# Daniel-Lin-S/decode_tonal_langauge

Measured on AMD Instinct MI355X. Metric: mel-frames/sec (train step) SynthesisModelCNN, 128ch x 400t batch256, higher is better.
Workload: dtype f32; 1 GPU; SynthesisModelCNN 128ch x 400t -> 80 mel, 4 tones x 2 syllables, L=5, global batch 256 (strong scaling: 256 windows on rank 0), dropout 0.5, NAdam, 1,376,768,720 params; per_gpu_batch=256, global_batch=256, parallelism=dp1, init=drawn on every rank

## Files before the change

### decode_tonal_langauge_amd/_classifier_engine.py

```python
from __future__ import annotations

import os
from typing import Dict, List, Tuple

import torch

from . import _kernels
from ._cnn_engine import CnnEngine, _r4
from ._lib import EPI_LRELU, EPI_STORE, LOAD_DIRECT, check, ptr


class CnnClassifierEngine(CnnEngine):
    F63_CAPABLE = False

    def __init__(self, n_electrodes: int, n_timepoints: int, stage_defs, hidden: int, n_classes: int,
                 negative_slope: float):
        super().__init__(n_classes, n_electrodes, n_timepoints, 0, stage_defs[-1][0], 0.0, negative_slope,
                         stage_defs, [4])
        self.hidden = hidden
        self.n_classes = n_classes
        last = self.stages[-1]
        self.c_last = last.cout
        self.tp_last = last.tp_out
        self.ld_last = last.cout if last.pool else self.ld5
        self.kflat_cls = n_electrodes * self.tp_last * self.ld_last
        self._packed: Dict[str, Tuple[int, torch.Tensor]] = {}
        self.n63, self.tp63 = self._plan63(stage_defs, n_timepoints)

    def _plan63(self, stage_defs, T):
        from . import _kernels
        if _kernels.get("wino") != "6":
            return 0, []
        c1, k1, p1 = stage_defs[0]
        if not (p1 and 1 <= k1 <= 3 and c1 in (128, 256, 512, 1024) and T >= 2 * self.tout1 + 2 and T * 4 <= 64 * 1024):
            return 0, []
        n, cin = 0, c1
        for st in self.stages:
            if not (st.k == 3 and st.pool and cin % 128 == 0 and st.cout % 64 == 0 and cin >= 40 and st.tout >= 1):
                break
            n, cin = n + 1, st.cout
        n = min(n, 3)
        if n == 0:
            return 0, []
        unit = 6 << (n - 1)
        tp = (self.tout1 + unit - 1) // unit * unit
        tps = []
        for _ in range(n):
            tps.append(tp)
            tp //= 2
        return n, tps

    def _forward63(self, convs, x, S, T):
        from ._lib import EPI_POOL, EPI_POOLV, LOAD_V
        lib, st_ = self.lib, self._stream()
        dev = x.device
        z = lambda *sh: torch.zeros(*sh, dtype=torch.float32, device=dev)
        zi = lambda *sh: torch.zeros(*sh, dtype=torch.int32, device=dev)
        buf = self._buf63
        w1, b1 = convs[0]
        tp1 = self.tp63[0]
        if "V1" not in buf:
            nh = S * tp1 // 6
            buf["V1"] = z((nh + 24 + 127) // 128 * 128, 8, self.c1)
            buf["b1"] = zi(S * tp1, self.c1 // 32)
        check(lib.tl_conv1_fwd_v6(ptr(x), ptr(w1.reshape(self.c1, self.k1).contiguous()), ptr(b1), None, ptr(buf["V1"]),
                                  ptr(buf["b1"]), None, S, T, self.k1, self.c1, tp1, self.tout1, self.slope, st_), "tl_conv1_fwd_v6")
        V = buf["V1"]
        tile_rows = self._nt63_rows()
        for i in range(self.n63):
            st, (w, b) = self.stages[i], convs[1 + i]
            tp_in = self.tp63[i]
            last = i == self.n63 - 1
            wp = self._cached(f"conv{st.idx}w63", w, lambda w=w: self._pack_wino63(w, True))
            rows_in = S * tp_in
            kb = f"bits{st.idx}"
            if kb not in buf:
                buf[kb] = zi(S * (st.tp_out if last else tp_in // 2), st.cout // 32)
            kw = dict(A=ptr(V), A_rows=V.shape[0], lda=V.shape[2], loader=LOAD_V, Bw=ptr(wp), bias=ptr(b), M=rows_in, N=st.cout,
                      K=st.cin, ldb=st.cin, J=3, row_shift=0, Tp=tp_in, slope=self.slope, obits=ptr(buf[kb]),
                      ld_obits=st.cout // 32, Tvalid=2 * st.tout)
            if last:
                dst = self.P[st.idx]
                self._nt(fn="tl_conv3_wino63v_nt", out=ptr(dst), ldo=dst.shape[1], epilogue=EPI_POOL, out_tp=st.tp_out, **kw)
            else:
                rows_out = S * (tp_in // 2)
                kv, kh = f"V{st.idx}", f"halo{st.idx}"
                ntm = -(-rows_in // tile_rows)
                if kv not in buf:
                    nh = rows_out // 6
                    buf[kv] = z((nh + 24 + 127) // 128 * 128, 8, st.cout)
                    buf[kh] = z(ntm, 2, st.cout)
                Vn, halo = buf[kv], buf[kh]
                self._nt(fn="tl_conv3_wino63v_nt", out=None, ldo=st.cout, epilogue=EPI_POOLV, vout=ptr(Vn), vhalo=ptr(halo),
                         vout_quads=Vn.shape[0], ld_vout=Vn.shape[2], **kw)
                check(lib.tl_wino63_v_fixup(ptr(Vn), ptr(halo), rows_out // 6, ntm, tp_in // 2, st.cout, Vn.shape[2], st_),
                      "tl_wino63_v_fixup")
                V = Vn
        return 1 + self.n63

    def _alloc(self, B: int, dev):
        if self._B == B and getattr(self, "_dev", None) == dev:
            return
        self._B, self._dev = B, dev
        S = B * self.C
        self.S = S
        self._buf63 = {}
        self.V = {}
        self._gy_A = None
        self._vhalo = {}
        z = lambda *s: torch.zeros(*s, dtype=torch.float32, device=dev)
        zi = lambda *s: torch.zeros(*s, dtype=torch.int32, device=dev)
        self.P = {1: z(S * self.tp1, self.c1)}
        self.bits = {1: zi(S * self.tp1, self.c1 // 32)}
        for st in self.stages:
            rows = S * st.tp_out
            self.P[st.idx] = z(rows, st.cout if st.pool else _r4(st.cout))
            if st.pool:
                self.bits[st.idx] = zi(rows, st.cout // 32)

    def _cached(self, key: str, param: torch.Tensor, build):
        ver = (param._version, param.data_ptr())
        hit = self._packed.get(key)
        if hit is None or hit[0] != ver:
            hit = self._packed[key] = (ver, build())
        return hit[1]

    def forward_scores(self, convs: List[Tuple[torch.Tensor, torch.Tensor]], fc1, fc2, x: torch.Tensor,
                       p_drop: float = 0.0, seed: int = 0) -> torch.Tensor:
        B, Cn, T = x.shape
        if Cn != self.C or T != self.T:
            raise ValueError(f"expected input (B, {self.C}, {self.T}), got {tuple(x.shape)}")
        x = x.contiguous().float()
        dev = x.device
        self._alloc(B, dev)
        lib, st_ = self.lib, self._stream()
        S = self.S
        w1, b1 = convs[0]
        done = 1
        if self.n63:
            done = self._forward63(convs, x, S, T)
        else:
            check(lib.tl_conv1_fwd(ptr(x), ptr(w1.reshape(self.c1, self.k1).contiguous()), ptr(b1), ptr(self.P[1]),
                                   ptr(self.bits[1]), None, S, T, self.k1, self.c1, self.tp1, self.tout1, self.slope, st_),
                  "tl_conv1_fwd")
        for st, (w, b) in list(zip(self.stages, convs[1:]))[done - 1:]:
            v43 = self._v43(st)
            if v43:
                wp = self._cached(f"conv{st.idx}w43", w, lambda w=w: self._pack_wino43(w, True))
            else:
                wp = self._cached(f"conv{st.idx}", w, lambda w=w, st=st: self._pack_conv(w, st.cin, False))
            src, dst = self.P[st.idx - 1], self.P[st.idx]
            kw = dict(A=ptr(src), Bw=ptr(wp), bias=ptr(b), out=ptr(dst), M=S * st.tp_in, A_rows=src.shape[0],
                      N=st.cout, K=st.cin, lda=src.shape[1], ldb=st.cin, ldo=dst.shape[1], J=st.k, row_shift=0,
                      Tp=st.tp_in, slope=self.slope, loader=LOAD_DIRECT)
            if st.pool:
                from ._lib import EPI_POOL
                kw.update(epilogue=EPI_POOL, obits=ptr(self.bits[st.idx]), ld_obits=st.cout // 32, Tvalid=2 * st.tout)
            else:
                kw.update(epilogue=EPI_LRELU, Tvalid=st.tout)
            if v43:
                from ._lib import LOAD_V
                V = self._input_transform(st)
                kw.update(A=ptr(V), A_rows=V.shape[0], lda=V.shape[2], loader=LOAD_V)
            self._nt(fn="tl_conv3_wino43v_nt" if v43 else "tl_gemm_nt_window", **kw)
        feat = self.P[self.stages[-1].idx]
        if p_drop > 0.0:
            check(lib.tl_dropout_scale(ptr(feat), feat.numel(), float(p_drop), int(seed), st_), "tl_dropout_scale")
        w_fc1, b_fc1 = fc1
        lat, latC = self.lat, self.lat * self.C

        def pack_fc1():
            dst = torch.empty(self.hidden, self.kflat_cls, dtype=torch.float32, device=dev)
            self._permute(w_fc1, dst, (self.hidden, self.C, self.tp_last, self.ld_last),
                          (self.c_last * latC, 1, self.C, latC), (self.hidden, self.C, lat, self.c_last))
            return dst
        wp1 = self._cached("fc1", w_fc1, pack_fc1)
        f32 = dict(dtype=torch.float32, device=dev)
        nkc = (self.kflat_cls + 31) // 32
        tiles = ((B + 127) // 128) * ((self.hidden + 127) // 128)
        sk = self._splitk(tiles, nkc, 1024)
        if sk > 1:
            slab = torch.empty(sk, B, self.hidden, **f32)
            self._nt(A=ptr(feat), Bw=ptr(wp1), out=ptr(slab), M=B, A_rows=B, N=self.hidden, K=self.kflat_cls,
                     lda=self.kflat_cls, ldb=self.kflat_cls, ldo=self.hidden, loader=LOAD_DIRECT, epilogue=EPI_STORE,
                     splitk=sk, slab_stride=B * self.hidden)
            a1 = torch.empty(B, self.hidden, **f32)
            check(lib.tl_splitk_bias_lrelu(ptr(slab), ptr(b_fc1), ptr(a1), sk, B * self.hidden, self.hidden, float(self.slope), st_),
                  "tl_splitk_bias_lrelu")
        else:
            a1 = torch.empty(B, self.hidden, **f32)
            self._nt(A=ptr(feat), Bw=ptr(wp1), bias=ptr(b_fc1), out=ptr(a1), M=B, A_rows=B, N=self.hidden,
                     K=self.kflat_cls, lda=self.kflat_cls, ldb=self.kflat_cls, ldo=self.hidden, loader=LOAD_DIRECT,
                     epilogue=EPI_LRELU, slope=self.slope)
        w_fc2, b_fc2 = fc2
        out = torch.empty(B, self.n_classes, **f32)
        if self.n_classes <= 64 and self.hidden % 4 == 0:
            check(lib.tl_linear_rows(ptr(a1), ptr(w_fc2.contiguous()), ptr(b_fc2), ptr(out), B, self.hidden, self.n_classes,
                                     self.hidden, 1, st_), "tl_linear_rows")
            return out
        self._nt(A=ptr(a1), Bw=ptr(w_fc2.contiguous()), bias=ptr(b_fc2), out=ptr(out), M=B, A_rows=B,
                 N=self.n_classes, K=self.hidden, lda=self.hidden, ldb=self.hidden, ldo=self.n_classes,
                 loader=LOAD_DIRECT, epilogue=EPI_STORE)
        return torch.sigmoid(out)


def _launch_nt(lib, fn: str = "tl_gemm_nt_window", **kw) -> None:
    import ctypes as C
    from ._lib import NtParams
    p = NtParams()
    p.splitk, p.bm, p.J, p.Tp, p.Tvalid, p.slope = 1, 128, 1, 1, 1, 0.0
    for k, v in kw.items():
        setattr(p, k, v)
    check(getattr(lib, fn)(C.byref(p), torch.cuda.current_stream().cuda_stream), fn)


class LstmInferEngine:

    def __init__(self, in_dim: int, hidden: int):
        from . import _lib
        self.lib = _lib.load()
        self.in_dim, self.H = in_dim, hidden
        self.Kp, self.Hp = _r4(in_dim), (hidden + 7) // 8 * 8
        self._packed = None

    def _weights(self, w_ih, w_hh, b_ih, b_hh):
        ver = tuple((t._version, t.data_ptr()) for t in (w_ih, w_hh, b_ih, b_hh))
        if self._packed is None or self._packed[0] != ver:
            H, Hp, Kp, dev = self.H, self.Hp, self.Kp, w_hh.device
            wi = torch.zeros(4, Hp, Kp, dtype=torch.float32, device=dev)
            wi[:, :H, :self.in_dim] = w_ih.detach().float().view(4, H, self.in_dim)
            wh = torch.zeros(4, Hp, Hp, dtype=torch.float32, device=dev)
            wh[:, :H, :H] = w_hh.detach().float().view(4, H, H)
            bs = torch.zeros(4, Hp, dtype=torch.float32, device=dev)
            bs[:, :H] = (b_ih.detach().float() + b_hh.detach().float()).view(4, H)
            whp = wh.permute(1, 0, 2).contiguous().view(4 * Hp, Hp)
            self._packed = (ver, wi.view(4 * Hp, Kp), wh.view(4 * Hp, Hp), bs.view(4 * Hp), whp)
        return self._packed[1:]

    @torch.no_grad()
    def last_hidden(self, x_seq: torch.Tensor, w_ih, w_hh, b_ih, b_hh) -> torch.Tensor:
        B, T, D = x_seq.shape
        if D != self.in_dim:
            raise ValueError(f"expected input width {self.in_dim}, got {D}")
        dev = x_seq.device
        wi, wh, bs, whp = self._weights(w_ih, w_hh, b_ih, b_hh)
        H, Hp, Kp = self.H, self.Hp, self.Kp
        f32 = dict(dtype=torch.float32, device=dev)
        x = x_seq.float()
        if Kp != D:
            xp_in = torch.zeros(B, T, Kp, **f32)
            xp_in[:, :, :D] = x
            x = xp_in
        x = x.contiguous()
        rows = B * T
        xp = torch.empty(rows, 4 * Hp, **f32)
        _launch_nt(self.lib, A=ptr(x), Bw=ptr(wi), bias=ptr(bs), out=ptr(xp), M=rows, A_rows=rows, N=4 * Hp, K=Kp,
                   lda=Kp, ldb=Kp, ldo=4 * Hp, loader=LOAD_DIRECT, epilogue=EPI_STORE)
        h = torch.empty(B, Hp, **f32)
        c = torch.empty(B, Hp, **f32)
        import ctypes as C
        h2 = torch.empty(B, Hp, **f32)
        in_b = C.c_int(0)
        check(self.lib.tl_lstm_infer_seq_fused(ptr(xp), T * 4 * Hp, ptr(whp), ptr(h), ptr(h2), ptr(c), B, Hp, T,
                                               C.byref(in_b), torch.cuda.current_stream().cuda_stream),
              "tl_lstm_infer_seq_fused")
        h = h2 if in_b.value else h
        return h[:, :H] if Hp != H else h


class CnnRnnConvEngine:

    K = 7

    def __init__(self, input_channels: int, input_length: int, lstm_dim: int, negative_slope: float):
        from . import _lib
        self.lib = _lib.load()
        self.C, self.T = input_channels, input_length
        self.w1 = lstm_dim // input_length
        self.W = self.w1 + input_channels
        self.slope = float(negative_slope)
        self.t1 = (input_length - self.K + 1) // 2
        self.ta = self.t1 - self.K + 1
        self.tb = self.ta - self.K + 1
        self.tq = self.tb // 3
        if self.tq < 1:
            raise ValueError("input_length too small for the CNN-RNN convolution stack")
        _kernels.validate()
        self.conv7_form = _kernels.get("conv7")
        self.Tp = (self.t1 + 5) // 6 * 6 if self.conv7_form == "wino63" else (self.t1 + 3) // 4 * 4
        self._packed: Dict[str, Tuple[tuple, torch.Tensor]] = {}
        self._B = None

    def _cached(self, key: str, param: torch.Tensor, build):
        ver = (param._version, param.data_ptr())
        hit = self._packed.get(key)
        if hit is None or hit[0] != ver:
            hit = self._packed[key] = (ver, build())
        return hit[1]

    def _alloc(self, B: int, dev):
        if self._B == B and self._dev == dev:
            return
        self._B, self._dev = B, dev
        z = lambda *s: torch.zeros(*s, dtype=torch.float32, device=dev)
        zi = lambda *s: torch.zeros(*s, dtype=torch.int32, device=dev)
        rows = B * self.W * self.Tp
        self.P, self.Y1, self.Y2 = z(rows + 8, 1024), z(rows + 8, 512), z(rows, 256)
        nb = B * self.w1 * self.Tp
        self.Pb, self.Pa = self.P[:nb], self.P[nb:rows]
        self.bits_a, self.bits_b = zi(B * self.C * self.Tp, 32), zi(B * self.w1 * self.Tp, 32)
        self.V7 = None
        if self.conv7_form == "wino63":
            nh_pad = (rows // 6 + 2 + 127) // 128 * 128
            self.V7 = (z(nh_pad, 8, 1024), z(nh_pad, 8, 1024))

    def _conv7(self, src, w, b, dst, cin, cout, key, rows):
        from ._lib import NtParams
        import ctypes as C
        st_ = torch.cuda.current_stream().cuda_stream
        if self.conv7_form == "wino63" and cin % 8 == 0 and cout % 32 == 0:
            nhex = rows // 6
            V0 = self.V7[0].view(-1)[: self.V7[0].shape[0] * 8 * cin].view(-1, 8, cin)
            V1 = self.V7[1].view(-1)[: self.V7[1].shape[0] * 8 * cin].view(-1, 8, cin)
            tvalid = self.t1 if cin == 1024 else self.ta
            if V0.shape[2] != self.V7[0].shape[2]:
                h0 = (nhex + 1) // 2 * 2
                V0[h0:].zero_()
                V1[h0:].zero_()
            check(self.lib.tl_wino63_xform2(ptr(src), ptr(V0), ptr(V1), rows, self.Tp, tvalid, cin, src.shape[1], cin, st_),
                  "tl_wino63_xform2")

            def pack63():
                wp = torch.empty(3 * cin // 8, 8, cout, 8, dtype=torch.float32, device=w.device)
                check(self.lib.tl_wino63_weights7(ptr(w.detach().reshape(cout, cin, self.K).contiguous()), ptr(wp), cout, cin,
                                                  self.K, st_), "tl_wino63_weights7")
                return wp
            wp = self._cached(key + "wino63", w, pack63)
            from ._lib import LOAD_V
            _launch_nt(self.lib, fn="tl_conv7_wino63v_nt", A=ptr(V0), aux=ptr(V1), A_rows=V0.shape[0], lda=cin, Bw=ptr(wp),
                       bias=ptr(b.detach()), out=ptr(dst), M=rows, N=cout, K=cin, ldb=3 * cin, ldo=dst.shape[1], J=self.K,
                       row_shift=0, Tp=self.Tp, Tvalid=self.Tp, slope=self.slope, loader=LOAD_V, epilogue=EPI_LRELU)
            return
        if src.shape[0] < rows + 8:
            raise RuntimeError("conv7: the input buffer is shorter than the rows the 7-tap window reads")
        wp = self._cached(key + "direct", w, lambda: w.detach().reshape(cout, cin, self.K).permute(2, 0, 1).contiguous())
        p = NtParams()
        p.A, p.Bw, p.bias, p.out = ptr(src), ptr(wp), ptr(b.detach()), ptr(dst)
        p.M, p.A_rows = rows, rows + 8
        p.N, p.K, p.lda, p.ldb, p.ldo = cout, cin, cin, cin, cout
        p.J, p.row_shift, p.Tp, p.Tvalid, p.slope = self.K, 0, self.Tp, self.Tp, self.slope
        p.loader, p.epilogue, p.splitk, p.bm = LOAD_DIRECT, EPI_LRELU, 1, 128
        check(self.lib.tl_gemm_nt_window(C.byref(p), st_), "tl_gemm_nt_window")

    @torch.no_grad()
    def linear(self, a: torch.Tensor, w: torch.Tensor, b: torch.Tensor, sigmoid: bool = False) -> torch.Tensor:
        a = a.contiguous().float()
        B, K = a.shape
        if K % 4 != 0:
            raise ValueError("linear: the feature width must be a multiple of 4")
        N = w.shape[0]
        out = torch.empty(B, N, dtype=torch.float32, device=a.device)
        if N <= 64:
            check(self.lib.tl_linear_rows(ptr(a), ptr(w.contiguous()), ptr(b), ptr(out), B, K, N, K, int(sigmoid),
                                          torch.cuda.current_stream().cuda_stream), "tl_linear_rows")
            return out
        _launch_nt(self.lib, A=ptr(a), Bw=ptr(w.contiguous()), bias=ptr(b), out=ptr(out), M=B, A_rows=B, N=N, K=K, lda=K,
                   ldb=K, ldo=N, loader=LOAD_DIRECT, epilogue=EPI_STORE)
        return torch.sigmoid(out) if sigmoid else out

    @torch.no_grad()
    def features(self, x: torch.Tensor, h1: torch.Tensor, block1, block2, conv3a, conv3b, p_drop: float = 0.0,
                 seed: int = 0) -> torch.Tensor:
        B = x.shape[0]
        dev = x.device
        self._alloc(B, dev)
        lib, st_ = self.lib, torch.cuda.current_stream().cuda_stream
        xa = x.contiguous().float()
        xb = h1.float().reshape(B, self.T, self.w1).permute(0, 2, 1).contiguous()
        for seqs, n, (w, b), P, bits in ((xa, B * self.C, block1, self.Pa, self.bits_a),
                                         (xb, B * self.w1, block2, self.Pb, self.bits_b)):
            check(lib.tl_conv1_fwd(ptr(seqs), ptr(w.detach().reshape(1024, self.K).contiguous()), ptr(b.detach()), ptr(P),
                                   ptr(bits), None, n, self.T, self.K, 1024, self.Tp, self.t1, self.slope, st_),
                  "tl_conv1_fwd")
        rows = B * self.W * self.Tp
        self._conv7(self.P, conv3a[0], conv3a[1], self.Y1, 1024, 512, "conv3a", rows)
# ... 10 lines not shown
```

### decode_tonal_langauge_amd/_cnn_engine.py

```python
from __future__ import annotations

import ctypes as C
import os
import math
from typing import Dict, List, Optional

import torch

from . import _kernels, _lib
from ._lib import (EPI_C1WGRAD, EPI_GY, EPI_LRELU, EPI_MASK, EPI_MASKY, EPI_POOL, EPI_POOLV, EPI_STORE, LOAD_DIRECT, LOAD_UNPOOL, LOAD_V,
                   LOAD_Y, NtParams, TnParams, check, ptr)


def _r4(n: int) -> int:
    return (n + 3) // 4 * 4


class _Stage:

    def __init__(self, idx, cin, cout, k, pool, tin, tp_in):
        self.idx, self.cin, self.cout, self.k, self.pool = idx, cin, cout, k, pool
        self.tin, self.tp_in = tin, tp_in
        self.tc = tin - k + 1
        self.tout = self.tc // 2 if pool else self.tc
        self.tp_out = tp_in // 2 if pool else tp_in


class CnnEngine:
    F63_CAPABLE = True

    def __init__(self, output_dim: int, n_channels: int, n_timepoints: int, lstm_channels: int,
                 conv_channels: int, dropout: float, negative_slope: float, stage_defs, concat_widths):
        if negative_slope < 0:
            raise ValueError("the MI355X path needs negative_slope >= 0 (max-pool / LeakyReLU are fused)")
        self.lib = _lib.load()
        self.out_dim = output_dim
        self.C = n_channels
        self.T = n_timepoints
        self.Lc = lstm_channels
        self.Cc = conv_channels
        self.p_drop = float(dropout)
        self.slope = float(negative_slope)
        self.cslope = 0.1
        k1 = stage_defs[0][1]
        npool_after = sum(1 for s in stage_defs[1:] if s[2])
        tc1 = n_timepoints - k1 + 1
        self.k1 = k1
        self.c1 = stage_defs[0][0]
        self.tout1 = tc1 // 2
        if not stage_defs[0][2]:
            raise ValueError("first stage must pool")
        align = 1 << npool_after
        self.tp1 = max(align, (self.tout1 + align - 1) // align * align)
        _kernels.validate()
        self.wino63 = (self.F63_CAPABLE and _kernels.get("wino") == "6"
                       and self._f63_covers(stage_defs, n_timepoints))
        tp1_default = self.tp1
        if self.wino63:
            self.tp1 = (self.tout1 + 11) // 12 * 12
        self.f63_yprod = (self.wino63 and _kernels.get("f63_yprod") != "0" and stage_defs[0][0] % 256 == 0
                          and self.tp1 >= 12)
        self.f63_yprod3 = (self.wino63 and _kernels.get("f63_yprod") != "0" and stage_defs[1][0] % 256 == 0)
        self.stages: List[_Stage] = []
        cin, tin, tp = self.c1, self.tout1, self.tp1
        for i, (cout, k, pool) in enumerate(stage_defs[1:], start=2):
            st = _Stage(i, cin, cout, k, pool, tin, tp)
            if st.tout < 1:
                raise ValueError("n_timepoints too small for the conv stack")
            if self.wino63 and i == 3:
                st.tp_out = tp1_default // 4
            self.stages.append(st)
            cin, tin, tp = cout, st.tout, st.tp_out
        self.gy4 = self._gy_applies()
        self.lat = tin
        self.tp5 = tp
        self.H = self.lat * n_channels * lstm_channels
        self.ld5 = _r4(conv_channels)
        self.ldx = _r4(conv_channels + lstm_channels)
        self.concat_dims = []
        cin_t, cin_ld = conv_channels + lstm_channels, self.ldx
        for w in concat_widths:
            self.concat_dims.append((cin_t, cin_ld, w, _r4(w)))
            cin_t, cin_ld = w, _r4(w)
        self.ldy5 = self.concat_dims[-1][3]
        self.kflat = n_channels * self.tp5 * self.ldy5
        self.ldd = _r4(output_dim)
        self.lowrank_param = "label_lstm.weight_hh_l0"
        self.lstm_shard = None
        self._sh = None
        self.timers = None
        mode = _kernels.get("wino")
        self.wino43 = mode != "0"
        self.store_p1 = _kernels.get("store_p1") == "1"
        self.fuse_c1 = True
        self.wino_vout = True
        self.tn_bm = 0
        self._gy_A = None
        self._vhalo = {}
        self._B = None
        self.generation = 0
        self._saved_generation = -1

    def _alloc(self, B: int, dev):
        if self._B == B and self._dev == dev:
            return
        self._B, self._dev = B, dev
        S = B * self.C
        self.S = S
        f32 = dict(dtype=torch.float32, device=dev)
        z = lambda *s: torch.zeros(*s, **f32)
        zi = lambda *s: torch.zeros(*s, dtype=torch.int32, device=dev)
        self._v_ready = {}
        self._gy_A = None
        self._vhalo = {}
        self.P = {}
        if not (self.wino63 or self._conv1_writes_v()) or self.store_p1:
            self.P[1] = z(S * self.tp1, self.c1)
        self.bits = {1: zi(S * self.tp1, self.c1 // 32)}
        self.sbits = {1: zi(S * self.tp1, self.c1 // 32)}
        for st in self.stages:
            rows = S * st.tp_out
            ld = st.cout if st.pool else self.ld5
            no_rows = (self.wino63 and st.idx == 2) or (self._writes_v(st) and not self._f63(st))
            if not no_rows or self.store_p1:
                self.P[st.idx] = z(rows, ld)
            if st.pool:
                self.bits[st.idx] = zi(rows, st.cout // 32)
                self.sbits[st.idx] = zi(rows, st.cout // 32)
        rows5 = S * self.tp5
        self.rows5 = rows5
        self.Xc = z(rows5, self.ldx)
        self.Y = [z(rows5, d[3]) for d in self.concat_dims]
        self.out_slab = None
        self.Yt = {}
        self._y_ready = {}
        self.V = {}
        self.Vd = {}
        self._vd_ready = {}
        self.G = None

    def _alloc_bwd(self):
        if self.G is not None:
            return
        dev = self._dev
        f32 = dict(dtype=torch.float32, device=dev)
        z = lambda *s: torch.zeros(*s, **f32)
        S = self.S
        self.G = {}
        if not self.wino63 and not (self.fuse_c1 and self._c1_fusable() and self._v43(self.stages[0])):
            self.G[1] = z(S * self.tp1, self.c1)
        for st in self.stages:
            if not (self.f63_yprod and st.idx == 2) and not (self.gy4 and st.idx == 3):
                self.G[st.idx] = z(S * st.tp_out, st.cout if st.pool else self.ld5)
        self.GY = [z(self.rows5, d[3]) for d in self.concat_dims]
        self.dXc = z(self.rows5, self.ldx)

    def _stream(self):
        return torch.cuda.current_stream().cuda_stream

    def enable_timers(self, on: bool = True):
        self.timers = {} if on else None

    def _tick(self, name):
        if self.timers is None or name is None:
            return None
        ev = (torch.cuda.Event(enable_timing=True), torch.cuda.Event(enable_timing=True))
        self.timers.setdefault(name, []).append(ev)
        ev[0].record()
        return ev

    def timer_summary(self):
        torch.cuda.synchronize()
        out = {}
        for k, evs in (self.timers or {}).items():
            ms = [a.elapsed_time(b) for a, b in evs]
            out[k] = (len(ms), sum(ms) / max(len(ms), 1))
        return out

    def _permute(self, src, dst, dims, strides, lims=None, nz=1, zs=0, src_off=0, bias=None):
        d = (C.c_int64 * 4)(*dims)
        s = (C.c_int64 * 4)(*strides)
        l = (C.c_int64 * 4)(*(lims if lims is not None else dims))
        check(self.lib.tl_permute_reduce(src.data_ptr() + 4 * src_off, dst.data_ptr(), d, s, l, nz, zs, ptr(bias),
                                         self._stream()), "tl_permute_reduce")

    def _nt(self, tag=None, fn="tl_gemm_nt_window", **kw):
        p = NtParams()
        p.splitk, p.bm, p.J, p.Tp, p.slope = 1, 128, 1, 1, 0.0
        for k, v in kw.items():
            setattr(p, k, v)
        ev = self._tick(tag)
        check(getattr(self.lib, fn)(C.byref(p), self._stream()), fn)
        if ev:
            ev[1].record()

    def _tn(self, tag=None, fn="tl_gemm_tn_window", **kw):
        p = TnParams()
        p.splitk, p.J, p.Tp, p.Tvalid = 1, 1, 1, 1
        for k, v in kw.items():
            setattr(p, k, v)
        ev = self._tick(tag)
        check(getattr(self.lib, fn)(C.byref(p), self._stream()), fn)
        if ev:
            ev[1].record()

    @staticmethod
    def _splitk(tiles: int, ksteps: int, target: int = 2048) -> int:
        return int(max(1, min(ksteps, (target + tiles - 1) // tiles, 1024)))

    @staticmethod
    def _splitk_rounds(tiles: int, ksteps: int, slots: int = 512, max_sk: int = 32, min_rounds: float = 1.9) -> int:
        cands = []
        for sk in range(1, max(1, min(max_sk, ksteps)) + 1):
            n = tiles * sk
            cands.append((sk, n, n / (-(-n // slots) * slots)))
        full = [c for c in cands if c[2] >= 0.95]
        for sk, n, _ in full:
            if n >= min_rounds * slots:
                return sk
        if full:
            return full[-1][0]
        return max(cands, key=lambda c: c[2])[0]

    def _pack_conv(self, w, cin_ld, flip_for_dgrad):
        O, I, J, _ = w.shape
        if not flip_for_dgrad:
            dst = torch.empty(J, O, cin_ld, dtype=torch.float32, device=w.device)
            self._permute(w, dst, (1, J, O, cin_ld), (0, 1, I * J, J), (1, J, O, I))
            return dst
        old = _r4(O)
        dst = torch.empty(J, cin_ld, old, dtype=torch.float32, device=w.device)
        self._permute(w, dst, (1, J, cin_ld, old), (0, -1, J, I * J), (1, J, I, O), src_off=J - 1)
        return dst


    @staticmethod
    def _f63_covers(stage_defs, T) -> bool:
        if len(stage_defs) < 4:
            return False
        (c1, k1, p1), (c2, k2, p2), (c3, k3, p3) = stage_defs[0], stage_defs[1], stage_defs[2]
        tout1 = (T - k1 + 1) // 2
        tout2 = (tout1 - 2) // 2
        tout3 = (tout2 - 2) // 2
        return (p1 and p2 and p3 and k2 == 3 and k3 == 3 and 1 <= k1 <= 3 and c1 in (128, 256, 512, 1024)
                and c2 % 128 == 0 and c3 % 64 == 0 and tout3 >= 1 and T >= 2 * tout1 + 2)

    def _f63(self, st) -> bool:
        return self.wino63 and st.idx in (2, 3)

    def _nt63_rows(self) -> int:
        return int(self.lib.tl_wino63_nt_tile_rows())

    def _v_hex_buffer(self, store, idx, rows, cin):
        nh = rows // 6
        nh_pad = (nh + 24 + 127) // 128 * 128
        V = store.get(idx)
        if V is None or V.shape[0] != nh_pad or V.shape[1] != 8 or V.shape[2] != cin:
            V = store[idx] = torch.zeros(nh_pad, 8, cin, dtype=torch.float32, device=self._dev)
        return V

    def _halo_buffer(self, key, ntm, cout):
        halo = self._vhalo.get(key)
        if halo is None or halo.shape[0] != ntm or halo.shape[2] != cout:
            halo = self._vhalo[key] = torch.zeros(ntm, 2, cout, dtype=torch.float32, device=self._dev)
        return halo

    def _pack_wino63(self, w, forward: bool):
        O, I = w.shape[0], w.shape[1]
        dst = torch.empty(8, O, I, dtype=torch.float32, device=w.device) if forward else \
            torch.empty(8, I, O, dtype=torch.float32, device=w.device)
        check(self.lib.tl_wino63_weights(ptr(w), ptr(dst) if forward else None, None if forward else ptr(dst), O, I, I, O,
                                         self._stream()), "tl_wino63_weights")
        return dst

    def f63_issue_factor(self, st) -> float:
        return (st.tp_in // 6) * 8.0 / (st.tc * 3.0)

    def _stage_forward63(self, st, w, bia) -> None:
        S = self.S
        wp = self._pack_wino63(w, True)
        V = self._v_ready[st.idx - 1]
        if st.idx == 2 and self.store_p1 and 2 not in self.P:
            self.P[2] = torch.zeros(S * st.tp_out, st.cout, dtype=torch.float32, device=self._dev)
        Pout = self.P.get(st.idx) if (st.idx != 2 or self.store_p1) else None
        kw = dict(A=ptr(V), A_rows=V.shape[0], lda=V.shape[2], loader=LOAD_V, Bw=ptr(wp), bias=ptr(bia), out=ptr(Pout),
                  M=S * st.tp_in, N=st.cout, K=st.cin, ldb=st.cin, ldo=Pout.shape[1] if Pout is not None else st.cout, J=3,
                  row_shift=0, Tp=st.tp_in, slope=self.slope, obits=ptr(self.bits[st.idx]), osign=ptr(self.sbits[st.idx]),
                  ld_obits=st.cout // 32, Tvalid=2 * st.tout)
        if st.idx == 2:
            rows_out = S * st.tp_out
            Vn = self._v_hex_buffer(self.V, 2, rows_out, st.cout)
            ntm = -(-(S * st.tp_in) // self._nt63_rows())
            halo = self._halo_buffer(2, ntm, st.cout)
            kw.update(epilogue=EPI_POOLV, vout=ptr(Vn), vhalo=ptr(halo), vout_quads=Vn.shape[0], ld_vout=Vn.shape[2])
            self._nt(tag="conv2_fwd", fn="tl_conv3_wino63v_nt", **kw)
            check(self.lib.tl_wino63_v_fixup(ptr(Vn), ptr(halo), rows_out // 6, ntm, st.tp_out, st.cout, Vn.shape[2],
                                             self._stream()), "tl_wino63_v_fixup")
            self._v_ready[2] = Vn
        else:
            if Pout is None:
                raise RuntimeError("F(6,3) stage 3 writes pooled rows: its output buffer was not allocated")
            kw.update(epilogue=EPI_POOL, out_tp=st.tp_out)
            self._nt(tag="conv3_fwd", fn="tl_conv3_wino63v_nt", **kw)

    def _stage_wgrad63(self, st, gw, gb) -> None:
        S = self.S
        f32 = dict(dtype=torch.float32, device=self._dev)
        rows_in = S * st.tp_in
        nd = st.cout
        ldg = nd
        V = self._v_ready[st.idx - 1]
        tiles = (st.cin // 64) * (nd // 64)
        sk = self._splitk(tiles, (rows_in + 35) // 36, 4096)
        slab = torch.empty(sk, 8 * st.cin, ldg, **f32)
        bias_part = torch.empty(sk, nd, **f32)
        if (st.idx == 3 and self.f63_yprod3 and self._y_ready.get(3) != self.generation):
            Gs = self.G[3]
            Y3 = self._v_hex_buffer(self.Yt, 3, rows_in, nd)
            Vd3 = self._v_hex_buffer(self.Vd, 3, rows_in, nd)
            ev = self._tick("conv3_yvd")
            check(self.lib.tl_wino63_unpool_yvd(ptr(Gs), ptr(self.bits[3]), ptr(Y3), ptr(Vd3), rows_in, Gs.shape[0], st.tp_in,
                                                st.tp_out, 2 * st.tout, nd, Gs.shape[1], st.cout // 32, nd, self._stream()),
                  "tl_wino63_unpool_yvd")
            if ev:
                ev[1].record()
            self._y_ready[3] = self.generation
            self._vd_ready[3] = self.generation
        if self._y_ready.get(st.idx) == self.generation:
            Y = self.Yt[st.idx]
            self._y_ready[st.idx] = -1
            self._tn(tag=f"conv{st.idx}_wgrad", fn="tl_conv3_wino63v_tn", A=ptr(V), B=ptr(Y), slab=ptr(slab), Krows=rows_in,
                     A_rows=V.shape[0], B_rows=Y.shape[0], Mdim=st.cin, Ndim=nd, lda=V.shape[2], ldb=Y.shape[2], ldc=ldg, J=3,
                     Tp=st.tp_in, splitk=sk, slab_stride=8 * st.cin * ldg, loader=LOAD_Y, Tvalid=2 * st.tout,
                     colsum=ptr(bias_part))
        else:
            Gs = self.G[st.idx]
            Vd = self._v_hex_buffer(self.Vd, st.idx, rows_in, nd)
            self._tn(tag=f"conv{st.idx}_wgrad", fn="tl_conv3_wino63v_tn", A=ptr(V), B=ptr(Gs), slab=ptr(slab), Krows=rows_in,
                     A_rows=V.shape[0], B_rows=Gs.shape[0], Mdim=st.cin, Ndim=nd, lda=V.shape[2], ldb=Gs.shape[1], ldc=ldg, J=3,
                     Tp=st.tp_in, splitk=sk, slab_stride=8 * st.cin * ldg, loader=LOAD_UNPOOL, bbits=ptr(self.bits[st.idx]),
                     ld_bbits=st.cout // 32, Tvalid=2 * st.tout, colsum=ptr(bias_part), vd=ptr(Vd), ld_vd=nd, g_tp=st.tp_out)
            self._vd_ready[st.idx] = self.generation
        if sk > 1:
            red = torch.empty(8 * st.cin, ldg, **f32)
            n = 8 * st.cin * ldg
            self._permute(slab, red, (1, 1, 1, n), (0, 0, 0, 1), nz=sk, zs=n)
        else:
            red = slab
        check(self.lib.tl_wino63_wgrad_finalize(ptr(red), ptr(gw), st.cout, st.cin, ldg, self._stream()),
              "tl_wino63_wgrad_finalize")
        self._permute(bias_part, gb, (1, 1, 1, st.cout), (0, 0, 0, 1), nz=sk, zs=nd)

    def _gy_stage(self, st) -> bool:
        return self.gy4 and st.idx == 4

    def _gy_applies(self) -> bool:
        if not (self.wino63 and self.f63_yprod3 and len(self.stages) >= 3):
            return False
        below, st = self.stages[1], self.stages[2]
        return (_kernels.get("conv4_dgrad") == "nt63" and st.k == 1 and st.pool and self._f63(below)
                and st.cout % 32 == 0 and st.cout >= 40 and st.cin % 32 == 0 and (below.tp_in // 2) % 3 == 0)

    def _stage_dgrad_gy(self, st, w):
        S = self.S
        below = self.stages[1]
        tpg = below.tp_in // 2
        rows = S * tpg
        f32 = dict(dtype=torch.float32, device=self._dev)
        nh = -(-rows // 6)
        nh_pad = (nh + 127) // 128 * 128
        A = self._gy_A
        if A is None or A.shape[0] != nh_pad or A.shape[2] != st.cout:
            A = self._gy_A = torch.zeros(nh_pad, 8, st.cout, **f32)
        Gs = self.G[st.idx]
        ev = self._tick(f"conv{st.idx}_dgrad")
        check(self.lib.tl_wino63_unpool_rows6(ptr(Gs), ptr(self.bits[st.idx]), ptr(A), rows, Gs.shape[0], tpg, st.tp_out,
                                              2 * st.tout, st.cout, Gs.shape[1], st.cout // 32, st.cout, 0, self._stream()),
              "tl_wino63_unpool_rows6")
        taps = torch.empty(st.cout // 8, 8, st.cin, 8, **f32)
        check(self.lib.tl_wino63_weights1(ptr(w), ptr(taps), st.cout, st.cin, st.cout, self._stream()), "tl_wino63_weights1")
        rows3 = S * below.tp_in
        Y3 = self._v_hex_buffer(self.Yt, below.idx, rows3, below.cout)
        Vd3 = self._v_hex_buffer(self.Vd, below.idx, rows3, below.cout)
        ntm = -(-rows // self._nt63_rows())
        halo = self._halo_buffer("d3", ntm, below.cout)
        self._nt(tag=None, fn="tl_conv1_wino63v_dgrad_nt", A=ptr(A), A_rows=A.shape[0], lda=A.shape[2], loader=LOAD_V,
                 Bw=ptr(taps), M=rows, N=st.cin, K=st.cout, ldb=st.cout, ldo=st.cin, J=1, row_shift=0, Tp=tpg, slope=self.slope,
                 auxbits=ptr(self.sbits[below.idx]), ld_auxbits=self.sbits[below.idx].shape[1], abits=ptr(self.bits[below.idx]),
                 ld_abits=below.cout // 32, out_tp=below.tp_out, Tvalid_in=2 * below.tout, epilogue=EPI_GY, out=None,
                 vout=ptr(Y3), vout2=ptr(Vd3), vhalo=ptr(halo), vout_quads=Y3.shape[0], ld_vout=Y3.shape[2])
        check(self.lib.tl_wino63_vd_fixup(ptr(Vd3), ptr(halo), rows // 3, ntm, below.tp_in // 6, below.cout, Vd3.shape[2],
                                          self._stream()), "tl_wino63_vd_fixup")
        if ev:
            ev[1].record()
        self._y_ready[below.idx] = self.generation
        self._vd_ready[below.idx] = self.generation
        return None

    def _stage_dgrad63(self, st, w):
        S = self.S
        rows_in = S * st.tp_in
        if self._vd_ready.get(st.idx) != self.generation:
            raise RuntimeError("F(6,3) input gradient: the stage's weight-gradient pass (which writes Vd) must run first")
        self._vd_ready[st.idx] = -1
        Vd = self.Vd[st.idx]
        wd = self._pack_wino63(w, False)
        kw = dict(A=ptr(Vd), A_rows=Vd.shape[0], lda=Vd.shape[2], loader=LOAD_V, Bw=ptr(wd), M=rows_in, N=st.cin,
                  K=st.cout, ldb=st.cout, ldo=st.cin, J=3, row_shift=-2, Tp=st.tp_in, slope=self.slope,
                  auxbits=ptr(self.sbits[st.idx - 1]), ld_auxbits=self.sbits[st.idx - 1].shape[1])
        if st.idx == 3 and self.f63_yprod:
            below = self.stages[0]
            rows2 = S * below.tp_in
            Y2 = self._v_hex_buffer(self.Yt, 2, rows2, below.cout)
            Vd2 = self._v_hex_buffer(self.Vd, 2, rows2, below.cout)
            ntm = -(-rows_in // self._nt63_rows())
            halo = self._halo_buffer("d2", ntm, below.cout)
            self._nt(tag="conv3_dgrad", fn="tl_conv3_wino63v_nt", epilogue=EPI_MASKY, out=None, vout=ptr(Y2), vout2=ptr(Vd2),
                     vhalo=ptr(halo), vout_quads=Y2.shape[0], ld_vout=Y2.shape[2], abits=ptr(self.bits[2]),
                     ld_abits=below.cout // 32, Tvalid_in=2 * below.tout, **kw)
            check(self.lib.tl_wino63_vd_fixup(ptr(Vd2), ptr(halo), rows_in // 3, ntm, below.tp_in // 6, below.cout, Vd2.shape[2],
                                              self._stream()), "tl_wino63_vd_fixup")
            self._y_ready[2] = self.generation
            self._vd_ready[2] = self.generation
            return None
        if st.idx == 3:
            self._nt(tag="conv3_dgrad", fn="tl_conv3_wino63v_nt", epilogue=EPI_MASK, out=ptr(self.G[2]), **kw)
            return None
        ntm = -(-rows_in // self._nt63_rows())
        part = torch.empty(ntm, (self.k1 + 1) * self.c1, dtype=torch.float32, device=self._dev)
        self._nt(tag="conv2_dgrad", fn="tl_conv3_wino63v_nt", epilogue=EPI_C1WGRAD, out=None, c1x=ptr(self._x),
                 c1bits=ptr(self.bits[1]), c1partial=ptr(part), c1T=self.T, c1kt=self.k1, Tvalid=self.tout1, **kw)
        return part

    def _c1_fusable(self) -> bool:
        return self.k1 <= 3 and self.T >= 2 * self.tout1 + 2

    def _v43(self, st) -> bool:
        return (self.wino43 and st.k == 3 and st.pool and st.cin % 64 == 0 and st.cout % 32 == 0 and st.tp_in % 4 == 0
                and _r4(st.cout) % 16 == 0)

    def _tn_bm(self, st) -> int:
        wide = st.cin % 128 == 0
        dma8 = wide and _r4(st.cout) % 64 == 0 and (st.cout // 32) % 2 == 0
        if self.tn_bm == 127:
            return 127 if wide else 64
        if self.tn_bm in (0, 128):
            return 128 if dma8 else 64
        return 64

    def _conv1_writes_v(self) -> bool:
        return (self._v43(self.stages[0]) and self.tp1 % 4 == 0 and self.c1 in (128, 256, 512, 1024)
                and (self.fuse_c1 and self._c1_fusable()))

    def _writes_v(self, st) -> bool:
        if not (self.wino_vout and st.pool and st.idx - 1 < len(self.stages)):
            return False
        nxt = self.stages[st.idx - 1]
        return self._v43(st) and self._v43(nxt) and st.tp_in % 8 == 0 and nxt.cin == st.cout

    def _pin(self, st):
        return self.P.get(st.idx - 1)

    def _v_buffer(self, idx, rows, cin):
        nq = rows // 4
        nq_pad = (nq + 127) // 128 * 128
        V = self.V.get(idx)
        if V is None or V.shape[0] != nq_pad or V.shape[2] != cin:
            V = self.V[idx] = torch.zeros(nq_pad, 6, cin, dtype=torch.float32, device=self._dev)
        return V

    def _input_transform(self, st):
        src = self.P[st.idx - 1]
        V = self._v_buffer(st.idx - 1, src.shape[0], st.cin)
        ev = self._tick(f"conv{st.idx}_xform")
        check(self.lib.tl_wino43_input_transform(ptr(src), ptr(V), src.shape[0], st.tp_in, st.cin, src.shape[1], st.cin,
                                                 self._stream()), "tl_wino43_input_transform")
        if ev:
            ev[1].record()
        return V

    def wgrad_issue_factor(self, st) -> float:
        if self._f63(st):
            return self.f63_issue_factor(st)
        return 0.5 if self._v43(st) else 1.0

    def kernel_families(self):
        if self.wino63:
            self._fam_share = {}
            st2, st3 = self.stages[0], self.stages[1]
            f6 = "Winograd F(6,3) on pre-transformed operands, LDS-DMA"
            tn = "wino63v_tn4_kernel<true>" if st3.cin % 256 == 0 and st3.tp_in >= 12 else "wino63v_tn_kernel<true>"
            tn2 = "wino63v_tn4_kernel<true>" if st2.cin % 256 == 0 else "wino63v_tn_kernel<true>"
            fams = {f"wino63v_nt_kernel<POOLV> (conv2 forward, {f6}; writes V of its pooled output for conv3)": ["conv2_fwd"],
                    f"wino63v_nt_kernel<POOL> (conv3 forward, {f6})": ["conv3_fwd"],
                    f"wino63v_nt_kernel<C1WGRAD> (conv2 input gradient + conv1 weight gradient, {f6})": ["conv2_dgrad"],
                    }
            if self.f63_yprod3:
                gy = self.gy4
                src = "the epilogue of conv4's input gradient" if gy else "wino63_unpool_yvd_kernel"
                fams[f"wino63v_tn4y_kernel (conv3 weight gradient, {f6}: both operands by LDS-DMA, no transform in the kernel; Y3 / Vd3 "
                     f"from {src})"] = ["conv3_wgrad"]
            else:
                fams[f"{tn} (conv3 weight gradient, {f6}; also writes Vd)"] = ["conv3_wgrad"]
            if self.f63_yprod:
                fams[f"wino63v_nt_kernel<MASKY> (conv3 input gradient, {f6}; writes Y and Vd of conv2 instead of the gradient rows)"] = ["conv3_dgrad"]
                fams[f"wino63v_tn4y_kernel (conv2 weight gradient, {f6}: both operands by LDS-DMA, no transform in the kernel)"] = ["conv2_wgrad"]
            else:
                fams[f"wino63v_nt_kernel<MASK> (conv3 input gradient, {f6})"] = ["conv3_dgrad"]
                fams[f"{tn2} (conv2 weight gradient, {f6}; also writes Vd)"] = ["conv2_wgrad"]
            issued = {k: self.f63_issue_factor(st2 if "conv2" in k else st3) for k in fams}
            return fams, issued
        self._fam_share = {}
        if not all(self._v43(st) for st in self.stages[:2]):
            fams = {"nt_window_kernel<128,UNPOOL,MASK> (conv input-gradient)": ["conv2_dgrad", "conv3_dgrad", "conv4_dgrad"],
                    "nt_window_kernel<128,DIRECT,POOL> (conv forward)": ["conv2_fwd", "conv3_fwd", "conv4_fwd"],
                    "tn3_kernel<UNPOOL> (conv weight-gradient)": ["conv2_wgrad", "conv3_wgrad"]}
            return fams, {k: 1.0 for k in fams}
        form = "Winograd F(4,3) on pre-transformed operands, LDS-DMA"
        fused = self.fuse_c1 and self._c1_fusable()
        bm = self._tn_bm(self.stages[0])
        extra = {}
        if bm == 128:
            tn = f"wino43v_tn8_kernel<true> (conv2/conv3 weight gradient, {form}; also writes Vd for the input gradient)"
        else:
            ntm = (self.stages[0].cin + 63) // 64
            tn = f"wino43v_tn_kernel<false, 2> (conv2/conv3 weight gradient, C_in tiles 1..{ntm - 1} of {ntm}, {form})"
            vdn = f"wino43v_tn_kernel<true, 2> (conv2/conv3 weight gradient, C_in tile 0 of {ntm}, {form}, + writes Vd for the input gradient)"
            extra[vdn] = ["conv2_wgrad_vd", "conv3_wgrad_vd"]
            self._fam_share = {tn: (ntm - 1) / ntm, vdn: 1.0 / ntm}
        fams = {tn: ["conv2_wgrad", "conv3_wgrad"]}
        if self._writes_v(self.stages[0]):
            fams[f"wino43v_nt_kernel<POOLV> (conv2 forward, {form}; writes V of its pooled output for conv3 instead of the raw rows)"] = ["conv2_fwd"]
            fams[f"wino43v_nt_kernel<POOL> (conv3 forward, {form})"] = ["conv3_fwd"]
        else:
            fams[f"wino43v_nt_kernel<POOL> (conv2/conv3 forward, {form})"] = ["conv2_fwd", "conv3_fwd"]
        fams.update(extra)
        if fused:
            fams[f"wino43v_nt_kernel<UNPOOL,C1WGRAD> (conv2 input gradient + conv1 weight gradient, {form})"] = ["conv2_dgrad"]
            fams[f"wino43v_nt_kernel<UNPOOL,MASK> (conv3 input gradient, {form})"] = ["conv3_dgrad"]
        else:
            fams[f"wino43v_nt_kernel<UNPOOL,MASK> (conv2/conv3 input gradient, {form})"] = ["conv2_dgrad", "conv3_dgrad"]
        return fams, {k: 0.5 for k in fams}

    def _pack_wino43(self, w, forward: bool):
        O, I = w.shape[0], w.shape[1]
        dst = torch.empty(6, O, I, dtype=torch.float32, device=w.device) if forward else \
            torch.empty(6, I, O, dtype=torch.float32, device=w.device)
        check(self.lib.tl_wino43_weights(ptr(w), ptr(dst) if forward else None, None if forward else ptr(dst), O, I, I, O,
                                         self._stream()), "tl_wino43_weights")
        return dst

    STAGE_NAMES = {2: "ecog_conv_block.3", 3: "ecog_conv_block.6", 4: "ecog_conv_block.9", 5: "ecog_conv_block.12"}

    def stage_forward(self, st: _Stage, w: torch.Tensor, bia: torch.Tensor) -> None:
        if self._f63(st):
            return self._stage_forward63(st, w, bia)
        S = self.S
        v43 = self._v43(st)
        wp = self._pack_wino43(w, True) if v43 else self._pack_conv(w, st.cin, False)
        src = self._pin(st)
        vout = self._writes_v(st)
        if vout and self.store_p1 and st.idx not in self.P:
            self.P[st.idx] = torch.zeros(S * st.tp_out, st.cout, dtype=torch.float32, device=self._dev)
        Pout = self.P.get(st.idx) if (not vout or self.store_p1) else None
        kw = dict(A=ptr(src), Bw=ptr(wp), bias=ptr(bia), out=ptr(Pout), M=S * st.tp_in,
                  A_rows=S * st.tp_in, N=st.cout, K=st.cin, lda=st.cin, ldb=st.cin,
                  ldo=Pout.shape[1] if Pout is not None else st.cout, J=st.k, row_shift=0, Tp=st.tp_in, slope=self.slope,
                  loader=LOAD_DIRECT)
        if st.pool:
            kw.update(epilogue=EPI_POOL, obits=ptr(self.bits[st.idx]), osign=ptr(self.sbits[st.idx]),
                      ld_obits=st.cout // 32, Tvalid=2 * st.tout)
        else:
            kw.update(epilogue=EPI_LRELU, Tvalid=st.tout)
        if not v43:
            self._nt(tag=f"conv{st.idx}_fwd", fn="tl_gemm_nt_window", **kw)
            return
        V = self._v_ready.get(st.idx - 1)
        if V is None:
            V = self._v_ready[st.idx - 1] = self._input_transform(st)
        kw.update(A=ptr(V), A_rows=V.shape[0], lda=V.shape[2], loader=LOAD_V)
        if vout:
            rows_out = S * st.tp_out
            Vn = self._v_buffer(st.idx, rows_out, st.cout)
            ntm = (S * st.tp_in + 511) // 512
            halo = self._halo_buffer(st.idx, ntm, st.cout)
            kw.update(epilogue=EPI_POOLV, vout=ptr(Vn), vhalo=ptr(halo), vout_quads=Vn.shape[0], ld_vout=Vn.shape[2])
            self._nt(tag=f"conv{st.idx}_fwd", fn="tl_conv3_wino43v_nt", **kw)
            check(self.lib.tl_wino43_v_fixup(ptr(Vn), ptr(halo), rows_out // 4, ntm, st.tp_out, st.cout, Vn.shape[2],
                                             self._stream()), "tl_wino43_v_fixup")
            self._v_ready[st.idx] = Vn
            return
        self._nt(tag=f"conv{st.idx}_fwd", fn="tl_conv3_wino43v_nt", **kw)

    def _colsum(self, Gm, rows, ncols, ld, Tp, Tvalid, dst):
        nc4 = _r4(ncols)
        rpb = max(1, 256 // (nc4 // 4))
        nblk = int(min(2048, max(1, rows // (rpb * 16))))
        part = torch.empty(nblk, nc4, dtype=torch.float32, device=Gm.device)
        check(self.lib.tl_colsum(ptr(Gm), ptr(part), nblk, rows, nc4, ld, Tp, Tvalid, self._stream()), "tl_colsum")
        self._permute(part, dst, (1, 1, 1, ncols), (0, 0, 0, 1), nz=nblk, zs=nc4)

    def _reduce_c1_partials(self, part: torch.Tensor, gw: torch.Tensor, gb: torch.Tensor) -> None:
        f32 = dict(dtype=torch.float32, device=part.device)
        nblk = part.shape[0]
        zs = (self.k1 + 1) * self.c1
        if nblk >= 256 and zs % 4 == 0:
            red = torch.empty(zs, **f32)
            flat = part.view(-1)
            for c0 in range(0, zs, 1024):
                nc = min(1024, zs - c0)
                self._colsum(flat[c0:], nblk, nc, zs, 1, 1, red[c0:c0 + nc])
            self._permute(red, gw, (1, 1, self.c1, self.k1), (0, 0, 1, self.c1))
            self._permute(red, gb, (1, 1, 1, self.c1), (0, 0, 0, 1), src_off=self.k1 * self.c1)
        else:
            self._permute(part, gw, (1, 1, self.c1, self.k1), (0, 0, 1, self.c1), nz=nblk, zs=zs)
            self._permute(part, gb, (1, 1, 1, self.c1), (0, 0, 0, 1), nz=nblk, zs=zs, src_off=self.k1 * self.c1)

    def stage_wgrad(self, st: _Stage, gw: torch.Tensor, gb: torch.Tensor) -> None:
        if self._f63(st):
            return self._stage_wgrad63(st, gw, gb)
        S = self.S
        f32 = dict(dtype=torch.float32, device=self._dev)
        Xin = self._pin(st)
        Gs = self.G[st.idx]
        rows_in = S * st.tp_in
        ldg = Gs.shape[1]
        nd = _r4(st.cout)
        if self._v43(st):
            tiles = ((st.cin + 63) // 64) * ((nd + 63) // 64)
            bm = self._tn_bm(st)
            sk = self._splitk(tiles, (rows_in + 31) // 32, 4096 if bm in (127, 128) else 8192)
            slab = torch.empty(sk, 6 * st.cin, ldg, **f32)
            bias_part = torch.empty(sk, nd, **f32)
            V = self._v_ready.get(st.idx - 1)
            if V is None:
                V = self._v_ready[st.idx - 1] = self._input_transform(st)
            nq_pad = (rows_in // 4 + 127) // 128 * 128
            Vd = self.Vd.get(st.idx)
            if Vd is None or Vd.shape[0] != nq_pad or Vd.shape[2] != nd:
                Vd = self.Vd[st.idx] = torch.zeros(nq_pad, 6, nd, **f32)
            kw = dict(A=ptr(V), B=ptr(Gs), slab=ptr(slab), Krows=rows_in, A_rows=V.shape[0], B_rows=Gs.shape[0],
                      Mdim=st.cin, Ndim=nd, lda=V.shape[2], ldb=ldg, ldc=ldg, J=3, Tp=st.tp_in, splitk=sk,
                      slab_stride=6 * st.cin * ldg, loader=LOAD_UNPOOL, bbits=ptr(self.bits[st.idx]),
                      ld_bbits=st.cout // 32, Tvalid=2 * st.tout, colsum=ptr(bias_part), bm=bm, vd=ptr(Vd), ld_vd=nd)
            self._vd_ready[st.idx] = self.generation
            if self.timers is not None and bm != 128:
                self._tn(tag=f"conv{st.idx}_wgrad_vd", fn="tl_conv3_wino43v_tn", part=1, **kw)
                self._tn(tag=f"conv{st.idx}_wgrad", fn="tl_conv3_wino43v_tn", part=2, **kw)
            else:
                self._tn(tag=f"conv{st.idx}_wgrad", fn="tl_conv3_wino43v_tn", **kw)
            if sk > 1:
                red = torch.empty(6 * st.cin, ldg, **f32)
                n = 6 * st.cin * ldg
                self._permute(slab, red, (1, 1, 1, n), (0, 0, 0, 1), nz=sk, zs=n)
            else:
                red = slab
            check(self.lib.tl_wino43_wgrad_finalize(ptr(red), ptr(gw), st.cout, st.cin, ldg, self._stream()),
                  "tl_wino43_wgrad_finalize")
            self._permute(bias_part, gb, (1, 1, 1, st.cout), (0, 0, 0, 1), nz=sk, zs=nd)
            return
        if st.k == 3:
            tiles = ((st.cin + 127) // 128) * ((nd + 63) // 64)
        else:
            tiles = st.k * ((st.cin + 127) // 128) * ((nd + 127) // 128)
        sk = self._splitk(tiles, (rows_in + 31) // 32, 1024)
        slab = torch.empty(sk, st.k * st.cin, ldg, **f32)
        kw = dict(A=ptr(Xin), B=ptr(Gs), slab=ptr(slab), Krows=rows_in, A_rows=Xin.shape[0], B_rows=Gs.shape[0],
                  Mdim=st.cin, Ndim=nd, lda=st.cin, ldb=ldg, ldc=ldg, J=st.k, Tp=st.tp_in, splitk=sk,
                  slab_stride=st.k * st.cin * ldg)
        if st.pool:
            kw.update(loader=LOAD_UNPOOL, bbits=ptr(self.bits[st.idx]), ld_bbits=st.cout // 32, Tvalid=2 * st.tout)
        else:
            kw.update(loader=LOAD_DIRECT, Tvalid=st.tout)
        fold = (not st.pool) and st.k == 1 and rows_in > 512 and st.cin > 32
        bpart = torch.empty(sk, nd, **f32) if fold else None
        if fold:
            kw.update(colsum=ptr(bpart))
        self._tn(tag=f"conv{st.idx}_wgrad", **kw)
        if sk > 1:
            red = torch.empty(st.k * st.cin, ldg, **f32)
            n = st.k * st.cin * ldg
            self._permute(slab, red, (1, 1, 1, n), (0, 0, 0, 1), nz=sk, zs=n)
        else:
            red = slab
        self._permute(red, gw, (1, st.cout, st.cin, st.k), (0, 1, ldg, st.cin * ldg))
        if fold:
            self._permute(bpart, gb, (1, 1, 1, st.cout), (0, 0, 0, 1), nz=sk, zs=nd)
        else:
            self._colsum(Gs, Gs.shape[0], st.cout, ldg, st.tp_out, st.tout, gb)

    def stage_dgrad(self, st: _Stage, w: torch.Tensor):
        if self._f63(st):
            return self._stage_dgrad63(st, w)
        if self._gy_stage(st):
            return self._stage_dgrad_gy(st, w)
        S = self.S
        Xin = self._pin(st)
        Gs = self.G[st.idx]
        rows_in = S * st.tp_in
        ldg = Gs.shape[1]
        v43 = self._v43(st)
        wd = self._pack_wino43(w, False) if v43 else self._pack_conv(w, st.cin, True)
        kd = wd.shape[2]
        fuse = st.idx == 2 and v43 and self.fuse_c1 and self._c1_fusable()
        kw = dict(A=ptr(Gs), Bw=ptr(wd), aux=ptr(Xin), out=None if fuse else ptr(self.G[st.idx - 1]), M=rows_in,
                  A_rows=Gs.shape[0], N=st.cin, K=kd, lda=ldg, ldb=kd, ldo=st.cin, ldaux=st.cin, J=st.k,
                  row_shift=-(st.k - 1), Tp=st.tp_in, epilogue=EPI_MASK, slope=self.slope)
        if (st.idx - 1) in self.sbits:
            kw.update(auxbits=ptr(self.sbits[st.idx - 1]), ld_auxbits=self.sbits[st.idx - 1].shape[1])
        if st.pool:
            kw.update(loader=LOAD_UNPOOL, abits=ptr(self.bits[st.idx]), ld_abits=st.cout // 32,
                      Tvalid_in=2 * st.tout)
        else:
            kw.update(loader=LOAD_DIRECT)
        if not v43:
            self._nt(tag=f"conv{st.idx}_dgrad", fn="tl_gemm_nt_window", **kw)
            return None
        part = None
        if fuse:
            ntm = (rows_in + 511) // 512
            part = torch.empty(ntm, (self.k1 + 1) * self.c1, dtype=torch.float32, device=self._dev)
            kw.update(epilogue=EPI_C1WGRAD, out=None, c1x=ptr(self._x), c1bits=ptr(self.bits[1]), c1partial=ptr(part),
                      c1T=self.T, c1kt=self.k1, Tvalid=self.tout1)
        if self._vd_ready.get(st.idx) != self.generation or st.idx not in self.Vd:
            raise RuntimeError("F(4,3) input gradient: the stage's weight-gradient pass (which writes Vd) must run first")
        Vd = self.Vd[st.idx]
        kw.update(A=ptr(Vd), A_rows=Vd.shape[0], lda=Vd.shape[2], loader=LOAD_V)
        self._vd_ready[st.idx] = -1
        self._nt(tag=f"conv{st.idx}_dgrad", fn="tl_conv3_wino43v_nt", **kw)
        return part

    def _lstm_forward(self, prm, xu, U, L, dev, training, label_table) -> None:
        lib, st_ = self.lib, self._stream()
        H = self.H
        f32 = dict(dtype=torch.float32, device=dev)
        self._act = torch.empty(L, U, 4 * H, **f32)
        self._c = torch.empty(L, U, H, **f32)
        self._h = torch.empty(L, U, H, **f32)
        hh = torch.empty(U, 4 * H, **f32) if L > 1 else None
        w_ih, w_hh = prm["label_lstm.weight_ih_l0"], prm["label_lstm.weight_hh_l0"]
        b_ih, b_hh = prm["label_lstm.bias_ih_l0"], prm["label_lstm.bias_hh_l0"]
        bm = 32 if U <= 64 else 128
        self._sh = None
        if (self.lstm_shard is not None and label_table is not None and training and L > 1 and (L - 1) * U <= 64
                and (4 * H) % (4 * self.lstm_shard[1]) == 0):
            rk, wd = self.lstm_shard
            self._sh = (rk * (4 * H // wd), 4 * H // wd, wd)
        nloc = self._sh[1] if self._sh else 4 * H
        sk_f = self._splitk_rounds(((U + bm - 1) // bm) * ((nloc + 127) // 128), (H + 31) // 32, min_rounds=8.9) if L > 1 else 1
        slab_f = torch.empty(sk_f, U, nloc, **f32) if sk_f > 1 else None
        if self._sh:
            from . import parallel
            hh_loc = torch.empty(U, nloc, **f32)
            hh_all = torch.empty(self._sh[2], U, nloc, **f32)
        for t in range(L):
            if t > 0 and self._sh:
                r0, R, wd = self._sh
                self._nt(A=ptr(self._h[t - 1]), Bw=w_hh.data_ptr() + 4 * r0 * H, out=ptr(slab_f if sk_f > 1 else hh_loc),
                         M=U, A_rows=U, N=R, K=H, lda=H, ldb=H, ldo=R, loader=LOAD_DIRECT, epilogue=EPI_STORE, bm=bm,
                         splitk=sk_f, slab_stride=U * R)
                if sk_f > 1:
                    self._permute(slab_f, hh_loc, (1, 1, 1, U * R), (0, 0, 0, 1), nz=sk_f, zs=U * R)
                parallel.all_gather_blocks(hh_all, hh_loc)
                self._permute(hh_all, hh, (1, U, wd, R), (0, R, U * R, 1))
            elif t > 0:
                self._nt(A=ptr(self._h[t - 1]), Bw=ptr(w_hh), out=ptr(slab_f if sk_f > 1 else hh), M=U, A_rows=U,
                         N=4 * H, K=H, lda=H, ldb=H, ldo=4 * H, loader=LOAD_DIRECT, epilogue=EPI_STORE, bm=bm,
                         splitk=sk_f, slab_stride=U * 4 * H)
                if sk_f > 1:
                    n = U * 4 * H
                    self._permute(slab_f, hh, (1, 1, 1, n), (0, 0, 0, 1), nz=sk_f, zs=n)
            check(lib.tl_lstm_cell_fwd(ptr(hh) if t > 0 else None, ptr(xu[t]), ptr(w_ih), ptr(b_ih), ptr(b_hh),
                                       ptr(self._c[t - 1]) if t > 0 else None, ptr(self._act[t]), ptr(self._c[t]),
                                       ptr(self._h[t]), U, H, 2, 4 * H, st_), "tl_lstm_cell_fwd")

    def forward(self, prm: Dict[str, torch.Tensor], x: torch.Tensor, labels: torch.Tensor, training: bool,
                save: bool, seed: int = 0, row0: int = 0, label_ids: Optional[torch.Tensor] = None,
                label_table: Optional[torch.Tensor] = None) -> torch.Tensor:
        B, Cn, T = x.shape
        if Cn != self.C or T != self.T:
            raise ValueError(f"expected ECoG input (B, {self.C}, {self.T}), got {tuple(x.shape)}")
        if labels.dim() != 3 or labels.shape[0] != B or labels.shape[1] != 2:
            raise ValueError(f"expected labels (B, 2, L), got {tuple(labels.shape)}")
        x = x.contiguous().float()
        labels = labels.contiguous().float()
        dev = x.device
        self._alloc(B, dev)
        lib, st_ = self.lib, self._stream()
        S = self.S
        self.generation += 1
        p_drop = self.p_drop if training else 0.0
        self._p_drop_used, self._seed_used = p_drop, seed
        self._drop_row0 = int(row0) * self.C * self.tp5
        self._x = x
        self._v_ready = {}
        w1 = prm["ecog_conv_block.0.weight"].reshape(self.c1, self.k1).contiguous()
        if self.wino63:
            V1 = self._v_hex_buffer(self.V, 1, S * self.tp1, self.c1)
            if self.store_p1 and 1 not in self.P:
                self.P[1] = torch.zeros(S * self.tp1, self.c1, dtype=torch.float32, device=dev)
            ev = self._tick("conv1_fwd")
            check(lib.tl_conv1_fwd_v6(ptr(x), ptr(w1), ptr(prm["ecog_conv_block.0.bias"]),
                                      ptr(self.P[1]) if self.store_p1 else None, ptr(V1), ptr(self.bits[1]), ptr(self.sbits[1]),
                                      S, T, self.k1, self.c1, self.tp1, self.tout1, self.slope, st_), "tl_conv1_fwd_v6")
            if ev:
                ev[1].record()
            self._v_ready[1] = V1
        elif self._conv1_writes_v():
            if self.store_p1 and 1 not in self.P:
                self.P[1] = torch.zeros(S * self.tp1, self.c1, dtype=torch.float32, device=dev)
            V1 = self._v_buffer(1, S * self.tp1, self.c1)
            check(lib.tl_conv1_fwd_v(ptr(x), ptr(w1), ptr(prm["ecog_conv_block.0.bias"]),
                                     ptr(self.P[1]) if self.store_p1 else None, ptr(V1), ptr(self.bits[1]), ptr(self.sbits[1]),
# ... 251 lines not shown
```

### decode_tonal_langauge_amd/_kernels.py

```python
from __future__ import annotations

import os
from typing import Callable, Dict, Tuple, Union

_Allowed = Union[frozenset, Callable[[str], bool]]


def _int(lo: int, hi: int) -> Callable[[str], bool]:
    def ok(v: str) -> bool:
        try:
            return lo <= int(v) <= hi
        except ValueError:
            return False
    return ok


_B = frozenset({"0", "1"})
KEYS: Dict[str, Tuple[str, _Allowed, str, str]] = {
    "wino": ("TONAL_WINO", frozenset({"6", "4", "0"}), "6",
             "conv2 / conv3: 6 Winograd F(6,3) on pre-transformed operands (F(4,3) V form where the stack does not allow it), "
             "4 the F(4,3) V form, 0 direct MFMA kernels (also the fallback for every shape neither form covers)"),
    "f63_yprod": ("TONAL_F63_YPROD", _B, "1", "F(6,3): the backward operands Y / Vd of stages 2 and 3 come pre-transformed out of the "
                                              "input-gradient epilogue of the stage above (0: the weight-gradient kernels un-pool and "
                                              "transform the gradient rows themselves)"),
    "conv4_dgrad": ("TONAL_CONV4_DGRAD", frozenset({"nt63", "gemm"}), "nt63",
                    "F(6,3): the one-tap stage behind conv3 - nt63: its input gradient on the NT63 kernel, writing Y3 / Vd3 "
                    "(no gradient rows, no tl_wino63_unpool_yvd); gemm: one-tap GEMM + tl_wino63_unpool_yvd"),
    "store_p1": ("TONAL_STORE_P1", _B, "0", "keep the raw pooled rows of stages 1 / 2 beside V (tests)"),
    "conv7": ("TONAL_CONV7", frozenset({"wino63", "direct"}), "wino63", "the CNN-RNN classifier's 7-tap convolutions"),
    "whh_dh": ("TONAL_WHH_DH", _B, "1", "single process: the W_hh NAdam pass also produces the last BPTT product dh_1 = dgates_2 . W_hh "
                                        "(0: a W_hh stream of its own for it)"),
    "whh_stream": ("TONAL_WHH_STREAM", _B, "1", "label LSTM backward: dgates . W_hh as a pure stream of the weight (tl_lstm_gw; 0: the skinny "
                                                "MFMA GEMM with split-K slabs, also the form for more than 8 distinct label rows)"),
    "graph": ("TONAL_GRAPH", _B, "1", "SynthesisLite step replayed as a HIP graph"),
    "lstm_shard": ("TONAL_LSTM_SHARD", _B, "1", "data parallel: label LSTM sharded by gate rows"),
    "hilbert": ("TONAL_HILBERT", frozenset({"auto", "ols", "ols_full", "sym", "taps", "fft"}), "auto",
                "Hilbert bank: force a path (ols band-limited overlap-save, ols_full all 1024 bins per band, sym / taps the "
                "time-domain kernels with / without Hermitian symmetry, fft the DFT-domain form)"),
    "hilbert_f32": ("TONAL_HILBERT_F32", _B, "0", "float32 recordings: fp32 transforms end to end (default: fp64 math)"),
    "butter": ("TONAL_BUTTER", frozenset({"seq", "scan"}), "seq",
               "zero-phase Butterworth: seq the sequential recurrence (bit-identical to scipy's loop), scan the time-parallel "
               "block scan (2e-8 - 5e-8 from it: the size of the reference's own rounding; ~20 x faster)"),
}
_LEGACY = {v[0]: k for k, v in KEYS.items()}
_cache: Tuple[str, Dict[str, str]] = ("", {})


def _check(key: str, value: str) -> str:
    allowed = KEYS[key][1]
    ok = allowed(value) if callable(allowed) else value in allowed
    if not ok:
        what = "an integer in range" if callable(allowed) else "one of " + ", ".join(sorted(allowed))
        raise ValueError(f"TONAL_KERNELS: {key}={value!r} is not a value this switch takes ({what})")
    return value


def _parsed() -> Dict[str, str]:
    global _cache
    raw = os.environ.get("TONAL_KERNELS", "")
    if raw == _cache[0]:
        return _cache[1]
    out: Dict[str, str] = {}
    for item in raw.split(","):
        item = item.strip()
        if not item:
            continue
        key, sep, value = item.partition("=")
        key, value = key.strip(), value.strip()
        if not sep or key not in KEYS:
            raise ValueError(f"TONAL_KERNELS: unknown setting {item!r}; keys: " + ", ".join(sorted(KEYS)))
        out[key] = _check(key, value)
    _cache = (raw, out)
    return out


def get(key: str, default: str = None) -> str:
    legacy, _allowed, table_default, _doc = KEYS[key]
    spec = _parsed()
    if key in spec:
        return spec[key]
    if legacy in os.environ:
        if os.environ.get("TONAL_AB") != "1":
            raise RuntimeError(f"{legacy} is an A/B switch of the test suite and is ignored by the product: use "
                               f"TONAL_KERNELS={key}={os.environ[legacy]} (or set TONAL_AB=1 to run an A/B comparison)")
        return _check(key, os.environ[legacy])
    return table_default if default is None else default


def validate() -> None:
    _parsed()
    if os.environ.get("TONAL_AB") != "1":
        for legacy, key in _LEGACY.items():
            if legacy in os.environ:
                get(key)
```

### decode_tonal_langauge_amd/csrc/tonal_wino63.hip

```cpp
#include "tonal_common.h"
#include "tonal_wino43_epi.h"
#include "tonal_wino43v_epi.h"
#include "tonal_wino63_epi.h"
#include "tonal_wino63_kloop.h"
#include <type_traits>

namespace tl {

typedef __attribute__((address_space(3))) void lds_void6_t;
__device__ __forceinline__ void dma16h(__amdgpu_buffer_rsrc_t rs, char* lds_dst, unsigned voff, unsigned soff) {
  __builtin_amdgcn_raw_ptr_buffer_load_lds(rs, (lds_void6_t*)lds_dst, 16, voff, soff, 0, 0);
}

typedef int v6_i32x4 __attribute__((ext_vector_type(4)));
__device__ __forceinline__ v6_i32x4 v6_rsrc_words(const void* base, long long bytes) {
  const unsigned long long a = (unsigned long long)base;
  const long long n = bytes < 0 ? 0 : (bytes < 0x7fffffffLL ? bytes : 0x7fffffffLL);
  return v6_i32x4{(int)(unsigned)a, (int)(unsigned)((a >> 32) & 0xffffu), (int)n, 0x00020000};
}

__device__ __forceinline__ long long v6_at(long long hex, int i, int c, int kc8) {
  return ((((hex >> 1) * kc8 + (c >> 3)) * 8 + i) * 2 + (hex & 1)) * 8 + (c & 7);
}

__global__ void wino63_weights_kernel(const float* __restrict__ w, float* __restrict__ fwd, float* __restrict__ dgr, int O,
                                      int I, int ld_f, int ld_d) {
  const long long n_f = (long long)O * ld_f, n_d = (long long)I * ld_d;
  const long long idx = (long long)blockIdx.x * blockDim.x + threadIdx.x;
  auto emit = [](float* dst, int R, int r, int k, float g0, float g1, float g2) {
    float* d0 = dst + (((long long)(k >> 3) * 8) * R + r) * 8 + (k & 7);
    const long long n = (long long)R * 8;
    const float s = g0 + g2;
    d0[0] = -g0;
    d0[n] = (-2.f / 9.f) * (s + g1);
    d0[2 * n] = (-2.f / 9.f) * (s - g1);
    const float a = fmaf(4.f, g2, g0), b = 2.f * g1;
    d0[3 * n] = (1.f / 90.f) * (a + b);
    d0[4 * n] = (1.f / 90.f) * (a - b);
    const float c = fmaf(4.f, g0, g2), d = 2.f * g1;
    d0[5 * n] = (8.f / 45.f) * (c + d);
    d0[6 * n] = (8.f / 45.f) * (c - d);
    d0[7 * n] = g2;
  };
  if (fwd != nullptr && idx < n_f) {
    const int o = (int)(idx / ld_f), i = (int)(idx % ld_f);
    float g0 = 0.f, g1 = 0.f, g2 = 0.f;
    if (i < I) {
      const float* s = w + ((long long)o * I + i) * 3;
      g0 = s[0], g1 = s[1], g2 = s[2];
    }
    emit(fwd, O, o, i, g0, g1, g2);
  }
  if (dgr != nullptr && idx < n_d) {
    const int i = (int)(idx / ld_d), o = (int)(idx % ld_d);
    float g0 = 0.f, g1 = 0.f, g2 = 0.f;
    if (o < O) {
      const float* s = w + ((long long)o * I + i) * 3;
      g0 = s[2], g1 = s[1], g2 = s[0];
    }
    emit(dgr, I, i, o, g0, g1, g2);
  }
}

__global__ void wino63_wgrad_finalize_kernel(const float* __restrict__ red, float* __restrict__ gw, int O, int I, int ld) {
  const long long idx = (long long)blockIdx.x * blockDim.x + threadIdx.x;
  if (idx >= (long long)O * I) return;
  const int i = (int)(idx / O), o = (int)(idx % O);
  const long long plane = (long long)I * ld;
  const float* s = red + (long long)i * ld + o;
  float m[8];
#pragma unroll
  for (int t = 0; t < 8; ++t) m[t] = s[t * plane];
  const float a12 = m[1] + m[2], s12 = m[1] - m[2], a34 = m[3] + m[4], s34 = m[3] - m[4], a56 = m[5] + m[6], s56 = m[5] - m[6];
  float* d = gw + ((long long)o * I + i) * 3;
  d[0] = -m[0] - (2.f / 9.f) * a12 + (1.f / 90.f) * a34 + (32.f / 45.f) * a56;
  d[1] = -(2.f / 9.f) * s12 + (1.f / 45.f) * s34 + (16.f / 45.f) * s56;
  d[2] = -(2.f / 9.f) * a12 + (2.f / 45.f) * a34 + (8.f / 45.f) * a56 + m[7];
}

__global__ void wino63_weights7_kernel(const float* __restrict__ w, float* __restrict__ fwd, int O, int I, int taps) {
  const long long idx = (long long)blockIdx.x * blockDim.x + threadIdx.x;
  if (idx >= 3LL * O * I) return;
  const int k = (int)(idx % (3LL * I)), o = (int)(idx / (3LL * I));
  const int seg = k / I, i = k - seg * I;
  const float* s = w + ((long long)o * I + i) * taps + 3 * seg;
  const float g0 = 3 * seg < taps ? s[0] : 0.f, g1 = 3 * seg + 1 < taps ? s[1] : 0.f, g2 = 3 * seg + 2 < taps ? s[2] : 0.f;
  float* d0 = fwd + (((long long)(k >> 3) * 8) * O + o) * 8 + (k & 7);
  const long long n = (long long)O * 8;
  const float sm = g0 + g2;
  d0[0] = -g0;
  d0[n] = (-2.f / 9.f) * (sm + g1);
  d0[2 * n] = (-2.f / 9.f) * (sm - g1);
  const float a = fmaf(4.f, g2, g0), b = 2.f * g1;
  d0[3 * n] = (1.f / 90.f) * (a + b);
  d0[4 * n] = (1.f / 90.f) * (a - b);
  const float c = fmaf(4.f, g0, g2), d = 2.f * g1;
  d0[5 * n] = (8.f / 45.f) * (c + d);
  d0[6 * n] = (8.f / 45.f) * (c - d);
  d0[7 * n] = g2;
}

__global__ __launch_bounds__(256, 4) void wino63_xform2_kernel(const float* __restrict__ P, float* __restrict__ V0, float* __restrict__ V1,
                                                             long long nhex, int hps, int Tp, int Tvalid, int C, int ldp, int ldv) {
  const int tpp = C >> 1;
  const long long idx = (long long)blockIdx.x * blockDim.x + threadIdx.x;
  const long long pair = idx / tpp;
  const int tl_ = (int)(idx - pair * tpp);
  const int half = tl_ & 1, hpar = (tl_ >> 1) & 1, kc = tl_ >> 2;
  const int c = 8 * kc + 4 * half;
  const long long hg = 2 * pair + hpar;
  if (hg >= nhex) return;
  const long long seq = hg / hps;
  const int hs = (int)(hg - seq * hps);
  const float* src = P + (seq * Tp + 6LL * hs) * (long long)ldp + c;
  f32x4 d[11];
#pragma unroll
  for (int j = 0; j < 11; ++j) {
    d[j] = f32x4{0.f, 0.f, 0.f, 0.f};
    if (6 * hs + j < Tvalid) d[j] = *reinterpret_cast<const f32x4*>(src + (long long)j * ldp);
  }
  f32x4 o0[8], o1[8];
#pragma unroll
  for (int k = 0; k < 4; ++k) {
    float a[8], b[8], va[8], vb[8];
#pragma unroll
    for (int j = 0; j < 8; ++j) {
      a[j] = d[j][k];
      b[j] = d[j + 3][k];
    }
    wino63_bt(a, va);
    wino63_bt(b, vb);
#pragma unroll
    for (int j = 0; j < 8; ++j) {
      o0[j][k] = va[j];
      o1[j][k] = vb[j];
    }
  }
  const long long at = v6_at(hg, 0, c, ldv >> 3);
#pragma unroll
  for (int j = 0; j < 8; ++j) *reinterpret_cast<f32x4*>(V0 + at + 16 * j) = o0[j];
#pragma unroll
  for (int j = 0; j < 8; ++j) *reinterpret_cast<f32x4*>(V1 + at + 16 * j) = o1[j];
}

__global__ __launch_bounds__(256, 4) void wino63_v_fixup_kernel(float* __restrict__ V, const float* __restrict__ halo, long long hexes,
                                                              long long tiles, int Tq, int C, int ldv) {
  const int c4n = C >> 2;
  const long long idx = (long long)blockIdx.x * blockDim.x + threadIdx.x;
  if (idx >= tiles * c4n) return;
  const long long t = idx / c4n;
  const int c = (int)(idx - t * c4n) * 4;
  const long long q = t * 64 + 63;
  if (q >= hexes) return;
  float* v = V + v6_at(q, 0, c, ldv >> 3);
  f32x4 d[8];
#pragma unroll
  for (int j = 0; j < 6; ++j) d[j] = *reinterpret_cast<const f32x4*>(v + 16 * j);
  const int tq = (int)((6 * q) % Tq);
  if (tq + 6 < Tq && t + 1 < tiles) {
    d[6] = *reinterpret_cast<const f32x4*>(halo + ((t + 1) * 2) * (long long)C + c);
    d[7] = *reinterpret_cast<const f32x4*>(halo + ((t + 1) * 2 + 1) * (long long)C + c);
  } else {
    d[6] = d[7] = f32x4{0.f, 0.f, 0.f, 0.f};
  }
  f32x4 o[8];
#pragma unroll
  for (int k = 0; k < 4; ++k) {
    float dd[8], vv[8];
#pragma unroll
    for (int j = 0; j < 8; ++j) dd[j] = d[j][k];
    wino63_bt(dd, vv);
#pragma unroll
    for (int j = 0; j < 8; ++j) o[j][k] = vv[j];
  }
#pragma unroll
  for (int j = 0; j < 8; ++j) *reinterpret_cast<f32x4*>(v + 16 * j) = o[j];
}

constexpr int V6_BH = 128, V6_BN = 64, V6_BK = 8;
constexpr int V6_ROWB = V6_BK * 4;
constexpr int V6_A_BYTES = 8 * V6_BH * V6_ROWB;
constexpr int V6_B_BYTES = 8 * V6_BN * V6_ROWB;
constexpr int V6_STAGE = V6_A_BYTES + V6_B_BYTES;
constexpr int V6_ROWS = 6 * V6_BH;

template <int EPI>
__global__ __launch_bounds__(512, 2) void wino63v_nt_kernel(const tl_nt_params p) {
  __shared__ __attribute__((aligned(1024))) char lds[3 * V6_STAGE + ((EPI == W_EPI_POOLV || EPI == W_EPI_MASKY || EPI == W_EPI_GY) ? 4096 : EPI == W_EPI_C1W ? 16384 : 0)];
  const int tid = threadIdx.x;
  const int lane = tid & 63;
  const int wave = __builtin_amdgcn_readfirstlane(tid >> 6);
  const int wm = wave >> 1, wn = wave & 1;
  const int lr = lane & 31, lh = lane >> 5;

  const int ntn = (p.N + V6_BN - 1) / V6_BN;
  const long long ntm = (p.M + V6_ROWS - 1) / V6_ROWS;
  const long long nwg = ntm * ntn;
  constexpr bool SEG3 = EPI == W_EPI_LRELU;
  constexpr bool SIX = EPI == W_EPI_GY;
  const int kseg = p.K / V6_BK;
  const int nsteps = SEG3 ? 3 * kseg : kseg;
  f32x16 acc[8];
  f32x4 faL[4], fbL[4], faH[4], fbH[4];

  const int prow = lane >> 1;
  const int src_chunk = (lane & 1) ^ ((lane >> 4) & 1);
  const v6_i32x4 rsB = v6_rsrc_words(p.Bw, (SIX && wave >= 6) ? 0 : 8LL * p.N * p.ldb * 4);
  const unsigned lds0 = (unsigned)(unsigned long long)(lds_void6_t*)lds;
  const unsigned dst_a0 = lds0 + (unsigned)(wave * V6_BH * V6_ROWB);
  const unsigned dst_b0 = lds0 + (unsigned)(V6_A_BYTES + wave * V6_BN * V6_ROWB);
  const int hex_of_row = (prow & 3) | ((prow >> 3) << 2) | (((prow >> 2) & 1) << 4);
  const int kc8 = p.lda >> 3;
  unsigned avoff[4], bv_lane[2];
#pragma unroll
  for (int t = 0; t < 4; ++t) avoff[t] = (unsigned)(v6_at(t * 32 + hex_of_row, wave, src_chunk * 4, kc8) * 4);
  unsigned avoff1[4];
#pragma unroll
  for (int t = 0; t < 4; ++t) avoff1[t] = SEG3 ? (unsigned)(v6_at(t * 32 + hex_of_row + 1, wave, src_chunk * 4, kc8) * 4) : avoff[t];
#pragma unroll
  for (int t = 0; t < 2; ++t) bv_lane[t] = (unsigned)((((long long)wave * p.N + t * 32 + prow) * 8 + src_chunk * 4) * 4);
  const unsigned b_step = (unsigned)p.N * 256u;

  struct tile_t {
    long long tm, R0;
    int n0;
    v6_i32x4 rsA, rsA1;
    unsigned bvoff[2];
  };
  const long long a_tile_bytes = (long long)V6_BH * 8 * p.lda * 4, a_total_bytes = p.A_rows * 8LL * p.lda * 4;
  auto place = [&](tile_t& t, long long tm, int tn) {
    t.tm = tm;
    t.R0 = tm * V6_ROWS;
    t.n0 = tn * V6_BN;
    const long long ab = tm * a_tile_bytes;
    t.rsA = v6_rsrc_words(reinterpret_cast<const char*>(p.A) + ab, (SIX && wave >= 6) ? 0 : a_total_bytes - ab);
    t.rsA1 = SEG3 ? v6_rsrc_words(reinterpret_cast<const char*>(p.aux) + ab, a_total_bytes - ab) : t.rsA;
    if (t.n0 + V6_BN <= p.N) {
      const unsigned nb4 = (unsigned)t.n0 * 32u;
#pragma unroll
      for (int k = 0; k < 2; ++k) t.bvoff[k] = bv_lane[k] + nb4;
    } else {
#pragma unroll
      for (int k = 0; k < 2; ++k) {
        int n = t.n0 + k * 32 + prow;
        if (n > p.N - 1) n = p.N - 1;
        t.bvoff[k] = (unsigned)((((long long)wave * p.N + n) * 8 + src_chunk * 4) * 4);
      }
    }
  };
  tile_t cur;
  {
    long long bid = blockIdx.x;
    const long long q = nwg / 8, r = nwg % 8, x = bid % 8, i = bid / 8;
    bid = (x < r ? x * (q + 1) : r * (q + 1) + (x - r) * q) + i;
    place(cur, bid / ntn, (int)(bid % ntn));
  }
  const int walk = (int)(gridDim.x >> 3), walk_q = walk / ntn, walk_r = walk - walk_q * ntn;
  auto advance = [&](const tile_t& c) -> tile_t {
    tile_t t = c;
    int tn = c.n0 / V6_BN + walk_r;
    long long tm = c.tm + walk_q;
    if (tn >= ntn) {
      tn -= ntn;
      ++tm;
    }
    place(t, tm, tn);
    return t;
  };
  auto next3 = [](int s) { return s == 2 ? 0 : s + 1; };

  const int cphys = (lh ^ ((lr >> 3) & 1)) << 4;
  const unsigned a_row = lds0 + (unsigned)((wm * 32 + lr) * V6_ROWB + cphys);
  const unsigned b_row = lds0 + (unsigned)((wn * 32 + lr) * V6_ROWB + cphys);
  int stg = 0;

  struct dma_src {
    v6_i32x4 ra;
    unsigned va[4], vb[2], sa, sb;
  };
  auto src_of = [&](const tile_t& t, int step) {
    dma_src d;
    int ks = step;
    if constexpr (SEG3) {
      const int seg = (step >= kseg ? 1 : 0) + (step >= 2 * kseg ? 1 : 0);
      ks = step - seg * kseg;
#pragma unroll
      for (int k = 0; k < 4; ++k) {
        d.ra[k] = seg == 1 ? t.rsA1[k] : t.rsA[k];
        d.va[k] = seg == 2 ? avoff1[k] : avoff[k];
      }
    } else {
      d.ra = t.rsA;
#pragma unroll
      for (int k = 0; k < 4; ++k) d.va[k] = avoff[k];
    }
    d.vb[0] = t.bvoff[0];
    d.vb[1] = t.bvoff[1];
#pragma unroll
    for (int k = 0; k < 4; ++k) d.ra[k] = __builtin_amdgcn_readfirstlane(d.ra[k]);
    d.sa = (unsigned)__builtin_amdgcn_readfirstlane(ks * 512);
    d.sb = (unsigned)__builtin_amdgcn_readfirstlane((int)((unsigned)step * b_step));
    return d;
  };
#define V6K_INPUTS(src, dst, wimm)                                                                                             \
  [a] "v"(a_row + (unsigned)stg * (unsigned)V6_STAGE), [b] "v"(b_row + (unsigned)stg * (unsigned)V6_STAGE),                    \
      [va0] "v"((src).va[0]), [va1] "v"((src).va[1]), [va2] "v"((src).va[2]), [va3] "v"((src).va[3]), [vb0] "v"((src).vb[0]), \
      [vb1] "v"((src).vb[1]), [ra] "s"((src).ra), [rb] "s"(rsB), [m0a] "s"(dst_a0 + (unsigned)(dst) * (unsigned)V6_STAGE),     \
      [m0b] "s"(dst_b0 + (unsigned)(dst) * (unsigned)V6_STAGE), [sa] "s"((src).sa), [sb] "s"((src).sb), [w] "n"(wimm)
#pragma clang diagnostic ignored "-Winline-asm"
#define V6K_STMT_R(REGS, TEXT, tl_, step, dst, wimm)                                                                     \
  do {                                                                                                                   \
    const dma_src src_ = src_of(tl_, step);                                                                              \
    asm volatile(TEXT : REGS(acc, faL, fbL, faH, fbH) : V6K_INPUTS(src_, dst, wimm) : "memory", "scc", "m0");                  \
  } while (0)
#define V6K_STMT(TEXT, tl_, step, dst, wimm) V6K_STMT_R(V6K_REGS, TEXT, tl_, step, dst, wimm)
  auto issue = [&](const tile_t& tl_, int step, int dst) {
    const dma_src src_ = src_of(tl_, step);
    asm volatile(V6K_ISSUE : : V6K_INPUTS(src_, dst, 0) : "memory", "scc", "m0");
  };
  constexpr bool early = EPI == W_EPI_POOLV || EPI == W_EPI_C1W;
  constexpr int NST = v6_stores<EPI>();
  constexpr int first_n = NST + 6 > 63 ? 63 : NST + 6;
  constexpr int first_wait = (first_n & 15) | (7 << 4) | (0 << 8) | ((first_n >> 4) << 14);

  issue(cur, 0, 0);
  issue(cur, 1, 1);
  __builtin_amdgcn_s_waitcnt(0x0f70);
  for (long long vb = blockIdx.x; vb < nwg; vb += gridDim.x) {
    __builtin_amdgcn_s_barrier();
    asm volatile("" ::: "memory");
    auto prefetch = [&] {
      if constexpr (EPI == W_EPI_POOL || EPI == W_EPI_POOLV || EPI == W_EPI_LRELU) return v5_prefetch_pool(p, cur.n0, wn, lr);
      else if constexpr (EPI == W_EPI_MASK) return v6_prefetch_mask(p, cur.R0, cur.n0, wm, wn, lr, lh);
      else if constexpr (EPI == W_EPI_MASKY) return v6_prefetch_masky(p, cur.R0, cur.n0, wm, wn, lr, lh);
      else if constexpr (EPI == W_EPI_GY) return v6_prefetch_masky<true>(p, cur.R0, cur.n0, wm, wn, lr, lh);
      else return v6_prefetch_c1w(p, cur.R0, cur.n0, wm, wn, lr, lh);
    };
    decltype(prefetch()) pre;
#define V6K_RUN(KIND, RSFX, tl_, step, dst, wimm)                                                                              \
  do {                                                                                                                         \
    if constexpr (SIX) V6K_STMT_R(V6K6_REGS##RSFX, V6K6_##KIND##_L, tl_, step, dst, wimm);                                     \
    else if constexpr (early) V6K_STMT_R(V6K_REGS##RSFX, V6K_##KIND##_E, tl_, step, dst, wimm);                                \
    else V6K_STMT_R(V6K_REGS##RSFX, V6K_##KIND##_L, tl_, step, dst, wimm);                                                     \
  } while (0)
    if constexpr (SIX) V6K_STMT_R(V6K6_REGS_FIRST, V6K6_FIRST, cur, 2, stg == 0 ? 2 : stg - 1, first_wait);
    else V6K_STMT_R(V6K_REGS_FIRST, V6K_FIRST, cur, 2, stg == 0 ? 2 : stg - 1, first_wait);
    stg = next3(stg);
    V6K_RUN(STEP1, _STEP1, cur, 3, stg == 0 ? 2 : stg - 1, 0);
    stg = next3(stg);
    {
      int s = 2;
      do {
        V6K_RUN(NORM, , cur, s + 2, stg == 0 ? 2 : stg - 1, 0);
        stg = next3(stg);
      } while (++s + 2 < nsteps);
    }
    V6K_RUN(PRELAST, , cur, 0, 0, 0);
    stg = next3(stg);
    pre = prefetch();
    V6K_RUN(LAST, , cur, 0, 0, 0);
    stg = next3(stg);
#undef V6K_RUN

    const tile_t done = cur;
    const long long nb = vb + gridDim.x;
    const int last_stage = stg == 0 ? 2 : stg - 1;
    __builtin_amdgcn_s_waitcnt(0x0f70);
    if (nb < nwg) {
      cur = advance(cur);
      issue(cur, 0, stg);
      issue(cur, 1, next3(stg));
    }
    __builtin_amdgcn_sched_barrier(0);
    float* scratch = reinterpret_cast<float*>(lds + last_stage * V6_STAGE);
    (void)scratch;
    const bool full = done.R0 + V6_ROWS <= p.M && done.n0 + V6_BN <= p.N;
    if constexpr (EPI == W_EPI_POOL) {
      if (full) v6_epilogue_pool<false, true>(p, acc, pre, nullptr, done.R0, done.n0, wm, wn, lr, lh, done.tm);
      else v6_epilogue_pool<false, false>(p, acc, pre, nullptr, done.R0, done.n0, wm, wn, lr, lh, done.tm);
    } else if constexpr (EPI == W_EPI_POOLV) {
      float* xch = reinterpret_cast<float*>(lds + 3 * V6_STAGE);
      if (full) v6_epilogue_pool<true, true>(p, acc, pre, xch, done.R0, done.n0, wm, wn, lr, lh, done.tm);
      else v6_epilogue_pool<true, false>(p, acc, pre, xch, done.R0, done.n0, wm, wn, lr, lh, done.tm);
    } else if constexpr (EPI == W_EPI_LRELU) {
      if (full) v6_epilogue_lrelu<true>(p, acc, pre, done.R0, done.n0, wm, wn, lr, lh);
      else v6_epilogue_lrelu<false>(p, acc, pre, done.R0, done.n0, wm, wn, lr, lh);
    } else if constexpr (EPI == W_EPI_MASK) {
      if (full) v6_epilogue_mask<true>(p, acc, pre, done.R0, done.n0, wm, wn, lr, lh);
      else v6_epilogue_mask<false>(p, acc, pre, done.R0, done.n0, wm, wn, lr, lh);
    } else if constexpr (EPI == W_EPI_MASKY) {
      float* xch = reinterpret_cast<float*>(lds + 3 * V6_STAGE);
      if (full) v6_epilogue_masky<true>(p, acc, pre, xch, done.R0, done.n0, wm, wn, lr, lh, done.tm);
      else v6_epilogue_masky<false>(p, acc, pre, xch, done.R0, done.n0, wm, wn, lr, lh, done.tm);
    } else if constexpr (EPI == W_EPI_GY) {
      float* xch = reinterpret_cast<float*>(lds + 3 * V6_STAGE);
      if (full) v6_epilogue_masky<true, true>(p, acc, pre, xch, done.R0, done.n0, wm, wn, lr, lh, done.tm);
      else v6_epilogue_masky<false, true>(p, acc, pre, xch, done.R0, done.n0, wm, wn, lr, lh, done.tm);
    } else {
      v6_epilogue_c1w(p, acc, pre, reinterpret_cast<float*>(lds + 3 * V6_STAGE) + wave * 512, scratch, done.R0, done.n0, wm, wn,
                      lr, lh, done.tm);
    }
    {
      constexpr int n = NST + 6 > 63 ? 63 : NST + 6;
      __builtin_amdgcn_s_waitcnt((n & 15) | (7 << 4) | (15 << 8) | ((n >> 4) << 14));
    }
  }
}



constexpr int T6_BN = 64, T6_H = 6;
constexpr int T6_PLANE = T6_H * 64;
constexpr int T6_TILE = 8 * T6_PLANE;
constexpr int T6_NA = 4, T6_NG = 6;
constexpr int T6_GW = T6_H * 4 * 64;
constexpr int T6_GT = T6_GW + 64;

template <bool WVD>
__global__ __launch_bounds__(512, 1) void wino63v_tn_kernel(const tl_tn_params p, int mtn) {
  constexpr int NA = T6_NA, NG = T6_NG, GW = T6_GW, GT = T6_GT;
  __shared__ __attribute__((aligned(1024))) float lds[(NA * 2 + 2) * T6_TILE + NG * GT];
  float* As = lds;
  float* Bs = lds + NA * 2 * T6_TILE;
  float* Gs = Bs + 2 * T6_TILE;
  const int tid = threadIdx.x, lane = tid & 63;
  const int wave = __builtin_amdgcn_readfirstlane(tid >> 6);
  const int wm = wave >> 1, wn = wave & 1, lr = lane & 31, lh = lane >> 5;
  const int ntn = p.Ndim / T6_BN;
  const long long tiles = (long long)mtn * ntn;
  const long long nwg = tiles * p.splitk;
  long long bid = (long long)blockIdx.y * gridDim.x + blockIdx.x;
  {
    const long long q = nwg / 8, r = nwg % 8, x = bid % 8, i = bid / 8;
    bid = (x < r ? x * (q + 1) : r * (q + 1) + (x - r) * q) + i;
  }
  const int z = __builtin_amdgcn_readfirstlane((int)(bid / tiles));
  const int tt = __builtin_amdgcn_readfirstlane((int)(bid % tiles));
  const int mi = __builtin_amdgcn_readfirstlane(tt / ntn);
  const int m0 = mi * 128, n0 = __builtin_amdgcn_readfirstlane((tt % ntn) * T6_BN);

  const long long hexes_all = p.Krows / 6;
  const long long ksteps_all = (hexes_all + T6_H - 1) / T6_H;
  const long long per = __builtin_amdgcn_readfirstlane((int)((ksteps_all + p.splitk - 1) / p.splitk));
  const long long ks_begin = z * per;
  long long ks_end = ks_begin + per;
  if (ks_end > ksteps_all) ks_end = ksteps_all;
  const int nsteps = ks_end > ks_begin ? (int)(ks_end - ks_begin) : 0;

  f32x16 acc[8];
#pragma unroll
  for (int i = 0; i < 8; ++i)
#pragma unroll
    for (int e = 0; e < 16; ++e) acc[i][e] = 0.f;

  const long long v_h0 = ks_begin * T6_H;
  const int kc8 = p.lda >> 3;
  const __amdgpu_buffer_rsrc_t rsV = __builtin_amdgcn_make_buffer_rsrc(
      (void*)(p.A + v_h0 * 8 * (long long)p.lda), 0, clip31((p.A_rows - v_h0) * 8 * (long long)p.lda * 4), 0x00020000);
  unsigned vvoff[3], vdst[3];
#pragma unroll
  for (int t = 0; t < 3; ++t) {
    const int half = (wave * 3 + t) / 12, pc = (wave * 3 + t) % 12;
    const int rho = 4 * pc + (lane >> 4), i = rho / 6, hx = rho % 6;
    const int chunk = (lane & 15) ^ ((hx & 1) << 3);
    vvoff[t] = (unsigned)(v6_at(hx, i, m0 + half * 64 + chunk * 4, kc8) * 4);
    vdst[t] = (unsigned)((half * T6_TILE + pc * 256) * 4);
  }
  const unsigned v_step = (unsigned)(T6_H * 8 * p.lda * 4);
  auto issue_v = [&](int step) {
    char* base = reinterpret_cast<char*>(As) + (step & (NA - 1)) * (2 * T6_TILE * 4);
    const unsigned soff = (unsigned)step * v_step;
#pragma unroll
    for (int t = 0; t < 3; ++t) dma16h(rsV, base + vdst[t], vvoff[t] + soff, 0u);
  };
  const int Tq = p.Tp >> 1, hps = p.Tp / 6;
  const int g_tp = p.g_tp > 0 ? p.g_tp : Tq;
  const bool wpiece = wave >= 6;
  const int myhex = wpiece ? (lane >> 3) : wave;
  const long long seq0 = v_h0 / hps;
  const int hs0 = (int)(v_h0 - seq0 * hps);
  const long long g_r0 = seq0 * g_tp + 3LL * hs0;
  int g_hs = hs0 + myhex, g_off = 3 * myhex;
  while (g_hs >= hps) {
    g_hs -= hps;
    g_off += g_tp - Tq;
  }
  const int ldw4 = p.ld_bbits * 4;
  const __amdgpu_buffer_rsrc_t rsG = __builtin_amdgcn_make_buffer_rsrc(
      wpiece ? (void*)(p.bbits + g_r0 * (long long)p.ld_bbits + (n0 >> 5)) : (void*)(p.B + g_r0 * (long long)p.ldb + n0), 0,
      wpiece ? clip31((p.B_rows - g_r0) * (long long)ldw4 - (long long)(n0 >> 5) * 4)
             : clip31((p.B_rows - g_r0) * (long long)p.ldb * 4 - (long long)n0 * 4),
      0x00020000);
  const unsigned g_lane = wpiece ? (unsigned)(((lane >> 1) & 3) * ldw4 + (lane & 1) * 4)
                                 : (unsigned)(((lane >> 4) * (long long)p.ldb + (lane & 15) * 4) * 4);
  const unsigned g_row4 = wpiece ? (unsigned)ldw4 : (unsigned)(p.ldb * 4);
  const unsigned gdst = wpiece ? (unsigned)(GW * 4) : (unsigned)(wave * 256 * 4);
  const bool g_live = !wpiece || lane < 48;
  auto issue_g = [&](int slot) {
    const unsigned voff = g_live ? (unsigned)g_off * g_row4 + g_lane : 0xfffffff0u;
    if (wpiece) __builtin_amdgcn_raw_ptr_buffer_load_lds(rsG, (lds_void6_t*)(reinterpret_cast<char*>(Gs) + slot * (GT * 4) + gdst), 4, voff, 0u, 0, 0);
    else dma16h(rsG, reinterpret_cast<char*>(Gs) + slot * (GT * 4) + gdst, voff, 0u);
    g_hs += T6_H;
    g_off += 3 * T6_H;
    while (g_hs >= hps) {
      g_hs -= hps;
      g_off += g_tp - Tq;
    }
  };
  auto next6 = [](int v) { return v == NG - 1 ? 0 : v + 1; };

  constexpr bool write_vd = WVD;
  const bool ywave = wave < T6_H;
  const int sw = lane ^ ((wave & 1) << 5);
  int tq = __builtin_amdgcn_readfirstlane((int)((6 * (v_h0 + (ywave ? wave : 0))) % p.Tp));
  const int dstep = __builtin_amdgcn_readfirstlane((6 * T6_H) % p.Tp);
  float bsum = 0.f;
  const int kcd = write_vd ? (p.ld_vd >> 3) : 1;
  const unsigned vd_pstride = (unsigned)(16 * p.ld_vd * 4);
  const long long vd_hexes = ((hexes_all + 1) >> 1) << 1;
  const __amdgpu_buffer_rsrc_t rsVd = __builtin_amdgcn_make_buffer_rsrc(
      write_vd ? (void*)(p.vd + v_h0 * 8 * (long long)p.ld_vd) : (void*)p.slab, 0,
      write_vd ? clip31((vd_hexes - v_h0) * 8 * (long long)p.ld_vd * 4) : 0, 0x00020000);
  const unsigned vdA_lane = (unsigned)(v6_at(0, lane & 3, n0 + (lane & ~3), kcd) * 4);
  const unsigned vdB_lane = vdA_lane + 4u * 64u;
  const int nhex = (int)hexes_all, h_first = (int)v_h0;
  const int h_end = h_first + nsteps * T6_H;
  const int hs_lim = nhex < h_end ? nhex : h_end;
  struct y_in {
    float g[3];
    unsigned long long mo[3], me[3];
    int tq;
  };
  struct y_out {
    float d[6];
  };
  auto uni = [](unsigned long long v) -> unsigned long long {
    return (unsigned long long)(unsigned)__builtin_amdgcn_readfirstlane((int)(unsigned)v) |
           ((unsigned long long)(unsigned)__builtin_amdgcn_readfirstlane((int)(unsigned)(v >> 32)) << 32);
  };
  const int wy = ywave ? wave : 0;
  auto fetch_y = [&](int sd, int slot, y_in& y) {
    const int h = h_first + sd * T6_H + wy;
    const int live = ywave & (h < hs_lim);
    const float* gs = Gs + slot * GT;
    const unsigned long long* ws = reinterpret_cast<const unsigned long long*>(gs + GW) + wy * 4;
#pragma unroll
    for (int r = 0; r < 3; ++r) {
      y.g[r] = gs[wy * 256 + r * 64 + lane];
      const unsigned long long w = uni(ws[r]);
      const int v = live & (tq + 2 * r < p.Tvalid);
      y.mo[r] = v ? w : 0ull;
      y.me[r] = v ? ~w : 0ull;
    }
    y.tq = tq;
    tq += dstep;
    if (tq >= p.Tp) tq -= p.Tp;
  };
  auto compute_y = [&](int sd, const y_in& y) -> y_out {
    y_out u;
#pragma unroll
    for (int r = 0; r < 3; ++r) {
      u.d[2 * r] = selm0(y.me[r], y.g[r]);
      u.d[2 * r + 1] = selm0(y.mo[r], y.g[r]);
    }
    const float ev1 = (u.d[0] + u.d[2]) + u.d[4], od1 = (u.d[1] + u.d[3]) + u.d[5];
    const float ev2 = fmaf(16.f, u.d[4], fmaf(4.f, u.d[2], u.d[0])), od2 = fmaf(32.f, u.d[5], fmaf(8.f, u.d[3], 2.f * u.d[1]));
    const float ev3 = fmaf(0.0625f, u.d[4], fmaf(0.25f, u.d[2], u.d[0])), od3 = fmaf(0.03125f, u.d[5], fmaf(0.125f, u.d[3], 0.5f * u.d[1]));
    float o[8];
    o[0] = u.d[0];
    o[1] = ev1 + od1;
    o[2] = ev1 - od1;
    o[3] = ev2 + od2;
    o[4] = ev2 - od2;
    o[5] = ev3 + od3;
    o[6] = ev3 - od3;
    o[7] = u.d[5];
    bsum += o[1];
    if (ywave) {
      float* dst = Bs + (sd & 1) * T6_TILE + wave * 64 + sw;
#pragma unroll
      for (int i = 0; i < 8; ++i) dst[i * T6_PLANE] = o[i];
    }
    return u;
  };
  typedef unsigned v4u32 __attribute__((ext_vector_type(4)));
  auto vd_part = [&](int sd, int tqc, const y_out& u, float gp, unsigned long long wp) {
    const int h = h_first + sd * T6_H + wy;
    const int vp = ywave & (tqc >= 2) & (tqc - 2 < p.Tvalid) & (h < hs_lim);
    float d[8], v[8];
    d[1] = selm0(vp ? wp : 0ull, gp);
    d[0] = selm0(vp ? ~wp : 0ull, gp);
#pragma unroll
    for (int k = 0; k < 6; ++k) d[2 + k] = u.d[k];
    wino63_bt(d, v);
    const bool odd = lane & 1, hi = lane & 2;
    auto xch = [](float x, auto CTRL) -> float {
      return __builtin_bit_cast(float, __builtin_amdgcn_mov_dpp(__builtin_bit_cast(int, x), decltype(CTRL)::value, 0xf, 0xf, true));
// ... 249 lines not shown
  const int sw = lane ^ ((wave & 1) << 5);
  int tq = __builtin_amdgcn_readfirstlane((int)((6 * (v_h0 + (ywave ? wave : 0))) % p.Tp));
  const int dstep = __builtin_amdgcn_readfirstlane((6 * T6_H) % p.Tp);
  float bsum = 0.f;
  const int kcd = write_vd ? (p.ld_vd >> 3) : 1;
  const unsigned vd_pstride = (unsigned)(16 * p.ld_vd * 4);
  const long long vd_hexes = ((hexes_all + 1) >> 1) << 1;
  const __amdgpu_buffer_rsrc_t rsVd = __builtin_amdgcn_make_buffer_rsrc(
      write_vd ? (void*)(p.vd + v_h0 * 8 * (long long)p.ld_vd) : (void*)p.slab, 0,
      write_vd ? clip31((vd_hexes - v_h0) * 8 * (long long)p.ld_vd * 4) : 0, 0x00020000);
  const unsigned vdA_lane = (unsigned)(v6_at(0, lane & 3, n0 + (lane & ~3), kcd) * 4);
  const unsigned vdB_lane = vdA_lane + 4u * 64u;
  const int nhex = (int)hexes_all, h_first = (int)v_h0;
  const int h_end = h_first + nsteps * T6_H;
  const int hs_lim = nhex < h_end ? nhex : h_end;
  struct y_in {
    float g[3];
    unsigned long long mo[3], me[3];
    int tq;
  };
  struct y_out {
    float d[6];
  };
  auto uni = [](unsigned long long v) -> unsigned long long {
    return (unsigned long long)(unsigned)__builtin_amdgcn_readfirstlane((int)(unsigned)v) |
           ((unsigned long long)(unsigned)__builtin_amdgcn_readfirstlane((int)(unsigned)(v >> 32)) << 32);
  };
  const int wy = ywave ? wave : 0;
  struct y_raw {
    float g[3];
    unsigned long long w[3];
  };
  auto fetch_raw = [&](int slot, y_raw& r) {
    const float* gs = Gs + slot * GT;
    const unsigned long long* ws = reinterpret_cast<const unsigned long long*>(gs + GW) + wy * 4;
#pragma unroll
    for (int q = 0; q < 3; ++q) {
      r.g[q] = gs[wy * 256 + q * 64 + lane];
      r.w[q] = ws[q];
    }
  };
  auto masks_y = [&](int sd, const y_raw& r, y_in& y) {
    const int h = h_first + sd * T6_H + wy;
    const int live = ywave & (h < hs_lim);
#pragma unroll
    for (int q = 0; q < 3; ++q) {
      y.g[q] = r.g[q];
      const unsigned long long w = uni(r.w[q]);
      const int v = live & (tq + 2 * q < p.Tvalid);
      y.mo[q] = v ? w : 0ull;
      y.me[q] = v ? ~w : 0ull;
    }
    y.tq = tq;
    tq += dstep;
    tq -= tq >= p.Tp ? p.Tp : 0;
  };
  auto fetch_y = [&](int sd, int slot, y_in& y) {
    y_raw r;
    fetch_raw(slot, r);
    masks_y(sd, r, y);
  };
  auto compute_y = [&](int sd, const y_in& y) -> y_out {
    y_out u;
#pragma unroll
    for (int r = 0; r < 3; ++r) {
      u.d[2 * r] = selm0(y.me[r], y.g[r]);
      u.d[2 * r + 1] = selm0(y.mo[r], y.g[r]);
    }
    const float ev2 = fmaf(16.f, u.d[4], fmaf(4.f, u.d[2], u.d[0])), od2 = fmaf(32.f, u.d[5], fmaf(8.f, u.d[3], 2.f * u.d[1]));
    float o[4];
    if (th == 0) {
      const float ev1 = (u.d[0] + u.d[2]) + u.d[4], od1 = (u.d[1] + u.d[3]) + u.d[5];
      o[0] = u.d[0];
      o[1] = ev1 + od1;
      o[2] = ev1 - od1;
      o[3] = ev2 + od2;
      bsum += o[1];
    } else {
      const float ev3 = fmaf(0.0625f, u.d[4], fmaf(0.25f, u.d[2], u.d[0])), od3 = fmaf(0.03125f, u.d[5], fmaf(0.125f, u.d[3], 0.5f * u.d[1]));
      o[0] = ev2 - od2;
      o[1] = ev3 + od3;
      o[2] = ev3 - od3;
      o[3] = u.d[5];
    }
    {
      float* dst = (ywave ? Bs + (sd & 1) * QT + wave * 64 : Ydummy + (wave - T6_H) * 64) + sw;
#pragma unroll
      for (int i = 0; i < 4; ++i) dst[i * T6_PLANE] = o[i];
    }
    return u;
  };
  typedef unsigned v4u32 __attribute__((ext_vector_type(4)));
  auto vd_part = [&](int sd, int tqc, const y_out& u, float gp, unsigned long long wp) {
    const int h = h_first + sd * T6_H + wy;
    const int vp = ywave & (tqc >= 2) & (tqc - 2 < p.Tvalid) & (h < hs_lim);
    float d[8], v[8];
    d[1] = selm0(vp ? wp : 0ull, gp);
    d[0] = selm0(vp ? ~wp : 0ull, gp);
#pragma unroll
    for (int k = 0; k < 6; ++k) d[2 + k] = u.d[k];
    wino63_bt(d, v);
    const bool odd = lane & 1, hi = lane & 2;
    auto xch = [](float x, auto CTRL) -> float {
      return __builtin_bit_cast(float, __builtin_amdgcn_mov_dpp(__builtin_bit_cast(int, x), decltype(CTRL)::value, 0xf, 0xf, true));
    };
    using X1 = std::integral_constant<int, 0xB1>;
    using X2 = std::integral_constant<int, 0x4E>;
    auto stage = [&](float& a, float& b, bool up, auto CTRL) {
      const float r = xch(up ? a : b, CTRL);
      a = up ? r : a;
      b = up ? b : r;
    };
#pragma unroll
    for (int g4 = 0; g4 < 8; g4 += 4) {
      stage(v[g4 + 0], v[g4 + 1], odd, X1{});
      stage(v[g4 + 2], v[g4 + 3], odd, X1{});
      stage(v[g4 + 0], v[g4 + 2], hi, X2{});
      stage(v[g4 + 1], v[g4 + 3], hi, X2{});
    }
    const f32x4 va4 = {v[0], v[1], v[2], v[3]};
    const f32x4 vb4 = {v[4], v[5], v[6], v[7]};
    const bool ok = ywave && h < hs_lim;
    const unsigned hoff = (unsigned)((h - h_first) >> 1) * vd_pstride + (unsigned)((h - h_first) & 1) * 32u;
    __builtin_amdgcn_raw_buffer_store_b128(__builtin_bit_cast(v4u32, va4), rsVd, ok ? hoff + vdA_lane : 0xfffffff0u, 0u, 2);
    __builtin_amdgcn_raw_buffer_store_b128(__builtin_bit_cast(v4u32, vb4), rsVd, ok ? hoff + vdB_lane : 0xfffffff0u, 0u, 2);
  };
  auto front_row = [&](int slot, int pslot, float& gp, unsigned long long& wp) {
    const int s_ = wy > 0 ? slot : pslot, hx = wy > 0 ? wy - 1 : T6_H - 1;
    gp = Gs[s_ * GT + hx * 256 + 128 + lane];
    wp = uni(reinterpret_cast<const unsigned long long*>(Gs + s_ * GT + GW)[hx * 4 + 2]);
  };

  const int a_off0 = wm * QT + lh * 64 + (lr ^ (lh << 5)), a_off1 = wm * QT + lh * 64 + ((32 + lr) ^ (lh << 5));
  const int b_off = lh * 64 + ((wn * 32 + lr) ^ (lh << 5));
  float fa0[8], fb0[4], fa1[8], fb1[4], fac[8], fbc[4];
  auto load_frag = [&](float (&fa)[8], float (&fb)[4], int abuf, int bbuf, int sl) {
    const float* a_s = As + abuf * (4 * QT) + sl * 128;
    const float* b_s = Bs + bbuf * QT + sl * 128 + b_off;
#pragma unroll
    for (int t = 0; t < 4; ++t) {
      fa[t] = a_s[a_off0 + t * T6_PLANE];
      fa[4 + t] = a_s[a_off1 + t * T6_PLANE];
      fb[t] = b_s[t * T6_PLANE];
    }
  };
  auto mfma8 = [&](const float (&fa)[8], const float (&fb)[4]) {
#pragma unroll
    for (int i = 0; i < 8; ++i) acc[i] = __builtin_amdgcn_mfma_f32_32x32x2f32(fa[i], fb[i & 3], acc[i], 0, 0, 0);
  };
#pragma unroll
  for (int i = 0; i < 8; ++i) fac[i] = 0.f;
#pragma unroll
  for (int i = 0; i < 4; ++i) fbc[i] = 0.f;

  {
    issue_v(0);
    issue_v(1);
    issue_v(2);
    issue_g(0);
    issue_g(1);
    issue_g(2);
    issue_g(3);
    float gp0 = 0.f;
    unsigned long long wp0 = 0ull;
    if (write_vd && hs0 > 0) {
      const long long pr = g_r0 - 1;
      if (pr < p.B_rows) {
        gp0 = p.B[pr * (long long)p.ldb + n0 + lane];
        const uint32_t* wsrc = p.bbits + pr * (long long)p.ld_bbits + (n0 >> 5);
        wp0 = (unsigned long long)wsrc[0] | ((unsigned long long)wsrc[1] << 32);
      }
    }
    __builtin_amdgcn_s_waitcnt(0x0070);
    __builtin_amdgcn_s_barrier();
    asm volatile("" ::: "memory");
    {
      y_in y0;
      fetch_y(0, 0, y0);
      const y_out u0 = compute_y(0, y0);
      if (write_vd && mi == 0) {
        float gp;
        unsigned long long wp;
        front_row(0, NG - 1, gp, wp);
        if (wave == 0) {
          gp = gp0;
          wp = uni(wp0);
        }
        vd_part(0, y0.tq, u0, gp, wp);
      }
    }
    __builtin_amdgcn_s_waitcnt(0x0070);
    __builtin_amdgcn_s_barrier();
    asm volatile("" ::: "memory");
  }
  int slot1 = 1, slot4 = 4;
  int turn = 1;
  for (int s = 0; s < nsteps; ++s) {
    const int abuf = s & (NA - 1), bbuf = s & 1;
    const int slot0 = slot1 == 0 ? NG - 1 : slot1 - 1;
    __builtin_amdgcn_sched_barrier(0);
    issue_v(s + 3);
    issue_g(slot4);
    y_raw yr;
    fetch_raw(slot1, yr);
    load_frag(fa0, fb0, abuf, bbuf, 0);
    mfma8(fac, fbc);
    load_frag(fa1, fb1, abuf, bbuf, 1);
    mfma8(fa0, fb0);
    __builtin_amdgcn_sched_group_barrier(0x100, 6 + 6, 0);
#pragma unroll
    for (int t = 0; t < 16; ++t) {
      __builtin_amdgcn_sched_group_barrier(0x008, 1, 0);
      if (t < 4) __builtin_amdgcn_sched_group_barrier(0x010, 1, 0);
      if (t >= 4 && t < 10) __builtin_amdgcn_sched_group_barrier(0x100, 1, 0);
    }
    __builtin_amdgcn_sched_barrier(0);
    load_frag(fac, fbc, abuf, bbuf, 2);
    y_in yn;
    y_out un = {};
    masks_y(s + 1, yr, yn);
    un = compute_y(s + 1, yn);
    mfma8(fa1, fb1);
    __builtin_amdgcn_sched_group_barrier(0x100, 6, 0);
#pragma unroll
    for (int t = 0; t < 8; ++t) {
      __builtin_amdgcn_sched_group_barrier(0x008, 1, 0);
      __builtin_amdgcn_sched_group_barrier(0x002, 5, 0);
      if (t >= 6) __builtin_amdgcn_sched_group_barrier(0x200, 2, 0);
    }
    __builtin_amdgcn_sched_barrier(0);
    if constexpr (write_vd) {
      if (ywave && turn == mi && s + 1 < nsteps) {
        float gp;
        unsigned long long wp;
        front_row(slot1, slot0, gp, wp);
        vd_part(s + 1, yn.tq, un, gp, wp);
      }
      turn = turn + 1 == nslots ? 0 : turn + 1;
    }
    __builtin_amdgcn_s_waitcnt(0x0078);
    __builtin_amdgcn_s_barrier();
    asm volatile("" ::: "memory");
    slot1 = next6(slot1);
    slot4 = next6(slot4);
  }
  mfma8(fac, fbc);

  if (p.colsum != nullptr && mi == 0) {
    __syncthreads();
    float* red = lds;
    red[wave * 64 + lane] = ywave ? bsum : 0.f;
    __syncthreads();
    if (tid < 64) {
      float t = 0.f;
#pragma unroll
      for (int q = 0; q < T6_H; ++q) t += red[q * 64 + tid];
      p.colsum[(long long)z * p.Ndim + n0 + tid] = t;
    }
  }
  float* out = p.slab + (long long)z * p.slab_stride;
  const int col = n0 + wn * 32 + lr;
#pragma unroll
  for (int i = 0; i < 8; ++i)
#pragma unroll
    for (int e = 0; e < 16; ++e) {
      const int m = m0 + wm * 64 + (i >> 2) * 32 + (e & 3) + 8 * (e >> 2) + 4 * lh;
      out[((long long)(i0 + (i & 3)) * p.Mdim + m) * (long long)p.ldc + col] = acc[i][e];
    }
}

__global__ __launch_bounds__(256, 4) void wino63_vd_fixup_kernel(float* __restrict__ Vd, const float* __restrict__ halo, long long hexes,
                                                               long long tiles, int hps, int C, int ldv) {
  const int c4n = C >> 2;
  const long long idx = (long long)blockIdx.x * blockDim.x + threadIdx.x;
  if (idx >= tiles * c4n) return;
  const long long t = idx / c4n;
  const int c = (int)(idx - t * c4n) * 4;
  const long long q = t * 256;
  if (q >= hexes) return;
  float* v = Vd + v6_at(q, 0, c, ldv >> 3);
  f32x4 d[8];
#pragma unroll
  for (int j = 2; j < 8; ++j) d[j] = *reinterpret_cast<const f32x4*>(v + 16 * j);
  if (t > 0 && (q % hps) != 0) {
    d[0] = *reinterpret_cast<const f32x4*>(halo + ((t - 1) * 2) * (long long)C + c);
    d[1] = *reinterpret_cast<const f32x4*>(halo + ((t - 1) * 2 + 1) * (long long)C + c);
  } else {
    d[0] = d[1] = f32x4{0.f, 0.f, 0.f, 0.f};
  }
  f32x4 o[8];
#pragma unroll
  for (int k = 0; k < 4; ++k) {
    float dd[8], vv[8];
#pragma unroll
    for (int j = 0; j < 8; ++j) dd[j] = d[j][k];
    wino63_bt(dd, vv);
#pragma unroll
    for (int j = 0; j < 8; ++j) o[j][k] = vv[j];
  }
#pragma unroll
  for (int j = 0; j < 8; ++j) *reinterpret_cast<f32x4*>(v + 16 * j) = o[j];
}

__global__ __launch_bounds__(512, 1) void wino63v_tn4y_kernel(const tl_tn_params p, int mtn) {
  constexpr int NA = 4;
  constexpr int QT = 4 * T6_PLANE;
  __shared__ __attribute__((aligned(1024))) float lds[NA * 4 * QT + NA * QT + 256];
  float* As = lds;
  float* Ys = lds + NA * 4 * QT;
  const int tid = threadIdx.x, lane = tid & 63;
  const int wave = __builtin_amdgcn_readfirstlane(tid >> 6);
  const int wm = wave >> 1, wn = wave & 1, lr = lane & 31, lh = lane >> 5;
  const int ntn = p.Ndim / T6_BN;
  const long long tiles = 2LL * mtn * ntn;
  const long long nwg = tiles * p.splitk;
  long long bid = (long long)blockIdx.y * gridDim.x + blockIdx.x;
  {
    const long long q = nwg / 8, r = nwg % 8, x = bid % 8, i = bid / 8;
    bid = (x < r ? x * (q + 1) : r * (q + 1) + (x - r) * q) + i;
  }
  const int z = __builtin_amdgcn_readfirstlane((int)(bid / tiles));
  const int tt = __builtin_amdgcn_readfirstlane((int)(bid % tiles));
  const int mi = __builtin_amdgcn_readfirstlane(tt % (2 * mtn));
  const int th = mi & 1, i0 = 4 * th;
  const int m0 = (mi >> 1) * 256, n0 = __builtin_amdgcn_readfirstlane((tt / (2 * mtn)) * T6_BN);
  const long long hexes_all = p.Krows / 6;
  const long long ksteps_all = (hexes_all + T6_H - 1) / T6_H;
  const long long per = __builtin_amdgcn_readfirstlane((int)((ksteps_all + p.splitk - 1) / p.splitk));
  const long long ks_begin = z * per;
  long long ks_end = ks_begin + per;
  if (ks_end > ksteps_all) ks_end = ksteps_all;
  const int nsteps = ks_end > ks_begin ? (int)(ks_end - ks_begin) : 0;

  f32x16 acc[8];
#pragma unroll
  for (int i = 0; i < 8; ++i)
#pragma unroll
    for (int e = 0; e < 16; ++e) acc[i][e] = 0.f;

  const long long v_h0 = ks_begin * T6_H;
  const int kc8 = p.lda >> 3, kcy = p.ldb >> 3;
  const __amdgpu_buffer_rsrc_t rsV = __builtin_amdgcn_make_buffer_rsrc(
      (void*)(p.A + v_h0 * 8 * (long long)p.lda), 0, clip31((p.A_rows - v_h0) * 8 * (long long)p.lda * 4), 0x00020000);
  const __amdgpu_buffer_rsrc_t rsY = __builtin_amdgcn_make_buffer_rsrc(
      (void*)(p.B + v_h0 * 8 * (long long)p.ldb), 0, clip31((p.B_rows - v_h0) * 8 * (long long)p.ldb * 4), 0x00020000);
  unsigned vvoff[3], vdst[3];
#pragma unroll
  for (int t = 0; t < 3; ++t) {
    const int quarter = (wave * 3 + t) / 6, pc = (wave * 3 + t) % 6;
    const int rho = 4 * pc + (lane >> 4), i = rho / 6, hx = rho % 6;
    const int chunk = (lane & 15) ^ ((hx & 1) << 3);
    vvoff[t] = (unsigned)(v6_at(hx, i0 + i, m0 + quarter * 64 + chunk * 4, kc8) * 4);
    vdst[t] = (unsigned)((quarter * QT + pc * 256) * 4);
  }
  const bool ypiece = wave < T6_H;
  unsigned yvoff;
  {
    const int rho = 4 * (ypiece ? wave : 0) + (lane >> 4), i = rho / 6, hx = rho % 6;
    const int chunk = (lane & 15) ^ ((hx & 1) << 3);
    yvoff = (unsigned)(v6_at(hx, i0 + i, n0 + chunk * 4, kcy) * 4);
  }
  const unsigned v_step = (unsigned)(T6_H * 8 * p.lda * 4), y_step = (unsigned)(T6_H * 8 * p.ldb * 4);
  auto issue = [&](int step) {
    char* vb = reinterpret_cast<char*>(As) + (step & (NA - 1)) * (4 * QT * 4);
    const unsigned soff = (unsigned)step * v_step;
#pragma unroll
    for (int t = 0; t < 3; ++t) dma16h(rsV, vb + vdst[t], vvoff[t] + soff, 0u);
    char* yb = reinterpret_cast<char*>(Ys) + (ypiece ? ((step & (NA - 1)) * QT + wave * 256) * 4 : NA * QT * 4);
    dma16h(rsY, yb, ypiece ? yvoff + (unsigned)step * y_step : 0xfffffff0u, 0u);
  };
  const int a_off0 = wm * QT + lh * 64 + (lr ^ (lh << 5)), a_off1 = wm * QT + lh * 64 + ((32 + lr) ^ (lh << 5));
  const int b_off = lh * 64 + ((wn * 32 + lr) ^ (lh << 5));
  float fa0[8], fb0[4], fa1[8], fb1[4], fac[8], fbc[4];
  auto load_frag = [&](float (&fa)[8], float (&fb)[4], int buf, int sl) {
    const float* a_s = As + buf * (4 * QT) + sl * 128;
    const float* b_s = Ys + buf * QT + sl * 128 + b_off;
#pragma unroll
    for (int t = 0; t < 4; ++t) {
      fa[t] = a_s[a_off0 + t * T6_PLANE];
      fa[4 + t] = a_s[a_off1 + t * T6_PLANE];
      fb[t] = b_s[t * T6_PLANE];
    }
  };
  auto mfma8 = [&](const float (&fa)[8], const float (&fb)[4]) {
#pragma unroll
    for (int i = 0; i < 8; ++i) acc[i] = __builtin_amdgcn_mfma_f32_32x32x2f32(fa[i], fb[i & 3], acc[i], 0, 0, 0);
  };
#pragma unroll
  for (int i = 0; i < 8; ++i) fac[i] = 0.f;
#pragma unroll
  for (int i = 0; i < 4; ++i) fbc[i] = 0.f;
  const bool summer = p.colsum != nullptr && mi == 0 && wave == 0;
  float bsum = 0.f;
  issue(0);
  issue(1);
  issue(2);
  __builtin_amdgcn_s_waitcnt(0x0078);
  __builtin_amdgcn_s_barrier();
  asm volatile("" ::: "memory");
  for (int s = 0; s < nsteps; ++s) {
    const int buf = s & (NA - 1);
    __builtin_amdgcn_sched_barrier(0);
    issue(s + 3);
    load_frag(fa0, fb0, buf, 0);
    mfma8(fac, fbc);
    load_frag(fa1, fb1, buf, 1);
    mfma8(fa0, fb0);
    load_frag(fac, fbc, buf, 2);
    mfma8(fa1, fb1);
    __builtin_amdgcn_sched_group_barrier(0x100, 6, 0);
#pragma unroll
    for (int t = 0; t < 24; ++t) {
      __builtin_amdgcn_sched_group_barrier(0x008, 1, 0);
      if (t < 4) __builtin_amdgcn_sched_group_barrier(0x010, 1, 0);
      if (t >= 4 && t < 16) __builtin_amdgcn_sched_group_barrier(0x100, 1, 0);
    }
    __builtin_amdgcn_sched_barrier(0);
    if (summer) {
      const float* y1 = Ys + buf * QT + T6_PLANE;
#pragma unroll
      for (int hx = 0; hx < T6_H; ++hx) bsum += y1[hx * 64 + (lane ^ ((hx & 1) << 5))];
    }
    __builtin_amdgcn_s_waitcnt(0x0078);
    __builtin_amdgcn_s_barrier();
    asm volatile("" ::: "memory");
  }
  mfma8(fac, fbc);
  if (summer) p.colsum[(long long)z * p.Ndim + n0 + lane] = bsum;
  float* out = p.slab + (long long)z * p.slab_stride;
  const int col = n0 + wn * 32 + lr;
#pragma unroll
  for (int i = 0; i < 8; ++i)
#pragma unroll
    for (int e = 0; e < 16; ++e) {
      const int m = m0 + wm * 64 + (i >> 2) * 32 + (e & 3) + 8 * (e >> 2) + 4 * lh;
      out[((long long)(i0 + (i & 3)) * p.Mdim + m) * (long long)p.ldc + col] = acc[i][e];
    }
}

__global__ __launch_bounds__(256, 4) void wino63_unpool_yvd_kernel(const float* __restrict__ G, const uint32_t* __restrict__ bits,
                                                                 float* __restrict__ Y, float* __restrict__ Vd, long long nhex,
                                                                 long long g_rows, int hps, int g_tp, int Tvalid, int C, int ldg,
                                                                 int ld_bits, int ldv) {
  const int tpp = C >> 1;
  const long long idx = (long long)blockIdx.x * blockDim.x + threadIdx.x;
  const long long pair = idx / tpp;
  const int tl_ = (int)(idx - pair * tpp);
  const int half = tl_ & 1, hpar = (tl_ >> 1) & 1, kc = tl_ >> 2;
  const int c = 8 * kc + 4 * half;
  const long long hg = 2 * pair + hpar;
  if (hg >= nhex) return;
  const long long seq = hg / hps;
  const int hs = (int)(hg - seq * hps);
  const long long row0 = seq * g_tp + 3LL * hs;
  float dz[8][4];
#pragma unroll
  for (int r = -1; r < 3; ++r) {
    const long long row = row0 + r;
    const bool ok = (r >= 0 || hs > 0) && 6 * hs + 2 * r < Tvalid && row >= 0 && row < g_rows;
    f32x4 g = {0.f, 0.f, 0.f, 0.f};
    uint32_t w = 0;
    if (ok) {
      g = *reinterpret_cast<const f32x4*>(G + row * (long long)ldg + c);
      w = bits[row * (long long)ld_bits + (c >> 5)] >> (c & 31);
    }
#pragma unroll
    for (int k = 0; k < 4; ++k) {
      const bool odd = (w >> k) & 1u;
      dz[2 * (r + 1)][k] = odd ? 0.f : g[k];
      dz[2 * (r + 1) + 1][k] = odd ? g[k] : 0.f;
    }
  }
  f32x4 oy[8], ov[8];
#pragma unroll
  for (int k = 0; k < 4; ++k) {
    float d[8], v[8];
#pragma unroll
    for (int j = 0; j < 8; ++j) d[j] = dz[j][k];
    wino63_bt(d, v);
    const float* d6 = d + 2;
    const float ev1 = (d6[0] + d6[2]) + d6[4], od1 = (d6[1] + d6[3]) + d6[5];
    const float ev2 = fmaf(16.f, d6[4], fmaf(4.f, d6[2], d6[0])), od2 = fmaf(32.f, d6[5], fmaf(8.f, d6[3], 2.f * d6[1]));
    const float ev3 = fmaf(0.0625f, d6[4], fmaf(0.25f, d6[2], d6[0])), od3 = fmaf(0.03125f, d6[5], fmaf(0.125f, d6[3], 0.5f * d6[1]));
    const float y[8] = {d6[0], ev1 + od1, ev1 - od1, ev2 + od2, ev2 - od2, ev3 + od3, ev3 - od3, d6[5]};
#pragma unroll
    for (int j = 0; j < 8; ++j) {
      oy[j][k] = y[j];
      ov[j][k] = v[j];
    }
  }
  const long long at = v6_at(hg, 0, c, ldv >> 3);
#pragma unroll
  for (int j = 0; j < 8; ++j) *reinterpret_cast<f32x4*>(Y + at + 16 * j) = oy[j];
#pragma unroll
  for (int j = 0; j < 8; ++j) *reinterpret_cast<f32x4*>(Vd + at + 16 * j) = ov[j];
}

__global__ __launch_bounds__(256, 4) void wino63_unpool_rows6_kernel(const float* __restrict__ G, const uint32_t* __restrict__ bits,
                                                                   float* __restrict__ A, long long nhex, long long rows,
                                                                   long long g_rows, int Tp, int g_tp, int Tvalid, int C, int ldg,
                                                                   int ld_bits, int lda, int pad) {
  const int tpp = C >> 1;
  const long long idx = (long long)blockIdx.x * blockDim.x + threadIdx.x;
  const long long pair = idx / tpp;
  const int tl_ = (int)(idx - pair * tpp);
  const int half = tl_ & 1, hpar = (tl_ >> 1) & 1, kc = tl_ >> 2;
  const int c = 8 * kc + 4 * half;
  const long long hg = 2 * pair + hpar;
  if (hg >= nhex) return;
  float* dst = A + v6_at(hg, 0, c, lda >> 3);
  const f32x4 zero = {0.f, 0.f, 0.f, 0.f};
#pragma unroll
  for (int i = 0; i < 6; ++i) {
    const long long R = 6 * hg + i;
    f32x4 v = zero;
    if (R < rows) {
      const long long seq = R / Tp;
      const int t = (int)(R - seq * Tp);
      const long long row = seq * g_tp + (t >> 1);
      if (t < Tvalid && row < g_rows) {
        const f32x4 g = *reinterpret_cast<const f32x4*>(G + row * (long long)ldg + c);
        const uint32_t w = bits[row * (long long)ld_bits + (c >> 5)] >> (c & 31);
#pragma unroll
        for (int k = 0; k < 4; ++k) v[k] = (int)((w >> k) & 1u) == (t & 1) ? g[k] : 0.f;
      }
    }
    *reinterpret_cast<f32x4*>(dst + 16 * i) = v;
  }
  if (pad) {
    *reinterpret_cast<f32x4*>(dst + 16 * 6) = zero;
    *reinterpret_cast<f32x4*>(dst + 16 * 7) = zero;
  }
}

__global__ void wino63_weights1_kernel(const float* __restrict__ w, float* __restrict__ out, int O, int I, int ldb) {
  const long long n_all = (long long)ldb * 8 * I;
  const long long idx = (long long)blockIdx.x * blockDim.x + threadIdx.x;
  if (idx >= n_all) return;
  const int k8 = (int)(idx & 7);
  const long long q = idx >> 3;
  const int n = (int)(q % I);
  const long long q2 = q / I;
  const int t = (int)(q2 & 7);
  const int o = (int)(q2 >> 3) * 8 + k8;
  out[idx] = (t < 6 && o < O) ? w[(long long)o * I + n] : 0.f;
}

constexpr int C1_MAXKT = 8;
template <int KT>
__global__ __launch_bounds__(256) void conv1_fwd_vh_kernel(const float* __restrict__ x, const float* __restrict__ w,
                                                           const float* __restrict__ b, float* __restrict__ P,
                                                           float* __restrict__ V, uint32_t* __restrict__ bits,
                                                           uint32_t* __restrict__ sign, long long S, int T, int C1,
                                                           int Tp, int Tout, float slope) {
  constexpr int kt = KT;
  extern __shared__ __attribute__((aligned(16))) float xs[];
  const long long seq = blockIdx.x;
  for (int i = threadIdx.x; i < T; i += blockDim.x) xs[i] = x[seq * T + i];
  __syncthreads();
  const int tpp = C1 >> 1;
  const int ppp = 256 / tpp;
  const int tl_ = threadIdx.x % tpp, psub = threadIdx.x / tpp;
  const int half = tl_ & 1, hpar = (tl_ >> 1) & 1, kc = tl_ >> 2;
  const int o = 8 * kc + 4 * half;
  float wv[4][KT], bv[4];
#pragma unroll
  for (int c = 0; c < 4; ++c) {
    bv[c] = b[o + c];
#pragma unroll
    for (int j = 0; j < KT; ++j) wv[c][j] = w[(o + c) * kt + j];
  }
  const int sh = 4 * (2 * (kc & 3) + half);
  const int Th = Tp / 6;
  auto row = [&](int pr, bool live, f32x4& out, uint32_t& wb, uint32_t& ws) {
    out = f32x4{0.f, 0.f, 0.f, 0.f};
    uint32_t nib = 0, nsg = 0;
    if (live && pr < Tout) {
#pragma unroll
      for (int c = 0; c < 4; ++c) {
        float z0 = 0.f, z1 = 0.f;
#pragma unroll
        for (int jj = 0; jj < KT; ++jj) {
          z0 = fmaf(wv[c][jj], xs[2 * pr + jj], z0);
          z1 = fmaf(wv[c][jj], xs[2 * pr + 1 + jj], z1);
        }
        const float y0 = lrelu(z0 + bv[c], slope), y1 = lrelu(z1 + bv[c], slope);
        const bool sel = y1 > y0;
        const float v = sel ? y1 : y0;
        out[c] = v;
        nib |= (sel ? 1u : 0u) << c;
        nsg |= (v > 0.f ? 1u : 0u) << c;
      }
    }
    auto or8 = [](uint32_t v) {
      v |= (uint32_t)__builtin_amdgcn_update_dpp(0, (int)v, 0xB1, 0xf, 0xf, false);
      v |= (uint32_t)__builtin_amdgcn_update_dpp(0, (int)v, 0x124, 0xf, 0xf, false);
      v |= (uint32_t)__builtin_amdgcn_update_dpp(0, (int)v, 0x128, 0xf, 0xf, false);
      return v;
    };
    wb = or8(nib << sh);
    ws = or8(nsg << sh);
  };
  const long long h0 = seq * Th;
  const int q0 = (int)((hpar - h0) & 1) + 2 * psub;
  const int trips = (Th + 2 * ppp - 1) / (2 * ppp) + 1;
  const bool word_writer = sh == 0;
  for (int i = 0; i < trips; ++i) {
    const int q = q0 + 2 * ppp * i;
    const bool live = q < Th;
    f32x4 d[8];
    uint32_t wb[8], ws[8];
#pragma unroll
    for (int j = 0; j < 8; ++j) row(6 * q + j, live && 6 * q + j < Tp, d[j], wb[j], ws[j]);
    if (live) {
      const long long row0 = seq * Tp + 6 * q;
#pragma unroll
      for (int j = 0; j < 6; ++j) {
        if (P != nullptr) *reinterpret_cast<f32x4*>(P + (row0 + j) * C1 + o) = d[j];
        if (word_writer) {
          bits[(row0 + j) * (C1 >> 5) + (o >> 5)] = wb[j];
          if (sign != nullptr) sign[(row0 + j) * (C1 >> 5) + (o >> 5)] = ws[j];
        }
      }
      f32x4 ov[8];
#pragma unroll
      for (int k = 0; k < 4; ++k) {
        float dd[8], vv[8];
#pragma unroll
        for (int j = 0; j < 8; ++j) dd[j] = d[j][k];
        wino63_bt(dd, vv);
#pragma unroll
        for (int j = 0; j < 8; ++j) ov[j][k] = vv[j];
      }
      float* dst = V + v6_at(h0 + q, 0, o, C1 >> 3);
#pragma unroll
      for (int j = 0; j < 8; ++j) *reinterpret_cast<f32x4*>(dst + 16 * j) = ov[j];
    }
  }
}

}

extern "C" int tl_wino63_weights(const float* w, float* fwd, float* dgr, int O, int I, int ld_f, int ld_d, void* stream) {
  using namespace tl;
  TL_REQUIRE(w != nullptr && (fwd != nullptr || dgr != nullptr), "wino63_weights: null pointer");
  TL_REQUIRE(O > 0 && I > 0, "wino63_weights: bad sizes");
  TL_REQUIRE((fwd == nullptr || (ld_f >= I && ld_f % 8 == 0)) && (dgr == nullptr || (ld_d >= O && ld_d % 8 == 0)),
             "wino63_weights: leading dimensions must cover the reduction length and be multiples of 8");
  const long long nf = (long long)O * ld_f, nd = (long long)I * ld_d;
  const long long n = nf > nd ? nf : nd;
  TL_REQUIRE((n + 255) / 256 < (1LL << 31), "wino63_weights: too large");
  hipLaunchKernelGGL(wino63_weights_kernel, dim3((unsigned)((n + 255) / 256)), dim3(256), 0, (hipStream_t)stream, w, fwd, dgr, O,
                     I, ld_f, ld_d);
  return check_launch("wino63_weights");
}

extern "C" int tl_wino63_wgrad_finalize(const float* red, float* gw, int O, int I, int ld, void* stream) {
  using namespace tl;
  TL_REQUIRE(red && gw && O > 0 && I > 0 && ld >= O, "wino63_wgrad_finalize: bad arguments");
  const long long n = (long long)O * I;
  hipLaunchKernelGGL(wino63_wgrad_finalize_kernel, dim3((unsigned)((n + 255) / 256)), dim3(256), 0, (hipStream_t)stream, red, gw,
                     O, I, ld);
  return check_launch("wino63_wgrad_finalize");
}

extern "C" int tl_wino63_v_fixup(float* V, const float* vhalo, int64_t hexes, int64_t tiles, int Tq, int C, int ldv, void* stream) {
  using namespace tl;
  TL_REQUIRE(V && vhalo, "wino63_v_fixup: null pointer");
  TL_REQUIRE(hexes > 0 && tiles > 0 && Tq > 0 && Tq % 6 == 0, "wino63_v_fixup: hexes, tiles > 0 and Tq %% 6 == 0 needed");
  TL_REQUIRE(C > 0 && C % 4 == 0 && ldv >= C && ldv % 8 == 0, "wino63_v_fixup: C %% 4 and ldv %% 8 needed");
  const long long n = (long long)tiles * (C / 4);
  TL_REQUIRE((n + 255) / 256 < (1LL << 31), "wino63_v_fixup: grid too large");
  hipLaunchKernelGGL(wino63_v_fixup_kernel, dim3((unsigned)((n + 255) / 256)), dim3(256), 0, (hipStream_t)stream, V, vhalo,
                     (long long)hexes, (long long)tiles, Tq, C, ldv);
  return check_launch("wino63_v_fixup");
}

extern "C" int tl_wino63_vd_fixup(float* Vd, const float* vhalo, int64_t hexes, int64_t tiles, int hexes_per_seq, int C, int ldv,
                                  void* stream) {
  using namespace tl;
  TL_REQUIRE(Vd && vhalo, "wino63_vd_fixup: null pointer");
  TL_REQUIRE(hexes > 0 && tiles > 0 && hexes_per_seq > 0, "wino63_vd_fixup: hexes, tiles, hexes per sequence > 0 needed");
  TL_REQUIRE(C > 0 && C % 4 == 0 && ldv >= C && ldv % 8 == 0, "wino63_vd_fixup: C %% 4 and ldv %% 8 needed");
  const long long n = (long long)tiles * (C / 4);
  TL_REQUIRE((n + 255) / 256 < (1LL << 31), "wino63_vd_fixup: grid too large");
  hipLaunchKernelGGL(wino63_vd_fixup_kernel, dim3((unsigned)((n + 255) / 256)), dim3(256), 0, (hipStream_t)stream, Vd, vhalo,
                     (long long)hexes, (long long)tiles, hexes_per_seq, C, ldv);
  return check_launch("wino63_vd_fixup");
}

extern "C" int tl_wino63_unpool_yvd(const float* G, const uint32_t* bits, float* Y, float* Vd, int64_t conv_rows, int64_t g_rows,
                                    int Tp, int g_tp, int Tvalid, int C, int ldg, int ld_bits, int ldv, void* stream) {
  using namespace tl;
  TL_REQUIRE(G && bits && Y && Vd, "wino63_unpool_yvd: null pointer");
  TL_REQUIRE(Tp > 0 && Tp % 6 == 0 && conv_rows > 0 && conv_rows % Tp == 0 && Tvalid % 2 == 0 && Tvalid <= Tp,
             "wino63_unpool_yvd: Tp %% 6 == 0, whole sequences, an even Tvalid <= Tp needed");
  TL_REQUIRE(g_tp > 0 && 2 * g_tp >= Tvalid && g_rows >= (conv_rows / Tp) * (long long)g_tp, "wino63_unpool_yvd: G holds fewer rows than sequences x g_tp");
  TL_REQUIRE(C > 0 && C % 8 == 0 && ldg >= C && ldg % 4 == 0 && ldv >= C && ldv % 8 == 0 && ld_bits * 32 >= C,
             "wino63_unpool_yvd: C %% 8, ldg %% 4, ldv %% 8 needed, bits row must cover C");
  const long long nhex = conv_rows / 6;
  const long long n = ((nhex + 1) / 2) * (C / 2);
  TL_REQUIRE((n + 255) / 256 < (1LL << 31), "wino63_unpool_yvd: grid too large");
  hipLaunchKernelGGL(wino63_unpool_yvd_kernel, dim3((unsigned)((n + 255) / 256)), dim3(256), 0, (hipStream_t)stream, G, bits, Y, Vd,
                     nhex, (long long)g_rows, Tp / 6, g_tp, Tvalid, C, ldg, ld_bits, ldv);
  return check_launch("wino63_unpool_yvd");
}

extern "C" int tl_wino63_weights7(const float* w, float* fwd, int O, int I, int taps, void* stream) {
  using namespace tl;
  TL_REQUIRE(w && fwd && O > 0 && I > 0 && I % 8 == 0 && taps >= 7 && taps <= 9, "wino63_weights7: I %% 8 == 0 and 7..9 taps needed");
  const long long n = 3LL * O * I;
  TL_REQUIRE((n + 255) / 256 < (1LL << 31), "wino63_weights7: grid too large");
  hipLaunchKernelGGL(wino63_weights7_kernel, dim3((unsigned)((n + 255) / 256)), dim3(256), 0, (hipStream_t)stream, w, fwd, O, I, taps);
  return check_launch("wino63_weights7");
}

extern "C" int tl_wino63_xform2(const float* P, float* V0, float* V1, int64_t rows, int Tp, int Tvalid, int C, int ldp, int ldv,
                                void* stream) {
  using namespace tl;
  TL_REQUIRE(P && V0 && V1, "wino63_xform2: null pointer");
  TL_REQUIRE(Tp > 0 && Tp % 6 == 0 && rows > 0 && rows % Tp == 0 && Tvalid >= 0 && Tvalid <= Tp, "wino63_xform2: Tp %% 6 == 0, whole sequences, Tvalid <= Tp needed");
  TL_REQUIRE(C > 0 && C % 8 == 0 && ldp >= C && ldp % 4 == 0 && ldv >= C && ldv % 8 == 0, "wino63_xform2: C %% 8, ldp %% 4, ldv %% 8 needed");
  const long long nhex = rows / 6;
  const long long n = ((nhex + 1) / 2) * (C / 2);
  TL_REQUIRE((n + 255) / 256 < (1LL << 31), "wino63_xform2: grid too large");
  hipLaunchKernelGGL(wino63_xform2_kernel, dim3((unsigned)((n + 255) / 256)), dim3(256), 0, (hipStream_t)stream, P, V0, V1, nhex,
                     Tp / 6, Tp, Tvalid, C, ldp, ldv);
  return check_launch("wino63_xform2");
}

extern "C" int tl_conv7_wino63v_nt(const tl_nt_params* pp, void* stream) {
  using namespace tl;
  TL_REQUIRE(pp != nullptr, "conv7_wino63: null params");
  const tl_nt_params& p = *pp;
  TL_REQUIRE(p.A && p.aux && p.Bw && p.out, "conv7_wino63: null V0 (A) / V1 (aux) / Bw / out");
  TL_REQUIRE(p.loader == W_LOAD_V && p.epilogue == W_EPI_LRELU && p.row_shift == 0 && p.splitk <= 1,
             "conv7_wino63: loader 2 (pre-transformed operands), LRELU epilogue, row_shift 0, no split-K");
  TL_REQUIRE(p.J >= 7 && p.J <= 9, "conv7_wino63: 7..9 taps (three segments)");
  TL_REQUIRE(p.M > 0 && p.M % 6 == 0 && p.N > 0 && p.N % 32 == 0 && p.K >= 16 && p.K % 8 == 0, "conv7_wino63: M %% 6, N %% 32, K %% 8, K >= 16 needed");
  TL_REQUIRE(p.lda >= p.K && p.lda % 8 == 0 && p.ldb >= 3 * p.K && p.ldb % 8 == 0 && p.ldo >= p.N, "conv7_wino63: bad leading dimensions");
  TL_REQUIRE(p.A_rows % 2 == 0 && p.Tp > 0 && p.Tp % 6 == 0 && p.M % p.Tp == 0, "conv7_wino63: V holds hex pairs; Tp %% 6, whole sequences");
  TL_REQUIRE(8LL * p.N * p.ldb * 4 < (1LL << 31), "conv7_wino63: tap set larger than a buffer resource");
  TL_REQUIRE(128LL * 8 * p.lda * 4 + 4LL * p.K < (1LL << 31) && p.M + V6_ROWS < (1LL << 31), "conv7_wino63: tile span / M too large");
  TL_REQUIRE(p.slope >= 0.f && p.slope <= 1.f, "conv7_wino63: LeakyReLU slope must lie in [0, 1]");
  const long long ntm = (p.M + V6_ROWS - 1) / V6_ROWS;
  const long long nwg = ntm * ((p.N + V6_BN - 1) / V6_BN);
  TL_REQUIRE(nwg < (1LL << 31), "conv7_wino63: grid too large");
  TL_REQUIRE(p.A_rows >= ntm * V6_BH, "conv7_wino63: V0 / V1 must hold whole 128-hex tiles (pad them with zero hexes)");
  const long long ngrid = nwg < 256 ? nwg : 256;
  hipLaunchKernelGGL((wino63v_nt_kernel<W_EPI_LRELU>), dim3((unsigned)ngrid), dim3(512), 0, (hipStream_t)stream, p);
  return check_launch("conv7_wino63");
}

extern "C" int tl_wino63_nt_tile_rows(void) { return tl::V6_ROWS; }

extern "C" int tl_conv3_wino63v_nt(const tl_nt_params* pp, void* stream) {
  using namespace tl;
  TL_REQUIRE(pp != nullptr, "wino63v_nt: null params");
  const tl_nt_params& p = *pp;
  TL_REQUIRE(p.A && p.Bw && (p.out || p.epilogue == W_EPI_C1W || p.epilogue == W_EPI_POOLV || p.epilogue == W_EPI_MASKY), "wino63v_nt: null V/Bw/out");
  TL_REQUIRE(p.loader == W_LOAD_V, "wino63v_nt: loader 2 (pre-transformed operand) only");
  TL_REQUIRE(p.J == 3 && p.splitk <= 1, "wino63v_nt: 3 taps, no split-K");
  TL_REQUIRE(p.M > 0 && p.M % 6 == 0 && p.N > 0 && p.K >= 40 && p.K % 8 == 0, "wino63v_nt: M %% 6, K %% 8, K >= 40 needed");
  TL_REQUIRE(p.lda >= p.K && p.ldb >= p.K && p.lda % 8 == 0 && p.ldb % 8 == 0, "wino63v_nt: bad leading dimensions (multiples of 8)");
  TL_REQUIRE(p.A_rows % 2 == 0, "wino63v_nt: V holds hex pairs");
  TL_REQUIRE(p.Tp > 0 && p.Tp % 6 == 0 && p.M % p.Tp == 0, "wino63v_nt: Tp must be a positive multiple of 6, M whole sequences");
  TL_REQUIRE(8LL * p.N * p.ldb * 4 < (1LL << 31), "wino63v_nt: tap set larger than a buffer resource");
  TL_REQUIRE(128LL * 8 * p.lda * 4 + 4LL * p.K < (1LL << 31), "wino63v_nt: tile span too large");
  const long long ntm = (p.M + V6_ROWS - 1) / V6_ROWS;
  const long long nwg = ntm * ((p.N + V6_BN - 1) / V6_BN);
  TL_REQUIRE(nwg < (1LL << 31), "wino63v_nt: grid too large");
  TL_REQUIRE(p.N % 32 == 0 && p.M + V6_ROWS < (1LL << 31), "wino63v_nt: N %% 32 == 0 and M < 2^31 - 768 needed");
  TL_REQUIRE(p.slope >= 0.f && p.slope <= 1.f, "wino63v_nt: LeakyReLU slope must lie in [0, 1]");
  TL_REQUIRE(p.A_rows >= ntm * V6_BH, "wino63v_nt: V must hold whole 128-hex tiles (pad it with zero hexes)");
  hipStream_t st = (hipStream_t)stream;
  const long long ngrid = nwg < 256 ? nwg : 256;
  if (p.epilogue == W_EPI_POOL) {
    TL_REQUIRE(p.row_shift == 0 && p.out && p.ldo >= p.N, "wino63v_nt: forward needs row_shift 0 and an output");
    TL_REQUIRE(p.obits != nullptr && p.Tvalid % 2 == 0 && p.Tvalid <= p.Tp, "wino63v_nt: POOL needs obits and an even Tvalid");
    TL_REQUIRE(p.ld_obits * 32 >= p.N, "wino63v_nt: POOL: ld_obits too small");
    TL_REQUIRE(p.out_tp >= 0 && (p.out_tp == 0 || 2 * p.out_tp >= p.Tvalid), "wino63v_nt: out_tp must cover the valid pooled rows");
    const long long orows = (p.M / p.Tp) * (long long)(p.out_tp > 0 ? p.out_tp : p.Tp / 2);
    TL_REQUIRE(orows * (long long)p.ldo * 4 < (1LL << 40), "wino63v_nt: output too large");
    hipLaunchKernelGGL((wino63v_nt_kernel<W_EPI_POOL>), dim3((unsigned)ngrid), dim3(512), 0, st, p);
  } else if (p.epilogue == W_EPI_POOLV) {
    TL_REQUIRE(p.row_shift == 0 && (p.out == nullptr || p.ldo >= p.N), "wino63v_nt: forward needs row_shift 0");
    TL_REQUIRE(p.obits != nullptr && p.Tvalid % 2 == 0 && p.Tvalid <= p.Tp, "wino63v_nt: POOLV needs obits and an even Tvalid");
    TL_REQUIRE(p.ld_obits * 32 >= p.N && p.Tp % 12 == 0, "wino63v_nt: POOLV needs Tp %% 12 == 0 (output hexes inside one sequence)");
    TL_REQUIRE(p.vout && p.vhalo && p.ld_vout >= p.N && p.ld_vout % 8 == 0 && p.vout_quads >= p.M / 12 && p.vout_quads % 2 == 0,
               "wino63v_nt: POOLV needs vout (>= M / 12 hexes, whole pairs, ld_vout %% 8 == 0) and vhalo");
    TL_REQUIRE(64LL * 8 * p.ld_vout * 4 < (1LL << 31), "wino63v_nt: ld_vout too large");
    hipLaunchKernelGGL((wino63v_nt_kernel<W_EPI_POOLV>), dim3((unsigned)ngrid), dim3(512), 0, st, p);
  } else if (p.epilogue == W_EPI_MASK) {
    TL_REQUIRE(p.row_shift == -2 && p.ldo >= p.N, "wino63v_nt: input gradient needs row_shift -2");
    TL_REQUIRE(p.auxbits != nullptr, "wino63v_nt: MASK needs auxbits (the sign bits of the stage input)");
    hipLaunchKernelGGL((wino63v_nt_kernel<W_EPI_MASK>), dim3((unsigned)ngrid), dim3(512), 0, st, p);
  } else if (p.epilogue == W_EPI_MASKY) {
    TL_REQUIRE(p.row_shift == -2 && p.auxbits != nullptr && p.abits != nullptr, "wino63v_nt: epilogue 6 needs row_shift -2, auxbits and abits");
    TL_REQUIRE(p.ld_abits * 32 >= p.N && p.Tvalid_in % 2 == 0 && p.Tvalid_in <= 2 * p.Tp, "wino63v_nt: epilogue 6: bad abits / Tvalid_in");
    TL_REQUIRE(p.vout && p.vout2 && p.vhalo && p.ld_vout >= p.N && p.ld_vout % 8 == 0 && p.vout_quads >= p.M / 3 && p.vout_quads % 2 == 0,
               "wino63v_nt: epilogue 6 needs vout / vout2 (>= M / 3 hexes, whole pairs, ld_vout %% 8 == 0) and vhalo");
    TL_REQUIRE(128LL * 8 * p.ld_vout * 4 < (1LL << 31), "wino63v_nt: ld_vout too large");
    hipLaunchKernelGGL((wino63v_nt_kernel<W_EPI_MASKY>), dim3((unsigned)ngrid), dim3(512), 0, st, p);
  } else if (p.epilogue == W_EPI_C1W) {
    TL_REQUIRE(p.row_shift == -2, "wino63v_nt: input gradient needs row_shift -2");
    TL_REQUIRE(p.auxbits && p.c1x && p.c1bits && p.c1partial, "wino63v_nt: epilogue 4 needs auxbits, c1x, c1bits, c1partial");
    TL_REQUIRE(p.c1kt >= 1 && p.c1kt <= 3 && p.c1T >= 2 * p.Tvalid + 2, "wino63v_nt: epilogue 4: 1..3 taps, c1T >= 2*Tvalid + 2");
    hipLaunchKernelGGL((wino63v_nt_kernel<W_EPI_C1W>), dim3((unsigned)ngrid), dim3(512), 0, st, p);
  } else {
    set_error("wino63v_nt: unsupported epilogue %d", p.epilogue);
    return TL_EINVAL;
  }
  return check_launch("wino63v_nt");
}

extern "C" int tl_wino63_unpool_rows6(const float* G, const uint32_t* bits, float* A, int64_t rows, int64_t g_rows, int Tp, int g_tp,
                                      int Tvalid, int C, int ldg, int ld_bits, int lda, int pad, void* stream) {
  using namespace tl;
  TL_REQUIRE(G && bits && A, "wino63_unpool_rows6: null pointer");
  TL_REQUIRE(rows > 0 && Tp > 0 && rows % Tp == 0 && Tvalid > 0 && Tvalid <= Tp, "wino63_unpool_rows6: whole sequences of Tp rows, 0 < Tvalid <= Tp needed");
  TL_REQUIRE(g_tp > 0 && 2 * g_tp >= Tvalid && g_rows >= (rows / Tp) * (long long)g_tp, "wino63_unpool_rows6: G holds fewer rows than sequences x g_tp");
  TL_REQUIRE(C > 0 && C % 8 == 0 && ldg >= C && ldg % 4 == 0 && lda >= C && lda % 8 == 0 && ld_bits * 32 >= C,
             "wino63_unpool_rows6: C %% 8, ldg %% 4, lda %% 8 needed, bits row must cover C");
  const long long nhex = (rows + 5) / 6;
  const long long n = (nhex + 1) / 2 * (C >> 1);
  TL_REQUIRE((n + 255) / 256 < (1LL << 31), "wino63_unpool_rows6: grid too large");
  hipLaunchKernelGGL(wino63_unpool_rows6_kernel, dim3((unsigned)((n + 255) / 256)), dim3(256), 0, (hipStream_t)stream, G, bits, A,
                     nhex, (long long)rows, (long long)g_rows, Tp, g_tp, Tvalid, C, ldg, ld_bits, lda, pad);
  return check_launch("wino63_unpool_rows6");
}

extern "C" int tl_wino63_weights1(const float* w, float* taps, int O, int I, int ldb, void* stream) {
  using namespace tl;
  TL_REQUIRE(w && taps && O > 0 && I > 0 && ldb >= O && ldb % 8 == 0, "wino63_weights1: w, taps, O, I > 0 and ldb %% 8 == 0, ldb >= O needed");
  const long long n = (long long)ldb * 8 * I;
  TL_REQUIRE((n + 255) / 256 < (1LL << 31), "wino63_weights1: too large");
  hipLaunchKernelGGL(wino63_weights1_kernel, dim3((unsigned)((n + 255) / 256)), dim3(256), 0, (hipStream_t)stream, w, taps, O, I, ldb);
  return check_launch("wino63_weights1");
}

extern "C" int tl_conv1_wino63v_dgrad_nt(const tl_nt_params* pp, void* stream) {
  using namespace tl;
  TL_REQUIRE(pp != nullptr, "conv1_wino63v_dgrad_nt: null params");
  const tl_nt_params& p = *pp;
  TL_REQUIRE(p.A && p.Bw, "conv1_wino63v_dgrad_nt: null A / taps");
  TL_REQUIRE(p.loader == W_LOAD_V && p.epilogue == W_EPI_GY && p.J == 1 && p.row_shift == 0 && p.splitk <= 1,
             "conv1_wino63v_dgrad_nt: loader 2, epilogue 7, one tap, row_shift 0, no split-K");
  TL_REQUIRE(p.M > 0 && p.N > 0 && p.K >= 40 && p.K % 8 == 0, "conv1_wino63v_dgrad_nt: K %% 8, K >= 40 needed");
  TL_REQUIRE(p.Tp > 0 && p.Tp % 3 == 0 && p.M % p.Tp == 0, "conv1_wino63v_dgrad_nt: Tp (rows per sequence) must be a multiple of 3, M whole sequences");
  TL_REQUIRE(p.lda >= p.K && p.ldb >= p.K && p.lda % 8 == 0 && p.ldb % 8 == 0, "conv1_wino63v_dgrad_nt: bad leading dimensions (multiples of 8)");
  TL_REQUIRE(p.A_rows % 2 == 0, "conv1_wino63v_dgrad_nt: A holds hex pairs");
  TL_REQUIRE(8LL * p.N * p.ldb * 4 < (1LL << 31), "conv1_wino63v_dgrad_nt: tap set larger than a buffer resource");
  TL_REQUIRE(128LL * 8 * p.lda * 4 + 4LL * p.K < (1LL << 31), "conv1_wino63v_dgrad_nt: tile span too large");
  const long long ntm = (p.M + V6_ROWS - 1) / V6_ROWS;
  const long long nwg = ntm * ((p.N + V6_BN - 1) / V6_BN);
  TL_REQUIRE(nwg < (1LL << 31), "conv1_wino63v_dgrad_nt: grid too large");
  TL_REQUIRE(p.N % 32 == 0 && p.M + V6_ROWS < (1LL << 31), "conv1_wino63v_dgrad_nt: N %% 32 == 0 and M < 2^31 - 768 needed");
  TL_REQUIRE(p.slope >= 0.f && p.slope <= 1.f, "conv1_wino63v_dgrad_nt: LeakyReLU slope must lie in [0, 1]");
  TL_REQUIRE(p.A_rows >= ntm * V6_BH, "conv1_wino63v_dgrad_nt: A must hold whole 128-hex tiles (pad it with zero hexes)");
  TL_REQUIRE(p.auxbits != nullptr && p.abits != nullptr, "conv1_wino63v_dgrad_nt: needs auxbits (sign) and abits (arg-max) of the stage below");
  TL_REQUIRE(p.out_tp > 0 && p.out_tp <= p.Tp && 2 * p.out_tp >= p.Tvalid_in, "conv1_wino63v_dgrad_nt: out_tp = rows per sequence of the bit arrays (0 < out_tp <= Tp, covering Tvalid_in / 2)");
  TL_REQUIRE(p.ld_abits * 32 >= p.N && p.ld_auxbits * 32 >= p.N && p.Tvalid_in % 2 == 0 && p.Tvalid_in <= 2 * p.Tp, "conv1_wino63v_dgrad_nt: bad abits / auxbits / Tvalid_in");
  TL_REQUIRE(p.vout && p.vout2 && p.vhalo && p.ld_vout >= p.N && p.ld_vout % 8 == 0 && p.vout_quads >= p.M / 3 && p.vout_quads % 2 == 0,
             "conv1_wino63v_dgrad_nt: needs vout / vout2 (>= M / 3 hexes, whole pairs, ld_vout %% 8 == 0) and vhalo");
  TL_REQUIRE(128LL * 8 * p.ld_vout * 4 < (1LL << 31), "conv1_wino63v_dgrad_nt: ld_vout too large");
  const long long ngrid = nwg < 256 ? nwg : 256;
  hipLaunchKernelGGL((wino63v_nt_kernel<W_EPI_GY>), dim3((unsigned)ngrid), dim3(512), 0, (hipStream_t)stream, p);
  return check_launch("conv1_wino63v_dgrad_nt");
}

extern "C" int tl_conv3_wino63v_tn(const tl_tn_params* pp, void* stream) {
  using namespace tl;
  TL_REQUIRE(pp != nullptr, "wino63v_tn: null params");
  tl_tn_params p = *pp;
  if (p.splitk < 1) p.splitk = 1;
  if (p.loader == 3) {
    TL_REQUIRE(p.A && p.B && p.slab, "wino63v_tn: null V/Y/slab");
    TL_REQUIRE(p.J == 3 && p.Tp > 0 && p.Tp % 6 == 0 && p.Krows > 0 && p.Krows % p.Tp == 0, "wino63v_tn: loader 3: bad Tp / Krows");
    TL_REQUIRE(p.Krows + 64 < (1LL << 31), "wino63v_tn: more than 2^31 reduction rows");
    TL_REQUIRE(p.Mdim % 256 == 0 && p.Ndim % 64 == 0 && p.lda % 8 == 0 && p.ldb % 8 == 0 && p.lda >= p.Mdim && p.ldb >= p.Ndim &&
               p.ldc >= p.Ndim, "wino63v_tn: loader 3 needs Mdim %% 256, Ndim %% 64, lda / ldb %% 8");
    TL_REQUIRE(p.A_rows % 2 == 0 && p.B_rows % 2 == 0 && p.vd == nullptr, "wino63v_tn: loader 3: whole hex pairs in V and Y, no Vd");
    TL_REQUIRE(p.splitk <= 65535 && (p.splitk == 1 || p.slab_stride >= 8LL * p.Mdim * p.ldc), "wino63v_tn: bad splitk / slab_stride");
    const long long ks = (p.Krows / 6 + T6_H - 1) / T6_H;
    TL_REQUIRE(p.A_rows >= ks * T6_H && p.B_rows >= ks * T6_H, "wino63v_tn: V and Y must hold whole 6-hex K-steps (pad with zero hexes)");
    const long long per3 = (ks + p.splitk - 1) / p.splitk;
    TL_REQUIRE((per3 + 4) * (long long)T6_H * 8 * p.lda * 4 < (1LL << 31) && (per3 + 4) * (long long)T6_H * 8 * p.ldb * 4 < (1LL << 31),
               "wino63v_tn: a reduction split spans more than 2 GB of V or Y: raise splitk");
    const int ntm3 = p.Mdim / 256;
    hipLaunchKernelGGL(wino63v_tn4y_kernel, dim3((unsigned)(2 * ntm3 * (p.Ndim / T6_BN)), (unsigned)p.splitk, 1), dim3(512), 0,
                       (hipStream_t)stream, p, ntm3);
    return check_launch("wino63v_tn (both operands pre-transformed)");
  }
  TL_REQUIRE(p.A && p.B && p.slab && p.bbits, "wino63v_tn: null V/B/bbits/slab");
  TL_REQUIRE(p.J == 3 && p.loader == 1, "wino63v_tn: 3 taps, UNPOOL loader (1) or pre-transformed Y (3)");
  TL_REQUIRE(p.Tp > 0 && p.Tp % 6 == 0 && p.Tvalid % 2 == 0 && p.Tvalid <= p.Tp, "wino63v_tn: Tp %% 6 == 0 and an even Tvalid <= Tp needed");
  TL_REQUIRE(p.Krows > 0 && p.Krows % p.Tp == 0 && p.Mdim > 0 && p.Ndim > 0, "wino63v_tn: bad sizes (Krows must be whole sequences)");
  TL_REQUIRE(p.Krows + 64 < (1LL << 31), "wino63v_tn: more than 2^31 reduction rows");
  TL_REQUIRE(p.Mdim % 128 == 0 && p.Ndim % 64 == 0 && p.lda % 8 == 0 && p.ldb % 4 == 0 && p.A_rows % 2 == 0,
             "wino63v_tn: Mdim %% 128, Ndim %% 64, lda %% 8, ldb %% 4, whole hex pairs in V needed");
  TL_REQUIRE(p.lda >= p.Mdim && p.ldb >= p.Ndim && p.ldc >= p.Ndim, "wino63v_tn: leading dimension too small");
  TL_REQUIRE(p.ld_bbits * 32 >= p.Ndim && p.ld_bbits % 2 == 0, "wino63v_tn: bbits row too short / odd");
  TL_REQUIRE(p.splitk <= 65535, "wino63v_tn: splitk too large");
  TL_REQUIRE(p.splitk == 1 || p.slab_stride >= 8LL * p.Mdim * p.ldc, "wino63v_tn: slab_stride smaller than 8*Mdim*ldc");
  const int g_tp = p.g_tp > 0 ? p.g_tp : p.Tp / 2;
  TL_REQUIRE(2 * g_tp >= p.Tvalid, "wino63v_tn: g_tp must cover the valid pooled rows");
  TL_REQUIRE(p.B_rows >= (p.Krows / p.Tp) * (long long)g_tp && p.B_rows < (1LL << 30), "wino63v_tn: G holds fewer rows than sequences x g_tp");
  const long long ksteps_all = (p.Krows / 6 + T6_H - 1) / T6_H;
  TL_REQUIRE(p.A_rows >= (ksteps_all + 3) * T6_H, "wino63v_tn: V must hold whole 6-hex K-steps and three more (pad it with zero hexes)");
  const long long per = (ksteps_all + p.splitk - 1) / p.splitk;
  TL_REQUIRE((per + 4) * (long long)T6_H * 8 * p.lda * 4 < (1LL << 31), "wino63v_tn: a reduction split spans more than 2 GB of V: raise splitk");
  TL_REQUIRE((per + 6) * 3LL * T6_H * p.ldb * 4 < (1LL << 31), "wino63v_tn: a reduction split spans more than 2 GB of G: raise splitk");
  TL_REQUIRE(p.vd == nullptr || (p.ld_vd >= p.Ndim && p.ld_vd % 8 == 0), "wino63v_tn: ld_vd must cover Ndim (multiple of 8)");
  TL_REQUIRE(p.vd == nullptr || (per + 4) * (long long)T6_H * 8 * p.ld_vd * 4 < (1LL << 31), "wino63v_tn: a reduction split spans more than 2 GB of Vd: raise splitk");
  const int ntn = p.Ndim / T6_BN;
  hipStream_t st = (hipStream_t)stream;
  TL_REQUIRE(p.bm == 0 || p.bm == 128 || (p.bm == 256 && p.Mdim % 256 == 0 && p.Tp >= 12),
             "wino63v_tn: bm must be 0, 128, or 256 with Mdim %% 256 == 0 and Tp >= 12");
  if (p.bm == 256 || (p.bm == 0 && p.Mdim % 256 == 0 && p.Tp >= 12)) {
    const int ntm = p.Mdim / 256;
    const dim3 grid((unsigned)(2 * ntm * ntn), (unsigned)p.splitk, 1);
    if (p.vd != nullptr) hipLaunchKernelGGL((wino63v_tn4_kernel<true>), grid, dim3(512), 0, st, p, ntm);
    else hipLaunchKernelGGL((wino63v_tn4_kernel<false>), grid, dim3(512), 0, st, p, ntm);
    return check_launch("wino63v_tn (4 transforms per workgroup)");
  }
  const int ntm = p.Mdim / 128;
  const dim3 grid((unsigned)(ntm * ntn), (unsigned)p.splitk, 1);
  if (p.vd != nullptr) hipLaunchKernelGGL((wino63v_tn_kernel<true>), grid, dim3(512), 0, st, p, ntm);
  else hipLaunchKernelGGL((wino63v_tn_kernel<false>), grid, dim3(512), 0, st, p, ntm);
  return check_launch("wino63v_tn");
}

extern "C" int tl_conv1_fwd_v6(const float* x, const float* w, const float* b, float* P, float* V, uint32_t* bits, uint32_t* sign,
                               int64_t S, int T, int ktaps, int C1, int Tp, int Tout, float slope, void* stream) {
  using namespace tl;
  TL_REQUIRE(x && w && b && V && bits, "conv1_fwd_v6: null pointer");
  TL_REQUIRE(S > 0 && S < (1LL << 31) && T > 0, "conv1_fwd_v6: bad sizes");
  TL_REQUIRE(ktaps >= 1 && ktaps <= C1_MAXKT, "conv1_fwd_v6: ktaps must be 1..%d", C1_MAXKT);
  TL_REQUIRE(C1 % 128 == 0 && C1 <= 1024 && (C1 & (C1 - 1)) == 0, "conv1_fwd_v6: C1 must be 128, 256, 512 or 1024");
  TL_REQUIRE(Tp > 0 && Tp % 6 == 0, "conv1_fwd_v6: Tp must be a multiple of 6");
  TL_REQUIRE(Tout >= 0 && Tout <= Tp && 2 * Tout + ktaps - 1 <= T, "conv1_fwd_v6: Tout/Tp/T inconsistent (%d,%d,%d)", Tout, Tp, T);
  TL_REQUIRE((size_t)T * 4 <= 64 * 1024, "conv1_fwd_v6: T too large for the LDS window");
#define TL_C1V_LAUNCH(KT_)                                                                                                   \
  case KT_:                                                                                                                  \
    hipLaunchKernelGGL(conv1_fwd_vh_kernel<KT_>, dim3((unsigned)S), dim3(256), (size_t)T * 4, (hipStream_t)stream, x, w, b, P, V, \
                       bits, sign, (long long)S, T, C1, Tp, Tout, slope);                                                    \
    break;
  switch (ktaps) {
    TL_C1V_LAUNCH(1) TL_C1V_LAUNCH(2) TL_C1V_LAUNCH(3) TL_C1V_LAUNCH(4) TL_C1V_LAUNCH(5) TL_C1V_LAUNCH(6) TL_C1V_LAUNCH(7)
    TL_C1V_LAUNCH(8)
  }
#undef TL_C1V_LAUNCH
  return check_launch("conv1_fwd_v6");
}
```

Before: 1263 mel-frames/s.

## Skip dead Winograd hexes in conv3 forward and pre-transformed weight gradients

New measurement: 1272 mel-frames/s, median of 6. Within noise of the previous version (+0.7%).

```diff
diff --git a/decode_tonal_langauge_amd/_classifier_engine.py b/decode_tonal_langauge_amd/_classifier_engine.py
--- a/decode_tonal_langauge_amd/_classifier_engine.py
+++ b/decode_tonal_langauge_amd/_classifier_engine.py
@@ -29,7 +29,7 @@
 
     def _plan63(self, stage_defs, T):
         from . import _kernels
-        if _kernels.get("wino") != "6":
+        if _kernels.get("wino") not in ("6", "6k"):
             return 0, []
         c1, k1, p1 = stage_defs[0]
         if not (p1 and 1 <= k1 <= 3 and c1 in (128, 256, 512, 1024) and T >= 2 * self.tout1 + 2 and T * 4 <= 64 * 1024):
@@ -81,6 +81,8 @@
                       ld_obits=st.cout // 32, Tvalid=2 * st.tout)
             if last:
                 dst = self.P[st.idx]
+                if _kernels.get("wino") == "6k":
+                    kw.update(bm=-1)
                 self._nt(fn="tl_conv3_wino63v_nt", out=ptr(dst), ldo=dst.shape[1], epilogue=EPI_POOL, out_tp=st.tp_out, **kw)
             else:
                 rows_out = S * (tp_in // 2)
diff --git a/decode_tonal_langauge_amd/_cnn_engine.py b/decode_tonal_langauge_amd/_cnn_engine.py
--- a/decode_tonal_langauge_amd/_cnn_engine.py
+++ b/decode_tonal_langauge_amd/_cnn_engine.py
@@ -24,6 +24,15 @@
         self.tc = tin - k + 1
         self.tout = self.tc // 2 if pool else self.tc
         self.tp_out = tp_in // 2 if pool else tp_in
+
+
+def f63_live_hexes(tp: int, tvalid: int, keep: bool = False) -> int:
+    hps, live = tp // 6, (tvalid + 5) // 6
+    return hps if (keep or tvalid <= 0 or live >= hps or live < 6) else live
+
+
+def f63_stored_hex(c: int, tp: int, live: int) -> int:
+    return (c // live) * (tp // 6) + c % live
 
 
 class CnnEngine:
@@ -53,7 +62,7 @@
         align = 1 << npool_after
         self.tp1 = max(align, (self.tout1 + align - 1) // align * align)
         _kernels.validate()
-        self.wino63 = (self.F63_CAPABLE and _kernels.get("wino") == "6"
+        self.wino63 = (self.F63_CAPABLE and _kernels.get("wino") in ("6", "6k")
                        and self._f63_covers(stage_defs, n_timepoints))
         tp1_default = self.tp1
         if self.wino63:
@@ -61,6 +70,7 @@
         self.f63_yprod = (self.wino63 and _kernels.get("f63_yprod") != "0" and stage_defs[0][0] % 256 == 0
                           and self.tp1 >= 12)
         self.f63_yprod3 = (self.wino63 and _kernels.get("f63_yprod") != "0" and stage_defs[1][0] % 256 == 0)
+        self.f63_keep = _kernels.get("wino") == "6k"
         self.stages: List[_Stage] = []
         cin, tin, tp = self.c1, self.tout1, self.tp1
         for i, (cout, k, pool) in enumerate(stage_defs[1:], start=2):
@@ -273,8 +283,21 @@
                                          self._stream()), "tl_wino63_weights")
         return dst
 
+    def _f63_live(self, st) -> int:
+        return f63_live_hexes(st.tp_in, 2 * st.tout, self.f63_keep)
+
+    def _f63_fwd_skips(self, st) -> bool:
+        return st.idx != 2
+
+    def f63_fwd_issue_factor(self, st) -> float:
+        hexes = self._f63_live(st) if self._f63_fwd_skips(st) else st.tp_in // 6
+        return hexes * 8.0 / (st.tc * 3.0)
+
+    def f63_dgrad_issue_factor(self, st) -> float:
+        return (st.tp_in // 6) * 8.0 / (st.tc * 3.0)
+
     def f63_issue_factor(self, st) -> float:
-        return (st.tp_in // 6) * 8.0 / (st.tc * 3.0)
+        return 0.5 * (self.f63_fwd_issue_factor(st) + self.f63_dgrad_issue_factor(st))
 
     def _stage_forward63(self, st, w, bia) -> None:
         S = self.S
@@ -301,6 +324,8 @@
             if Pout is None:
                 raise RuntimeError("F(6,3) stage 3 writes pooled rows: its output buffer was not allocated")
             kw.update(epilogue=EPI_POOL, out_tp=st.tp_out)
+            if self.f63_keep:
+                kw.update(bm=-1)
             self._nt(tag="conv3_fwd", fn="tl_conv3_wino63v_nt", **kw)
 
     def _stage_wgrad63(self, st, gw, gb) -> None:
@@ -311,7 +336,9 @@
         ldg = nd
         V = self._v_ready[st.idx - 1]
         tiles = (st.cin // 64) * (nd // 64)
-        sk = self._splitk(tiles, (rows_in + 35) // 36, 4096)
+        yready = self._y_ready.get(st.idx) == self.generation or (st.idx == 3 and self.f63_yprod3)
+        rows_red = S * 6 * self._f63_live(st) if yready else rows_in
+        sk = self._splitk(tiles, (rows_red + 35) // 36, 4096)
         slab = torch.empty(sk, 8 * st.cin, ldg, **f32)
         bias_part = torch.empty(sk, nd, **f32)
         if (st.idx == 3 and self.f63_yprod3 and self._y_ready.get(3) != self.generation):
@@ -332,7 +359,7 @@
             self._tn(tag=f"conv{st.idx}_wgrad", fn="tl_conv3_wino63v_tn", A=ptr(V), B=ptr(Y), slab=ptr(slab), Krows=rows_in,
                      A_rows=V.shape[0], B_rows=Y.shape[0], Mdim=st.cin, Ndim=nd, lda=V.shape[2], ldb=Y.shape[2], ldc=ldg, J=3,
                      Tp=st.tp_in, splitk=sk, slab_stride=8 * st.cin * ldg, loader=LOAD_Y, Tvalid=2 * st.tout,
-                     colsum=ptr(bias_part))
+                     colsum=ptr(bias_part), bm=-1 if self.f63_keep else 0)
         else:
             Gs = self.G[st.idx]
             Vd = self._v_hex_buffer(self.Vd, st.idx, rows_in, nd)
@@ -481,7 +508,8 @@
 
     def wgrad_issue_factor(self, st) -> float:
         if self._f63(st):
-            return self.f63_issue_factor(st)
+            yprod = self.f63_yprod if st.idx == 2 else self.f63_yprod3
+            return (self._f63_live(st) if yprod else st.tp_in // 6) * 8.0 / (st.tc * 3.0)
         return 0.5 if self._v43(st) else 1.0
 
     def kernel_families(self):
@@ -508,7 +536,11 @@
             else:
                 fams[f"wino63v_nt_kernel<MASK> (conv3 input gradient, {f6})"] = ["conv3_dgrad"]
                 fams[f"{tn2} (conv2 weight gradient, {f6}; also writes Vd)"] = ["conv2_wgrad"]
-            issued = {k: self.f63_issue_factor(st2 if "conv2" in k else st3) for k in fams}
+            issued = {}
+            for k, tags in fams.items():
+                st = st2 if tags[0].startswith("conv2") else st3
+                issued[k] = (self.wgrad_issue_factor(st) if tags[0].endswith("_wgrad") else
+                             self.f63_fwd_issue_factor(st) if tags[0].endswith("_fwd") else self.f63_dgrad_issue_factor(st))
             return fams, issued
         self._fam_share = {}
         if not all(self._v43(st) for st in self.stages[:2]):
diff --git a/decode_tonal_langauge_amd/_kernels.py b/decode_tonal_langauge_amd/_kernels.py
--- a/decode_tonal_langauge_amd/_kernels.py
+++ b/decode_tonal_langauge_amd/_kernels.py
@@ -17,9 +17,11 @@
 
 _B = frozenset({"0", "1"})
 KEYS: Dict[str, Tuple[str, _Allowed, str, str]] = {
-    "wino": ("TONAL_WINO", frozenset({"6", "4", "0"}), "6",
+    "wino": ("TONAL_WINO", frozenset({"6", "6k", "4", "0"}), "6",
              "conv2 / conv3: 6 Winograd F(6,3) on pre-transformed operands (F(4,3) V form where the stack does not allow it), "
-             "4 the F(4,3) V form, 0 direct MFMA kernels (also the fallback for every shape neither form covers)"),
+             "4 the F(4,3) V form, 0 direct MFMA kernels (also the fallback for every shape neither form covers); 6k = 6 with the "
+             "dead hexes kept: conv3 forward and the transform-free weight gradients visit every hex of a sequence, not only those "
+             "that hold a valid conv row (the parity partner and same-build A/B of the dead-hex skip)"),
     "f63_yprod": ("TONAL_F63_YPROD", _B, "1", "F(6,3): the backward operands Y / Vd of stages 2 and 3 come pre-transformed out of the "
                                               "input-gradient epilogue of the stage above (0: the weight-gradient kernels un-pool and "
                                               "transform the gradient rows themselves)"),
diff --git a/decode_tonal_langauge_amd/csrc/tonal_wino63.hip b/decode_tonal_langauge_amd/csrc/tonal_wino63.hip
--- a/decode_tonal_langauge_amd/csrc/tonal_wino63.hip
+++ b/decode_tonal_langauge_amd/csrc/tonal_wino63.hip
@@ -21,6 +21,11 @@
 
 __device__ __forceinline__ long long v6_at(long long hex, int i, int c, int kc8) {
   return ((((hex >> 1) * kc8 + (c >> 3)) * 8 + i) * 2 + (hex & 1)) * 8 + (c & 7);
+}
+
+__host__ __device__ inline int v6_live_hexes(int Tp, int Tvalid, int bm) {
+  const int hps = Tp / 6, live = (Tvalid + 5) / 6;
+  return (bm == -1 || Tvalid <= 0 || live >= hps || live < 6) ? 0 : live;
 }
 
 __global__ void wino63_weights_kernel(const float* __restrict__ w, float* __restrict__ fwd, float* __restrict__ dgr, int O,
@@ -185,7 +190,17 @@
 constexpr int V6_ROWS = 6 * V6_BH;
 
 template <int EPI>
-__global__ __launch_bounds__(512, 2) void wino63v_nt_kernel(const tl_nt_params p) {
+__global__ __launch_bounds__(512, 2) void wino63v_nt_kernel(const tl_nt_params p_in, const int live) {
+  constexpr bool SKIP = EPI == W_EPI_POOL;
+  tl_nt_params p = p_in;
+  const int hps = p_in.Tp / 6;
+  if constexpr (SKIP) {
+    if (live > 0) {
+      p.out_tp = p_in.out_tp > 0 ? p_in.out_tp : p_in.Tp >> 1;
+      p.Tp = 6 * live;
+      p.M = (p_in.M / p_in.Tp) * p.Tp;
+    }
+  }
   __shared__ __attribute__((aligned(1024))) char lds[3 * V6_STAGE + ((EPI == W_EPI_POOLV || EPI == W_EPI_MASKY || EPI == W_EPI_GY) ? 4096 : EPI == W_EPI_C1W ? 16384 : 0)];
   const int tid = threadIdx.x;
   const int lane = tid & 63;
@@ -226,13 +241,28 @@
     int n0;
     v6_i32x4 rsA, rsA1;
     unsigned bvoff[2];
+    unsigned av[4];
   };
   const long long a_tile_bytes = (long long)V6_BH * 8 * p.lda * 4, a_total_bytes = p.A_rows * 8LL * p.lda * 4;
   auto place = [&](tile_t& t, long long tm, int tn) {
     t.tm = tm;
     t.R0 = tm * V6_ROWS;
     t.n0 = tn * V6_BN;
-    const long long ab = tm * a_tile_bytes;
+    long long ab = tm * a_tile_bytes;
+#pragma unroll
+    for (int k = 0; k < 4; ++k) t.av[k] = avoff[k];
+    if constexpr (SKIP) {
+      if (live > 0) {
+        const unsigned c0 = (unsigned)tm * (unsigned)V6_BH, s0 = c0 / (unsigned)live;
+        const unsigned base = (s0 * (unsigned)hps + (c0 - s0 * (unsigned)live)) & ~1u;
+        ab = (long long)base * 8 * p.lda * 4;
+#pragma unroll
+        for (int k = 0; k < 4; ++k) {
+          const unsigned c = c0 + (unsigned)(k * 32 + hex_of_row), sq = c / (unsigned)live;
+          t.av[k] = (unsigned)(v6_at((long long)(sq * (unsigned)hps + (c - sq * (unsigned)live) - base), wave, src_chunk * 4, kc8) * 4);
+        }
+      }
+    }
     t.rsA = v6_rsrc_words(reinterpret_cast<const char*>(p.A) + ab, (SIX && wave >= 6) ? 0 : a_total_bytes - ab);
     t.rsA1 = SEG3 ? v6_rsrc_words(reinterpret_cast<const char*>(p.aux) + ab, a_total_bytes - ab) : t.rsA;
     if (t.n0 + V6_BN <= p.N) {
@@ -292,7 +322,7 @@
     } else {
       d.ra = t.rsA;
 #pragma unroll
-      for (int k = 0; k < 4; ++k) d.va[k] = avoff[k];
+      for (int k = 0; k < 4; ++k) d.va[k] = SKIP ? t.av[k] : avoff[k];
     }
     d.vb[0] = t.bvoff[0];
     d.vb[1] = t.bvoff[1];
@@ -1148,7 +1178,7 @@
   for (int j = 0; j < 8; ++j) *reinterpret_cast<f32x4*>(v + 16 * j) = o[j];
 }
 
-__global__ __launch_bounds__(512, 1) void wino63v_tn4y_kernel(const tl_tn_params p, int mtn) {
+__global__ __launch_bounds__(512, 1) void wino63v_tn4y_kernel(const tl_tn_params p, int mtn, const int live) {
   constexpr int NA = 4;
   constexpr int QT = 4 * T6_PLANE;
   __shared__ __attribute__((aligned(1024))) float lds[NA * 4 * QT + NA * QT + 256];
@@ -1170,7 +1200,9 @@
   const int mi = __builtin_amdgcn_readfirstlane(tt % (2 * mtn));
   const int th = mi & 1, i0 = 4 * th;
   const int m0 = (mi >> 1) * 256, n0 = __builtin_amdgcn_readfirstlane((tt / (2 * mtn)) * T6_BN);
-  const long long hexes_all = p.Krows / 6;
+  const int hps = p.Tp / 6;
+  const int gap = live > 0 ? hps - live : 0;
+  const long long hexes_all = live > 0 ? (p.Krows / p.Tp) * live : p.Krows / 6;
   const long long ksteps_all = (hexes_all + T6_H - 1) / T6_H;
   const long long per = __builtin_amdgcn_readfirstlane((int)((ksteps_all + p.splitk - 1) / p.splitk));
   const long long ks_begin = z * per;
@@ -1185,35 +1217,66 @@
     for (int e = 0; e < 16; ++e) acc[i][e] = 0.f;
 
   const long long v_h0 = ks_begin * T6_H;
+  long long st0 = v_h0;
+  int left0 = 0x3fffffff;
+  if (live > 0) {
+    const long long sq = v_h0 / live;
+    const int hs = (int)(v_h0 - sq * live);
+    st0 = sq * hps + hs;
+    left0 = live - hs;
+  }
+  const long long base = st0 & ~1LL;
   const int kc8 = p.lda >> 3, kcy = p.ldb >> 3;
   const __amdgpu_buffer_rsrc_t rsV = __builtin_amdgcn_make_buffer_rsrc(
-      (void*)(p.A + v_h0 * 8 * (long long)p.lda), 0, clip31((p.A_rows - v_h0) * 8 * (long long)p.lda * 4), 0x00020000);
+      (void*)(p.A + base * 8 * (long long)p.lda), 0, clip31((p.A_rows - base) * 8 * (long long)p.lda * 4), 0x00020000);
   const __amdgpu_buffer_rsrc_t rsY = __builtin_amdgcn_make_buffer_rsrc(
-      (void*)(p.B + v_h0 * 8 * (long long)p.ldb), 0, clip31((p.B_rows - v_h0) * 8 * (long long)p.ldb * 4), 0x00020000);
-  unsigned vvoff[3], vdst[3];
-#pragma unroll
-  for (int t = 0; t < 3; ++t) {
-    const int quarter = (wave * 3 + t) / 6, pc = (wave * 3 + t) % 6;
+      (void*)(p.B + base * 8 * (long long)p.ldb), 0, clip31((p.B_rows - base) * 8 * (long long)p.ldb * 4), 0x00020000);
+  const unsigned hv = (unsigned)(8 * p.lda * 4), hy = (unsigned)(8 * p.ldb * 4);
+  const bool ypiece = wave < T6_H;
+  unsigned cst[4][4], nw[4][2], vdst[3];
+  int hxq[4];
+#pragma unroll
+  for (int q = 0; q < 4; ++q) {
+    const int pcq = q < 3 ? wave * 3 + q : 6 * 0 + (ypiece ? wave : 0);
+    const int pc = q < 3 ? pcq % 6 : pcq;
     const int rho = 4 * pc + (lane >> 4), i = rho / 6, hx = rho % 6;
     const int chunk = (lane & 15) ^ ((hx & 1) << 3);
-    vvoff[t] = (unsigned)(v6_at(hx, i0 + i, m0 + quarter * 64 + chunk * 4, kc8) * 4);
-    vdst[t] = (unsigned)((quarter * QT + pc * 256) * 4);
-  }
-  const bool ypiece = wave < T6_H;
-  unsigned yvoff;
-  {
-    const int rho = 4 * (ypiece ? wave : 0) + (lane >> 4), i = rho / 6, hx = rho % 6;
-    const int chunk = (lane & 15) ^ ((hx & 1) << 3);
-    yvoff = (unsigned)(v6_at(hx, i0 + i, n0 + chunk * 4, kcy) * 4);
-  }
-  const unsigned v_step = (unsigned)(T6_H * 8 * p.lda * 4), y_step = (unsigned)(T6_H * 8 * p.ldb * 4);
+    const unsigned hb = q < 3 ? hv : hy;
+    const unsigned lane_c = (unsigned)(v6_at(0, i0 + i, q < 3 ? m0 + (pcq / 6) * 64 + chunk * 4 : n0 + chunk * 4, q < 3 ? kc8 : kcy) * 4);
+    hxq[q] = hx;
+#pragma unroll
+    for (int w = 0; w < 2; ++w)
+#pragma unroll
+      for (int e = 0; e < 2; ++e) {
+        const unsigned k = (unsigned)(hx + w * gap);
+        cst[q][2 * w + e] = lane_c + k * hb + (((unsigned)e + k) & 1u) * (32u - hb);
+      }
+    if (q < 3) vdst[q] = (unsigned)(((pcq / 6) * QT + pc * 256) * 4);
+  }
+  int sE = __builtin_amdgcn_readfirstlane((int)(st0 - base)), left = __builtin_amdgcn_readfirstlane(left0);
+  auto select = [&] {
+    const bool odd = sE & 1;
+#pragma unroll
+    for (int q = 0; q < 4; ++q) {
+      nw[q][0] = odd ? cst[q][1] : cst[q][0];
+      nw[q][1] = odd ? cst[q][3] : cst[q][2];
+    }
+  };
+  select();
   auto issue = [&](int step) {
     char* vb = reinterpret_cast<char*>(As) + (step & (NA - 1)) * (4 * QT * 4);
-    const unsigned soff = (unsigned)step * v_step;
-#pragma unroll
-    for (int t = 0; t < 3; ++t) dma16h(rsV, vb + vdst[t], vvoff[t] + soff, 0u);
+    const unsigned sv = (unsigned)sE * hv, sy = (unsigned)sE * hy;
+#pragma unroll
+    for (int t = 0; t < 3; ++t) dma16h(rsV, vb + vdst[t], (hxq[t] >= left ? nw[t][1] : nw[t][0]) + sv, 0u);
     char* yb = reinterpret_cast<char*>(Ys) + (ypiece ? ((step & (NA - 1)) * QT + wave * 256) * 4 : NA * QT * 4);
-    dma16h(rsY, yb, ypiece ? yvoff + (unsigned)step * y_step : 0xfffffff0u, 0u);
+    dma16h(rsY, yb, ypiece ? (hxq[3] >= left ? nw[3][1] : nw[3][0]) + sy : 0xfffffff0u, 0u);
+  };
+  auto advance = [&]() -> bool {
+    const bool wrap = left <= T6_H;
+    left += wrap ? live - T6_H : -T6_H;
+    const int add = wrap ? T6_H + gap : T6_H;
+    sE += add;
+    return add & 1;
   };
   const int a_off0 = wm * QT + lh * 64 + (lr ^ (lh << 5)), a_off1 = wm * QT + lh * 64 + ((32 + lr) ^ (lh << 5));
   const int b_off = lh * 64 + ((wn * 32 + lr) ^ (lh << 5));
@@ -1238,9 +1301,11 @@
   for (int i = 0; i < 4; ++i) fbc[i] = 0.f;
   const bool summer = p.colsum != nullptr && mi == 0 && wave == 0;
   float bsum = 0.f;
-  issue(0);
-  issue(1);
-  issue(2);
+#pragma unroll
+  for (int s = 0; s < 3; ++s) {
+    issue(s);
+    if (advance()) select();
+  }
   __builtin_amdgcn_s_waitcnt(0x0078);
   __builtin_amdgcn_s_barrier();
   asm volatile("" ::: "memory");
@@ -1267,6 +1332,7 @@
 #pragma unroll
       for (int hx = 0; hx < T6_H; ++hx) bsum += y1[hx * 64 + (lane ^ ((hx & 1) << 5))];
     }
+    if (advance()) select();
     __builtin_amdgcn_s_waitcnt(0x0078);
     __builtin_amdgcn_s_barrier();
     asm volatile("" ::: "memory");
@@ -1594,7 +1660,7 @@
   TL_REQUIRE(nwg < (1LL << 31), "conv7_wino63: grid too large");
   TL_REQUIRE(p.A_rows >= ntm * V6_BH, "conv7_wino63: V0 / V1 must hold whole 128-hex tiles (pad them with zero hexes)");
   const long long ngrid = nwg < 256 ? nwg : 256;
-  hipLaunchKernelGGL((wino63v_nt_kernel<W_EPI_LRELU>), dim3((unsigned)ngrid), dim3(512), 0, (hipStream_t)stream, p);
+  hipLaunchKernelGGL((wino63v_nt_kernel<W_EPI_LRELU>), dim3((unsigned)ngrid), dim3(512), 0, (hipStream_t)stream, p, 0);
   return check_launch("conv7_wino63");
 }
 
@@ -1628,7 +1694,17 @@
     TL_REQUIRE(p.out_tp >= 0 && (p.out_tp == 0 || 2 * p.out_tp >= p.Tvalid), "wino63v_nt: out_tp must cover the valid pooled rows");
     const long long orows = (p.M / p.Tp) * (long long)(p.out_tp > 0 ? p.out_tp : p.Tp / 2);
     TL_REQUIRE(orows * (long long)p.ldo * 4 < (1LL << 40), "wino63v_nt: output too large");
-    hipLaunchKernelGGL((wino63v_nt_kernel<W_EPI_POOL>), dim3((unsigned)ngrid), dim3(512), 0, st, p);
+    int live = v6_live_hexes(p.Tp, p.Tvalid, p.bm);
+    long long lgrid = ngrid;
+    if (live > 0) {
+      const long long hps = p.Tp / 6, span = V6_BH + (V6_BH / live + 2) * (hps - live) + 2;
+      if (span * 8 * p.lda * 4 + 4LL * p.K >= (1LL << 31)) live = 0;
+    }
+    if (live > 0) {
+      const long long ntm_l = ((p.M / p.Tp) * 6 * live + V6_ROWS - 1) / V6_ROWS, nwg_l = ntm_l * ((p.N + V6_BN - 1) / V6_BN);
+      lgrid = nwg_l < 256 ? nwg_l : 256;
+    }
+    hipLaunchKernelGGL((wino63v_nt_kernel<W_EPI_POOL>), dim3((unsigned)lgrid), dim3(512), 0, st, p, live);
   } else if (p.epilogue == W_EPI_POOLV) {
     TL_REQUIRE(p.row_shift == 0 && (p.out == nullptr || p.ldo >= p.N), "wino63v_nt: forward needs row_shift 0");
     TL_REQUIRE(p.obits != nullptr && p.Tvalid % 2 == 0 && p.Tvalid <= p.Tp, "wino63v_nt: POOLV needs obits and an even Tvalid");
@@ -1636,23 +1712,23 @@
     TL_REQUIRE(p.vout && p.vhalo && p.ld_vout >= p.N && p.ld_vout % 8 == 0 && p.vout_quads >= p.M / 12 && p.vout_quads % 2 == 0,
                "wino63v_nt: POOLV needs vout (>= M / 12 hexes, whole pairs, ld_vout %% 8 == 0) and vhalo");
     TL_REQUIRE(64LL * 8 * p.ld_vout * 4 < (1LL << 31), "wino63v_nt: ld_vout too large");
-    hipLaunchKernelGGL((wino63v_nt_kernel<W_EPI_POOLV>), dim3((unsigned)ngrid), dim3(512), 0, st, p);
+    hipLaunchKernelGGL((wino63v_nt_kernel<W_EPI_POOLV>), dim3((unsigned)ngrid), dim3(512), 0, st, p, 0);
   } else if (p.epilogue == W_EPI_MASK) {
     TL_REQUIRE(p.row_shift == -2 && p.ldo >= p.N, "wino63v_nt: input gradient needs row_shift -2");
     TL_REQUIRE(p.auxbits != nullptr, "wino63v_nt: MASK needs auxbits (the sign bits of the stage input)");
-    hipLaunchKernelGGL((wino63v_nt_kernel<W_EPI_MASK>), dim3((unsigned)ngrid), dim3(512), 0, st, p);
+    hipLaunchKernelGGL((wino63v_nt_kernel<W_EPI_MASK>), dim3((unsigned)ngrid), dim3(512), 0, st, p, 0);
   } else if (p.epilogue == W_EPI_MASKY) {
     TL_REQUIRE(p.row_shift == -2 && p.auxbits != nullptr && p.abits != nullptr, "wino63v_nt: epilogue 6 needs row_shift -2, auxbits and abits");
     TL_REQUIRE(p.ld_abits * 32 >= p.N && p.Tvalid_in % 2 == 0 && p.Tvalid_in <= 2 * p.Tp, "wino63v_nt: epilogue 6: bad abits / Tvalid_in");
     TL_REQUIRE(p.vout && p.vout2 && p.vhalo && p.ld_vout >= p.N && p.ld_vout % 8 == 0 && p.vout_quads >= p.M / 3 && p.vout_quads % 2 == 0,
                "wino63v_nt: epilogue 6 needs vout / vout2 (>= M / 3 hexes, whole pairs, ld_vout %% 8 == 0) and vhalo");
     TL_REQUIRE(128LL * 8 * p.ld_vout * 4 < (1LL << 31), "wino63v_nt: ld_vout too large");
-    hipLaunchKernelGGL((wino63v_nt_kernel<W_EPI_MASKY>), dim3((unsigned)ngrid), dim3(512), 0, st, p);
+    hipLaunchKernelGGL((wino63v_nt_kernel<W_EPI_MASKY>), dim3((unsigned)ngrid), dim3(512), 0, st, p, 0);
   } else if (p.epilogue == W_EPI_C1W) {
     TL_REQUIRE(p.row_shift == -2, "wino63v_nt: input gradient needs row_shift -2");
     TL_REQUIRE(p.auxbits && p.c1x && p.c1bits && p.c1partial, "wino63v_nt: epilogue 4 needs auxbits, c1x, c1bits, c1partial");
     TL_REQUIRE(p.c1kt >= 1 && p.c1kt <= 3 && p.c1T >= 2 * p.Tvalid + 2, "wino63v_nt: epilogue 4: 1..3 taps, c1T >= 2*Tvalid + 2");
-    hipLaunchKernelGGL((wino63v_nt_kernel<W_EPI_C1W>), dim3((unsigned)ngrid), dim3(512), 0, st, p);
+    hipLaunchKernelGGL((wino63v_nt_kernel<W_EPI_C1W>), dim3((unsigned)ngrid), dim3(512), 0, st, p, 0);
   } else {
     set_error("wino63v_nt: unsupported epilogue %d", p.epilogue);
     return TL_EINVAL;
@@ -1711,7 +1787,7 @@
              "conv1_wino63v_dgrad_nt: needs vout / vout2 (>= M / 3 hexes, whole pairs, ld_vout %% 8 == 0) and vhalo");
   TL_REQUIRE(128LL * 8 * p.ld_vout * 4 < (1LL << 31), "conv1_wino63v_dgrad_nt: ld_vout too large");
   const long long ngrid = nwg < 256 ? nwg : 256;
-  hipLaunchKernelGGL((wino63v_nt_kernel<W_EPI_GY>), dim3((unsigned)ngrid), dim3(512), 0, (hipStream_t)stream, p);
+  hipLaunchKernelGGL((wino63v_nt_kernel<W_EPI_GY>), dim3((unsigned)ngrid), dim3(512), 0, (hipStream_t)stream, p, 0);
   return check_launch("conv1_wino63v_dgrad_nt");
 }
 
@@ -1728,14 +1804,18 @@
                p.ldc >= p.Ndim, "wino63v_tn: loader 3 needs Mdim %% 256, Ndim %% 64, lda / ldb %% 8");
     TL_REQUIRE(p.A_rows % 2 == 0 && p.B_rows % 2 == 0 && p.vd == nullptr, "wino63v_tn: loader 3: whole hex pairs in V and Y, no Vd");
     TL_REQUIRE(p.splitk <= 65535 && (p.splitk == 1 || p.slab_stride >= 8LL * p.Mdim * p.ldc), "wino63v_tn: bad splitk / slab_stride");
-    const long long ks = (p.Krows / 6 + T6_H - 1) / T6_H;
-    TL_REQUIRE(p.A_rows >= ks * T6_H && p.B_rows >= ks * T6_H, "wino63v_tn: V and Y must hold whole 6-hex K-steps (pad with zero hexes)");
+    const int live = v6_live_hexes(p.Tp, p.Tvalid, p.bm);
+    const long long hexes = live > 0 ? (p.Krows / p.Tp) * live : p.Krows / 6;
+    const long long ks = (hexes + T6_H - 1) / T6_H;
+    TL_REQUIRE(p.A_rows >= (p.Krows / 6 + T6_H - 1) / T6_H * T6_H && p.B_rows >= (p.Krows / 6 + T6_H - 1) / T6_H * T6_H,
+               "wino63v_tn: V and Y must hold whole 6-hex K-steps (pad with zero hexes)");
     const long long per3 = (ks + p.splitk - 1) / p.splitk;
-    TL_REQUIRE((per3 + 4) * (long long)T6_H * 8 * p.lda * 4 < (1LL << 31) && (per3 + 4) * (long long)T6_H * 8 * p.ldb * 4 < (1LL << 31),
+    const long long span3 = live > 0 ? ((per3 + 4) * T6_H / live + 2) * (p.Tp / 6) : (per3 + 4) * (long long)T6_H;
+    TL_REQUIRE(span3 * 8 * p.lda * 4 < (1LL << 31) && span3 * 8 * p.ldb * 4 < (1LL << 31),
                "wino63v_tn: a reduction split spans more than 2 GB of V or Y: raise splitk");
     const int ntm3 = p.Mdim / 256;
     hipLaunchKernelGGL(wino63v_tn4y_kernel, dim3((unsigned)(2 * ntm3 * (p.Ndim / T6_BN)), (unsigned)p.splitk, 1), dim3(512), 0,
-                       (hipStream_t)stream, p, ntm3);
+                       (hipStream_t)stream, p, ntm3, live);
     return check_launch("wino63v_tn (both operands pre-transformed)");
   }
   TL_REQUIRE(p.A && p.B && p.slab && p.bbits, "wino63v_tn: null V/B/bbits/slab");
```
